# LiyaoTang/contrastBoundary

Hardware: AMD Instinct MI355X
Metric: points/sec through KNN+group+KPConv+CBL block, S3DIS N=40960 K=16 (higher is better)
Workload: dtype f32

## Files before the change

contrastboundary_amd/csrc/knn_dispatch.hip:

```cpp
#include "cbl_common.h"

size_t cbl_knn_grid_workspace_bytes(int b, int n, int m, int nsample);
int cbl_knn_grid_launch(int b, int n, int m, int nsample, const float* xyz, const float* new_xyz, const int* offset,
                        const int* new_offset, int* idx, float* dist2, void* ws, size_t ws_bytes, int set_exact, hipStream_t st, int* order_out, CblKnnNarrow* narrow);

size_t cbl_knn_select_workspace_bytes(int b, int n, int m, int nsample);
int cbl_knn_select_launch(int b, int n, int m, int nsample, const float* xyz, const float* new_xyz, const int* offset, const int* new_offset,
                          int* idx, float* dist2, void* ws, size_t ws_bytes, int set_exact, hipStream_t st);

CBL_EXPORT size_t cbl_knnquery_workspace_bytes(int b, int n, int m, int nsample)
{
    const size_t g = cbl_knn_grid_workspace_bytes(b, n, m, nsample);
    return g ? g : cbl_knn_select_workspace_bytes(b, n, m, nsample);
}

static int knnquery_impl(int b, int n, int m, int nsample, const float* xyz, const float* new_xyz,
                         const int* offset, const int* new_offset, int* idx, float* dist2,
                         void* workspace, size_t workspace_bytes, int set_exact, void* stream, int* order_out = nullptr, CblKnnNarrow* narrow = nullptr)
{
    if (b <= 0 || n < 0 || m < 0 || nsample <= 0 || nsample > CBL_KNN_MAX_NSAMPLE) return CBL_ERR_BAD_ARG;
    if (m == 0) return CBL_OK;
    if (!xyz || !new_xyz || !offset || !new_offset || !idx || !dist2) return CBL_ERR_BAD_ARG;
    const size_t need = cbl_knn_grid_workspace_bytes(b, n, m, nsample);
    if (need > 0 && workspace && workspace_bytes >= need)
        return cbl_knn_grid_launch(b, n, m, nsample, xyz, new_xyz, offset, new_offset, idx, dist2, workspace, workspace_bytes, set_exact, cbl_stream(stream), order_out, narrow);
    if (order_out) return CBL_ERR_UNSUPPORTED;
    const size_t need_sel = cbl_knn_select_workspace_bytes(b, n, m, nsample);
    if (need_sel > 0 && workspace && workspace_bytes >= need_sel)
        return cbl_knn_select_launch(b, n, m, nsample, xyz, new_xyz, offset, new_offset, idx, dist2, workspace, workspace_bytes, set_exact, cbl_stream(stream));
    return cbl_knnquery_exact(b, n, m, nsample, xyz, new_xyz, offset, new_offset, idx, dist2, stream);
}

CBL_EXPORT int cbl_knnquery(int b, int n, int m, int nsample, const float* xyz, const float* new_xyz,
                            const int* offset, const int* new_offset, int* idx, float* dist2,
                            void* workspace, size_t workspace_bytes, void* stream)
{
    return knnquery_impl(b, n, m, nsample, xyz, new_xyz, offset, new_offset, idx, dist2, workspace, workspace_bytes, 0, stream);
}

CBL_EXPORT int cbl_knnquery_set(int b, int n, int m, int nsample, const float* xyz, const float* new_xyz,
                                const int* offset, const int* new_offset, int* idx, float* dist2,
                                void* workspace, size_t workspace_bytes, void* stream)
{
    return knnquery_impl(b, n, m, nsample, xyz, new_xyz, offset, new_offset, idx, dist2, workspace, workspace_bytes, 1, stream);
}

CBL_EXPORT int cbl_knnquery_anytie(int b, int n, int m, int nsample, const float* xyz, const float* new_xyz,
                                   const int* offset, const int* new_offset, int* idx, float* dist2,
                                   void* workspace, size_t workspace_bytes, void* stream)
{
    return knnquery_impl(b, n, m, nsample, xyz, new_xyz, offset, new_offset, idx, dist2, workspace, workspace_bytes, 2, stream);
}

CBL_EXPORT int cbl_knnquery_ordered(int b, int n, int m, int nsample, const float* xyz, const float* new_xyz,
                                    const int* offset, const int* new_offset, int* idx, float* dist2, int tie_policy, int* cell_order,
                                    void* workspace, size_t workspace_bytes, void* stream)
{
    if (tie_policy < 0 || tie_policy > 2 || !cell_order) return CBL_ERR_BAD_ARG;
    return knnquery_impl(b, n, m, nsample, xyz, new_xyz, offset, new_offset, idx, dist2, workspace, workspace_bytes, tie_policy, stream, cell_order);
}

int cbl_knn_block_candidates_launch(int b, int n, const int* offset, void* ws, int* count, hipStream_t st);

CBL_EXPORT int cbl_knn_grid_block_candidates(int b, int n, int nsample, const int* offset, int* count, void* workspace, size_t workspace_bytes, void* stream)
{
    const size_t need = cbl_knn_grid_workspace_bytes(b, n, n, nsample);
    if (need == 0) return CBL_ERR_UNSUPPORTED;
    if (workspace_bytes < need) return CBL_ERR_WORKSPACE;
    return cbl_knn_block_candidates_launch(b, n, offset, workspace, count, cbl_stream(stream));
}

int cbl_knn_exact_worklist(int b, int m, int K, const float* xyz, const float* new_xyz, const int* offset, const int* new_offset,
                           int* idx, float* dist2, const int* worklist, const int* worklist_count, int max_work, hipStream_t st,
                           const void* grids, const int* cell_start, const void* sorted);

namespace {
__global__ __launch_bounds__(256) void knn_prefix_kernel(int m, int kb, int ks, const int* __restrict__ idx_big, const float* __restrict__ d2_big,
                                                         int* __restrict__ idx, float* __restrict__ dist2, int set_exact,
                                                         int* __restrict__ worklist, int* __restrict__ counter)
{
    const int q = blockIdx.x * 256 + threadIdx.x;
    if (q >= m) return;
    const int* ib = idx_big + (size_t)q * kb; const float* db = d2_big + (size_t)q * kb;
    float prev = -1.f; bool dup = false, dup0 = false;
    for (int j = 0; j < ks; j++) {
        const float d = db[j];
        idx[(size_t)q * ks + j] = ib[j]; dist2[(size_t)q * ks + j] = d;
        dup = dup || (d == prev);
        dup0 = dup0 || (j == 1 && d == prev);
        prev = d;
    }
    const bool full = prev < 1e10f;
    const bool boundary = db[ks] == prev;
    const bool ok = full && !boundary && (set_exact ? !dup0 : !dup);
    if (!ok) worklist[atomicAdd(counter, 1)] = q;
}
template <int KS>
__global__ __launch_bounds__(256) void knn_prefix_pow2_kernel(int m, int kb, const int* __restrict__ idx_big, const float* __restrict__ d2_big,
                                                              int* __restrict__ idx, float* __restrict__ dist2, int set_exact,
                                                              int* __restrict__ worklist, int* __restrict__ counter)
{
    const long long e = (long long)blockIdx.x * 256 + threadIdx.x;
    const int lane = threadIdx.x & 63;
    const long long qq = e / KS;
    const int j = (int)(e - qq * KS);
    const bool live = qq < m;
    const int q = live ? (int)qq : m - 1;
    const float d = d2_big[(size_t)q * kb + j], dn = d2_big[(size_t)q * kb + j + 1];
    if (live) { idx[(size_t)q * KS + j] = idx_big[(size_t)q * kb + j]; dist2[(size_t)q * KS + j] = d; }
    const bool last = j == KS - 1;
    const bool bad = (d == dn && (last || j == 0 || !set_exact)) || (last && !(d < 1e10f));
    const unsigned long long bm = __ballot(bad && live);
    const unsigned long long gm = (KS == 64) ? bm : ((bm >> (lane & ~(KS - 1))) & ((1ull << KS) - 1ull));
    if (live && j == 0 && gm != 0ull) worklist[atomicAdd(counter, 1)] = q;
}
}

void cbl_knn_grid_scratch(void* ws, int b, int n, int m, int** worklist, int** worklist2, int** zero_counter, const void** grids,
                          const int** cell_start, const void** sorted);
int cbl_knn_exact_worklist2(int b, int m, const float* xyz, const float* new_xyz, const int* offset, const int* new_offset,
                            int K1, int* idx1, float* dist2_1, const int* worklist1, const int* count1,
                            int K2, int* idx2, float* dist2_2, const int* worklist2, const int* count2,
                            hipStream_t st, const void* grids, const int* cell_start, const void* sorted);

static int launch_prefix(int m, int nsample_wide, int nsample, const int* idx_wide, const float* dist2_wide, int* idx, float* dist2, int tie_policy,
                         int* worklist, int* counter, hipStream_t st)
{
#define CBL_PREFIX_POW2(KS) hipLaunchKernelGGL(knn_prefix_pow2_kernel<KS>, dim3(cbl_div_up((long long)m * KS, 256)), dim3(256), 0, st, m, nsample_wide, idx_wide, dist2_wide, \
                                               idx, dist2, tie_policy, worklist, counter)
    switch (nsample) {
        case 1: CBL_PREFIX_POW2(1); break;
        case 2: CBL_PREFIX_POW2(2); break;
        case 4: CBL_PREFIX_POW2(4); break;
        case 8: CBL_PREFIX_POW2(8); break;
        case 16: CBL_PREFIX_POW2(16); break;
        case 32: CBL_PREFIX_POW2(32); break;
        default:
            hipLaunchKernelGGL(knn_prefix_kernel, dim3(cbl_div_up(m, 256)), dim3(256), 0, st, m, nsample_wide, nsample, idx_wide, dist2_wide, idx, dist2, tie_policy, worklist, counter);
    }
#undef CBL_PREFIX_POW2
    return cbl_status();
}

CBL_EXPORT int cbl_knnquery_nested(int b, int n, int m, int nsample_wide, int tie_policy_wide, int nsample, int tie_policy,
                                   const float* xyz, const float* new_xyz, const int* offset, const int* new_offset,
                                   int* idx_wide, float* dist2_wide, int* idx, float* dist2, int* cell_order, void* event_after_wide,
                                   void* workspace, size_t workspace_bytes, void* stream)
{
    if (nsample <= 0 || nsample >= nsample_wide || tie_policy < 0 || tie_policy > 1 || tie_policy_wide < 0 || tie_policy_wide > 2 || !idx || !dist2) return CBL_ERR_BAD_ARG;
    const size_t need = cbl_knn_grid_workspace_bytes(b, n, m, nsample_wide);
    if (need == 0 || !workspace || workspace_bytes < need) return CBL_ERR_UNSUPPORTED;
    CblKnnNarrow narrow{nsample, tie_policy, idx, dist2, false, true};
    int rc = knnquery_impl(b, n, m, nsample_wide, xyz, new_xyz, offset, new_offset, idx_wide, dist2_wide, workspace, workspace_bytes, tie_policy_wide, stream, cell_order, &narrow);
    if (rc || m == 0) return rc;
    hipStream_t st = cbl_stream(stream);
    int *worklist, *worklist2, *counter; const void *grids, *sorted; const int* cell_start;
    cbl_knn_grid_scratch(workspace, b, n, m, &worklist, &worklist2, &counter, &grids, &cell_start, &sorted);
    if (narrow.fused) {
        const bool self = (new_xyz == xyz) && (m == n);
        rc = cbl_knn_exact_worklist2(b, m, xyz, new_xyz, offset, self ? offset : new_offset, nsample_wide, idx_wide, dist2_wide, worklist, counter - 1,
                                     nsample, idx, dist2, worklist2, counter, st, grids, cell_start, sorted);
        if (rc) return rc;
        if (event_after_wide && hipEventRecord(reinterpret_cast<hipEvent_t>(event_after_wide), st) != hipSuccess) return cbl_status() ? cbl_status() : CBL_ERR_BAD_ARG;
        return cbl_status();
    }
    if (event_after_wide && hipEventRecord(reinterpret_cast<hipEvent_t>(event_after_wide), st) != hipSuccess) return cbl_status() ? cbl_status() : CBL_ERR_BAD_ARG;
    {
        rc = launch_prefix(m, nsample_wide, nsample, idx_wide, dist2_wide, idx, dist2, tie_policy, worklist, counter, st);
        if (rc) return rc;
    }
    return cbl_knn_exact_worklist(b, m, nsample, xyz, new_xyz, offset, new_offset, idx, dist2, worklist, counter, m, st, grids, cell_start, sorted);
}

CBL_EXPORT size_t cbl_knnquery_prefix_workspace_bytes(int m) { return m < 0 ? 0 : sizeof(int) * ((size_t)m + 64); }

CBL_EXPORT int cbl_knnquery_prefix(int b, int n, int m, int nsample_wide, int nsample, const float* xyz, const float* new_xyz,
                                   const int* offset, const int* new_offset, const int* idx_wide, const float* dist2_wide,
                                   int* idx, float* dist2, int tie_policy, void* workspace, size_t workspace_bytes, void* stream)
{
    (void)n;
    if (b <= 0 || m < 0 || nsample <= 0 || nsample >= nsample_wide || nsample_wide > CBL_KNN_MAX_NSAMPLE || tie_policy < 0 || tie_policy > 1) return CBL_ERR_BAD_ARG;
    if (m == 0) return CBL_OK;
    if (!xyz || !new_xyz || !offset || !new_offset || !idx_wide || !dist2_wide || !idx || !dist2 || !workspace) return CBL_ERR_BAD_ARG;
    if (workspace_bytes < cbl_knnquery_prefix_workspace_bytes(m)) return CBL_ERR_WORKSPACE;
    hipStream_t st = cbl_stream(stream);
    int* counter = reinterpret_cast<int*>(workspace);
    int* worklist = counter + 64;
    (void)hipMemsetAsync(counter, 0, sizeof(int), st);
    { const int rcp = launch_prefix(m, nsample_wide, nsample, idx_wide, dist2_wide, idx, dist2, tie_policy, worklist, counter, st); if (rcp) return rcp; }
    const int rc = cbl_status();
    if (rc) return rc;
    return cbl_knn_exact_worklist(b, m, nsample, xyz, new_xyz, offset, new_offset, idx, dist2, worklist, counter, m, st, nullptr, nullptr, nullptr);
}
```

contrastboundary_amd/csrc/knn_grid.hip:

```cpp
#include "cbl_common.h"
#include <cstdlib>
#include "grid_core.h"
#include <knn_wave.h>

int cbl_knn_exact_worklist(int b, int m, int K, const float* xyz, const float* new_xyz, const int* offset,
                           const int* new_offset, int* idx, float* dist2,
                           const int* worklist, const int* worklist_count, int max_work, hipStream_t st,
                           const void* grids, const int* cell_start, const void* sorted);

namespace {

constexpr int GRID_MAX_K = 64;
constexpr int CELLS_PER_POINT = 2;
constexpr int CELLS_PER_CLOUD = 64;

struct Workspace {
    CblGrid* grids;
    int* counters;
    unsigned* bbox;
    int* cell_count;
    int* cell_start;
    int* cell_local;
    int* tile_sum;
    int* pt_cell;
// ... 1 lines not shown
    int* worklist;
    int* worklist2;
    size_t bytes;
    int ncap;
};

inline size_t align_up(size_t v) { return (v + 255) & ~(size_t)255; }

Workspace carve(void* base, int b, int n, int m)
{
    Workspace w;
    w.ncap = CELLS_PER_POINT * n + CELLS_PER_CLOUD * b;
    char* p = reinterpret_cast<char*>(base);
    size_t off = 0;
    auto take = [&](size_t bytes) { char* r = p ? p + off : nullptr; off += align_up(bytes); return r; };
    w.grids = reinterpret_cast<CblGrid*>(take(sizeof(CblGrid) * (size_t)b));
    w.counters = reinterpret_cast<int*>(take(sizeof(int) * 64));
    w.bbox = reinterpret_cast<unsigned*>(take(sizeof(unsigned) * 6 * (size_t)b));
    w.cell_count = reinterpret_cast<int*>(take(sizeof(int) * ((size_t)w.ncap + 1)));
    w.cell_start = reinterpret_cast<int*>(take(sizeof(int) * ((size_t)w.ncap + 1)));
    w.cell_local = reinterpret_cast<int*>(take(sizeof(int) * ((size_t)w.ncap + 1)));
    w.tile_sum = reinterpret_cast<int*>(take(sizeof(int) * ((size_t)w.ncap / 4096 + 2)));
    w.pt_cell = reinterpret_cast<int*>(take(sizeof(int) * (size_t)n));
    w.sorted = reinterpret_cast<float4*>(take(sizeof(float4) * (size_t)n));
    w.worklist = reinterpret_cast<int*>(take(sizeof(int) * (size_t)m));
    w.worklist2 = reinterpret_cast<int*>(take(sizeof(int) * (size_t)m));
    w.bytes = off;
    return w;
}

__device__ __forceinline__ unsigned f2key(float f) { const unsigned u = __float_as_uint(f); return (u & 0x80000000u) ? ~u : (u | 0x80000000u); }
__device__ __forceinline__ float key2f(unsigned k) { return __uint_as_float((k & 0x80000000u) ? (k & 0x7fffffffu) : ~k); }

__global__ __launch_bounds__(256) void grid_bbox_kernel(int b, int n, const float* __restrict__ xyz, const int* __restrict__ offset,
                                                        unsigned* __restrict__ bbox)
{
    const int per = (n + gridDim.x - 1) / gridDim.x;
    const int r0 = blockIdx.x * per, r1 = min(n, r0 + per);
    const int lane = threadIdx.x & 63;
    int i = r0 + threadIdx.x;
    if (r0 >= r1) return;
    {
        const int cfirst = cbl_cloud_of(r0, offset, b);
        if (cfirst == cbl_cloud_of(r1 - 1, offset, b)) {
            __shared__ float red[6][4];
            float lo[3] = {INFINITY, INFINITY, INFINITY}, hi[3] = {-INFINITY, -INFINITY, -INFINITY};
            for (; i < r1; i += 256) {
#pragma unroll
                for (int a = 0; a < 3; a++) { const float v = xyz[3 * i + a]; lo[a] = fminf(lo[a], v); hi[a] = fmaxf(hi[a], v); }
            }
#pragma unroll
            for (int a = 0; a < 3; a++) {
                for (int s = 32; s >= 1; s >>= 1) { lo[a] = fminf(lo[a], __shfl_xor(lo[a], s)); hi[a] = fmaxf(hi[a], __shfl_xor(hi[a], s)); }
                if (lane == 0) { red[a][threadIdx.x >> 6] = lo[a]; red[3 + a][threadIdx.x >> 6] = hi[a]; }
            }
            __syncthreads();
            if (threadIdx.x < 6) {
                const int a = threadIdx.x;
                const float v0 = red[a][0], v1 = red[a][1], v2 = red[a][2], v3 = red[a][3];
                if (a < 3) atomicMin(bbox + cfirst * 6 + a, f2key(fminf(fminf(v0, v1), fminf(v2, v3))));
                else       atomicMax(bbox + cfirst * 6 + a, f2key(fmaxf(fmaxf(v0, v1), fmaxf(v2, v3))));
            }
            return;
        }
    }
    while (__any(i < r1)) {
        const bool act = i < r1;
        const int myc = act ? cbl_cloud_of(i, offset, b) : -1;
        const int lead = __builtin_ctzll(__ballot(act));
        const int c0 = __shfl(myc, lead);
        float lo[3] = {INFINITY, INFINITY, INFINITY}, hi[3] = {-INFINITY, -INFINITY, -INFINITY};
        if (act && myc == c0) {
            const int cend = min(r1, offset[c0]);
            for (; i < cend; i += 256) {
#pragma unroll
                for (int a = 0; a < 3; a++) { const float v = xyz[3 * i + a]; lo[a] = fminf(lo[a], v); hi[a] = fmaxf(hi[a], v); }
            }
        }
#pragma unroll
        for (int a = 0; a < 3; a++) {
            for (int s = 32; s >= 1; s >>= 1) { lo[a] = fminf(lo[a], __shfl_xor(lo[a], s)); hi[a] = fmaxf(hi[a], __shfl_xor(hi[a], s)); }
            if (lane == 0 && lo[a] <= hi[a]) { atomicMin(bbox + c0 * 6 + a, f2key(lo[a])); atomicMax(bbox + c0 * 6 + 3 + a, f2key(hi[a])); }
        }
    }
}

__device__ __forceinline__ CblGrid grid_of_cloud(int c, float pts_per_cell, const int* __restrict__ offset, const unsigned* __restrict__ bbox)
{
    const int start = c ? offset[c - 1] : 0, end = offset[c];
    float l[3] = {0.f, 0.f, 0.f}, h[3] = {0.f, 0.f, 0.f};
    if (end > start)
        for (int a = 0; a < 3; a++) { l[a] = key2f(bbox[c * 6 + a]); h[a] = key2f(bbox[c * 6 + 3 + a]); }
    CblGrid g;
    const int cap = CELLS_PER_POINT * (end - start) + CELLS_PER_CLOUD;
    if (pts_per_cell < 0.f) cbl_grid_choose_radius(g, l, h, -pts_per_cell, cap);
    else cbl_grid_choose(g, l, h, end - start, pts_per_cell, cap);
    g.cell_base = CELLS_PER_POINT * start + CELLS_PER_CLOUD * c;
    g.start = start; g.end = end; g.pad0 = g.pad1 = 0;
    return g;
}

__global__ __launch_bounds__(256) void grid_count_kernel(int b, int n, float pts_per_cell, const float* __restrict__ xyz, const int* __restrict__ offset,
                                                         const unsigned* __restrict__ bbox, CblGrid* __restrict__ grids,
                                                         int* __restrict__ pt_cell, int* __restrict__ cell_count)
{
    if (blockIdx.x == 0)
        for (int c = threadIdx.x; c < b; c += 256) grids[c] = grid_of_cloud(c, pts_per_cell, offset, bbox);
    int cached_c = -1; CblGrid g;
    for (int i = blockIdx.x * 256 + threadIdx.x; i < n; i += gridDim.x * 256) {
        const int c = cbl_cloud_of(i, offset, b);
        if (c != cached_c) { g = grid_of_cloud(c, pts_per_cell, offset, bbox); cached_c = c; }
        const int cell = cbl_cell_of(g, xyz[3 * i], xyz[3 * i + 1], xyz[3 * i + 2]);
        pt_cell[i] = cell;
        atomicAdd(cell_count + cell, 1);
    }
}

constexpr int SCAN_TILE = 4096;

__global__ __launch_bounds__(256) void grid_scan_tiles_kernel(int total, const int* __restrict__ cell_count, int* __restrict__ cell_start_local,
                                                              int* __restrict__ tile_sum)
{
    __shared__ int wsum[4];
    const int tid = threadIdx.x, lane = tid & 63, wave = tid >> 6;
    const int base = blockIdx.x * SCAN_TILE + tid * 16;
    int v[16];
#pragma unroll
    for (int j = 0; j < 16; j += 4) {
        if (base + j + 3 < total) {
            const int4 x = *reinterpret_cast<const int4*>(cell_count + base + j);
            v[j] = x.x; v[j + 1] = x.y; v[j + 2] = x.z; v[j + 3] = x.w;
        } else {
#pragma unroll
            for (int k = 0; k < 4; k++) v[j + k] = (base + j + k < total) ? cell_count[base + j + k] : 0;
        }
    }
    int sum = 0;
#pragma unroll
    for (int j = 0; j < 16; j++) { const int x = v[j]; v[j] = sum; sum += x; }
    int incl = sum;
#pragma unroll
    for (int s = 1; s < 64; s <<= 1) { const int o = __shfl_up(incl, s); if (lane >= s) incl += o; }
    if (lane == 63) wsum[wave] = incl;
    __syncthreads();
    int off = incl - sum;
    for (int w = 0; w < wave; w++) off += wsum[w];
    if (tid == 255) tile_sum[blockIdx.x] = off + sum;
#pragma unroll
    for (int j = 0; j < 16; j++) if (base + j < total) cell_start_local[base + j] = off + v[j];
}

__global__ __launch_bounds__(256) void grid_scatter_kernel(int n, int total, int ntiles, const float* __restrict__ xyz, const int* __restrict__ pt_cell,
                                                           const int* __restrict__ tile_sum, int* __restrict__ cell_start_local, int* __restrict__ cell_start,
                                                           int* __restrict__ cell_count, float4* __restrict__ sorted, int* __restrict__ order_out)
{
    extern __shared__ int tile_lds[];
    int* tile_pre = tile_lds + ntiles;
    {
        for (int t = threadIdx.x; t < ntiles; t += 256) tile_lds[t] = tile_sum[t];
        __syncthreads();
        for (int t = threadIdx.x; t < ntiles; t += 256) { int run = 0; for (int u = 0; u < t; u++) run += tile_lds[u]; tile_pre[t] = run; }
        __syncthreads();
    }
    for (int i = blockIdx.x * 256 + threadIdx.x; i < total; i += gridDim.x * 256) cell_start[i] = cell_start_local[i] + tile_pre[i / SCAN_TILE];
    for (int i = blockIdx.x * 256 + threadIdx.x; i < n; i += gridDim.x * 256) {
        const int cell = pt_cell[i];
        const int pos = cell_start_local[cell] + tile_pre[cell / SCAN_TILE] + atomicSub(cell_count + cell, 1) - 1;
        sorted[pos] = make_float4(xyz[3 * i], xyz[3 * i + 1], xyz[3 * i + 2], __int_as_float(i));
        if (order_out) order_out[pos] = i;
    }
}

__device__ __forceinline__ void grid_order_canon_body(int n, const int* __restrict__ pt_cell, const int* __restrict__ cell_start,
                                                      const float4* __restrict__ sorted, int* __restrict__ order, int block, int nblocks)
{
    for (int i = block * 256 + threadIdx.x; i < n; i += nblocks * 256) {
        const int cell = pt_cell[i];
        const int s = cell_start[cell], e = cell_start[cell + 1];
        if (e - s < 2 || e - s > 1024) continue;
        int rank = 0;
        for (int j = s; j < e; j += 8) {
            int v[8];
#pragma unroll
            for (int u = 0; u < 8; u++) v[u] = __float_as_int(sorted[min(j + u, e - 1)].w);
#pragma unroll
            for (int u = 0; u < 8; u++) rank += (j + u < e && v[u] < i) ? 1 : 0;
        }
        order[s + rank] = i;
    }
}
__global__ __launch_bounds__(256) void grid_order_canon_kernel(int n, const int* __restrict__ pt_cell, const int* __restrict__ cell_start,
                                                               const float4* __restrict__ sorted, int* __restrict__ order)
{
    grid_order_canon_body(n, pt_cell, cell_start, sorted, order, blockIdx.x, gridDim.x);
}
struct CblCanon { int blocks, n; const int* pt_cell; int* order; };

template <int G> __device__ __forceinline__ float dpp_shr1_f(float v);
template <int G> __device__ __forceinline__ int dpp_shr1_i(int v);
template <> __device__ __forceinline__ int dpp_shr1_i<16>(int v) { return __builtin_amdgcn_update_dpp(v, v, 0x111, 0xf, 0xf, false); }
template <> __device__ __forceinline__ int dpp_shr1_i<64>(int v) { return __builtin_amdgcn_update_dpp(v, v, 0x138, 0xf, 0xf, false); }
template <> __device__ __forceinline__ int dpp_shr1_i<32>(int v) { return __builtin_amdgcn_update_dpp(v, v, 0x138, 0xf, 0xf, false); }
template <int G> __device__ __forceinline__ int dpp_shr1_zero(int v)
{
    if constexpr (G == 16) return __builtin_amdgcn_update_dpp(0, v, 0x111, 0xf, 0xf, true);
    else                   return __builtin_amdgcn_update_dpp(0, v, 0x138, 0xf, 0xf, true);
}
template <> __device__ __forceinline__ float dpp_shr1_f<16>(float v) { return __int_as_float(dpp_shr1_i<16>(__float_as_int(v))); }
template <> __device__ __forceinline__ float dpp_shr1_f<64>(float v) { return __int_as_float(dpp_shr1_i<64>(__float_as_int(v))); }
template <> __device__ __forceinline__ float dpp_shr1_f<32>(float v) { return __int_as_float(dpp_shr1_i<32>(__float_as_int(v))); }

constexpr int WV_NB = 16;

template <int CTRL> __device__ __forceinline__ int dppx_i(int v) { return __builtin_amdgcn_update_dpp(0, v, CTRL, 0xf, 0xf, true); }
struct PermQuadXor1  { __device__ __forceinline__ int operator()(int v, int) const { return dppx_i<0xB1>(v); } };
struct PermQuadXor2  { __device__ __forceinline__ int operator()(int v, int) const { return dppx_i<0x4E>(v); } };
struct PermQuadMir   { __device__ __forceinline__ int operator()(int v, int) const { return dppx_i<0x1B>(v); } };
struct PermHalfMir   { __device__ __forceinline__ int operator()(int v, int) const { return dppx_i<0x141>(v); } };
struct PermRowMir    { __device__ __forceinline__ int operator()(int v, int) const { return dppx_i<0x140>(v); } };
struct PermRowRor8   { __device__ __forceinline__ int operator()(int v, int) const { return dppx_i<0x128>(v); } };
struct PermSwzXor4   { __device__ __forceinline__ int operator()(int v, int) const { return __builtin_amdgcn_ds_swizzle(v, 0x101f); } };
struct PermSwzXor16  { __device__ __forceinline__ int operator()(int v, int) const { return __builtin_amdgcn_ds_swizzle(v, 0x401f); } };
struct PermSwzMir32  { __device__ __forceinline__ int operator()(int v, int) const { return __builtin_amdgcn_ds_swizzle(v, 0x7c1f); } };
struct PermMir64     { __device__ __forceinline__ int operator()(int v, int lane) const { return __builtin_amdgcn_ds_bpermute((63 - lane) << 2, v); } };

template <bool LEX, class Perm> __device__ __forceinline__ void sort_cx(float& d, int& i, bool lower, int lane, Perm perm)
{
    const float pd = __int_as_float(perm(__float_as_int(d), lane));
    const int pi = perm(i, lane);
    if (LEX) {
        const bool take = lower ? (pd < d || (pd == d && (unsigned)pi < (unsigned)i)) : (pd > d || (pd == d && (unsigned)pi > (unsigned)i));
        d = take ? pd : d; i = take ? pi : i;
    } else {
        const int di = __float_as_int(d), pdi = __float_as_int(pd);
        const int nd = lower ? min(di, pdi) : max(di, pdi);
        i = (nd != di) ? pi : i; d = __int_as_float(nd);
    }
}
template <bool LEX> __device__ __forceinline__ void wave_sort64(float& d, int& i, int lane)
{
    const bool l1 = !(lane & 1), l2 = !(lane & 2), l4 = !(lane & 4), l8 = !(lane & 8), l16 = !(lane & 16), l32 = !(lane & 32);
    sort_cx<LEX>(d, i, l1, lane, PermQuadXor1());
    sort_cx<LEX>(d, i, l2, lane, PermQuadMir());   sort_cx<LEX>(d, i, l1, lane, PermQuadXor1());
    sort_cx<LEX>(d, i, l4, lane, PermHalfMir());   sort_cx<LEX>(d, i, l2, lane, PermQuadXor2()); sort_cx<LEX>(d, i, l1, lane, PermQuadXor1());
    sort_cx<LEX>(d, i, l8, lane, PermRowMir());    sort_cx<LEX>(d, i, l4, lane, PermSwzXor4());  sort_cx<LEX>(d, i, l2, lane, PermQuadXor2());
    sort_cx<LEX>(d, i, l1, lane, PermQuadXor1());
    sort_cx<LEX>(d, i, l16, lane, PermSwzMir32()); sort_cx<LEX>(d, i, l8, lane, PermRowRor8());  sort_cx<LEX>(d, i, l4, lane, PermSwzXor4());
    sort_cx<LEX>(d, i, l2, lane, PermQuadXor2());  sort_cx<LEX>(d, i, l1, lane, PermQuadXor1());
    sort_cx<LEX>(d, i, l32, lane, PermMir64());    sort_cx<LEX>(d, i, l16, lane, PermSwzXor16()); sort_cx<LEX>(d, i, l8, lane, PermRowRor8());
    sort_cx<LEX>(d, i, l4, lane, PermSwzXor4());   sort_cx<LEX>(d, i, l2, lane, PermQuadXor2()); sort_cx<LEX>(d, i, l1, lane, PermQuadXor1());
}
__device__ __forceinline__ float rl_f(float v, int l) { return __int_as_float(__builtin_amdgcn_readlane(__float_as_int(v), l)); }
template <int G> __device__ __forceinline__ float group_min_nonneg(float f)
{
    int v = __float_as_int(f);
    v = min(v, dppx_i<0xB1>(v)); v = min(v, dppx_i<0x4E>(v)); v = min(v, dppx_i<0x141>(v)); v = min(v, dppx_i<0x140>(v));
    if constexpr (G == 32) v = min(v, __builtin_amdgcn_ds_swizzle(v, 0x401f));
    if constexpr (G == 64) v = min(min(__builtin_amdgcn_readlane(v, 0), __builtin_amdgcn_readlane(v, 16)),
                                   min(__builtin_amdgcn_readlane(v, 32), __builtin_amdgcn_readlane(v, 48)));
    return __int_as_float(v);
}

template <int G, bool SELF, bool LEX>
__global__ __launch_bounds__(256) void knn_grid_group_kernel(int b, int m, int K, const float* __restrict__ new_xyz,
                                                             const int* __restrict__ offset, const int* __restrict__ new_offset,
                                                             const CblGrid* __restrict__ grids, const int* __restrict__ cell_start,
                                                             const float4* __restrict__ sorted, int* __restrict__ idx, float* __restrict__ dist2,
                                                             int* __restrict__ worklist, int* __restrict__ counters, int set_exact)
{
    constexpr int QPW = 64 / G;
    using mask_t = unsigned long long;
    const int lane = threadIdx.x & 63;
    const int gl = lane & (G - 1);
    const int grp = lane / G;
    const int wave_global = (blockIdx.x * 256 + threadIdx.x) >> 6;
    const int t = wave_global * QPW + grp;
    const bool live = t < m;
    const int tt = live ? t : m - 1;

    int q; float qx, qy, qz;
    if (SELF) { const float4 s = sorted[tt]; q = __float_as_int(s.w); qx = s.x; qy = s.y; qz = s.z; }
    else      { q = tt; qx = new_xyz[3 * q]; qy = new_xyz[3 * q + 1]; qz = new_xyz[3 * q + 2]; }
    const int c = cbl_cloud_of(q, SELF ? offset : new_offset, b);
    const CblGrid g = grids[c];
    const float uqx = cbl_u(qx, g.ox, g.inv_cs), uqy = cbl_u(qy, g.oy, g.inv_cs), uqz = cbl_u(qz, g.oz, g.inv_cs);
    const int cx = cbl_cell_coord(uqx, g.nx), cy = cbl_cell_coord(uqy, g.ny), cz = cbl_cell_coord(uqz, g.nz);

    float ed = INFINITY; int ei = -1;
    float rejmin = INFINITY;
    int evict = 0x7f800000;
    const int last_src = ((lane & ~(G - 1)) + K - 1) << 2;
    bool done = !live;

    int rs9 = 0, re9 = 0;
    if (!done && gl < 9) {
        const int o = (int)((0xa82091645ull >> (4 * gl)) & 0xFull);
        const int y = cy + (o & 3) - 1, z = cz + (o >> 2) - 1;
        if (y >= 0 && y < g.ny && z >= 0 && z < g.nz) {
            const int row = g.cell_base + g.nx * (y + g.ny * z);
            rs9 = cell_start[row + max(cx - 1, 0)]; re9 = cell_start[row + min(cx + 1, g.nx - 1) + 1];
        }
    }
    const int grp_src = (lane & ~(G - 1)) << 2;

    for (int r = 1;; r++) {
        const int side = 2 * r + 1;
        for (int ri = 0; ri < side * side; ri++) {
            int dy, dz;
            if (r == 1) { const int o = (int)((0xa82091645ull >> (4 * ri)) & 0xFull); dy = (o & 3) - 1; dz = (o >> 2) - 1; }
            else        { dz = ri / side - r; dy = ri % side - r; }
            {
                const bool full = (r == 1) || dz == -r || dz == r || dy == -r || dy == r;
                const int nseg = full ? 1 : 2;
                for (int sg = 0; sg < nseg; sg++) {
                    int x0, x1;
                    if (full) { x0 = max(cx - r, 0); x1 = min(cx + r, g.nx - 1); }
                    else      { x0 = x1 = sg ? cx + r : cx - r; }
                    const int y = cy + dy, z = cz + dz;
                    int s = 0, e = 0;
                    if (r == 1) {
                        s = __builtin_amdgcn_ds_bpermute(grp_src + (ri << 2), rs9); e = __builtin_amdgcn_ds_bpermute(grp_src + (ri << 2), re9);
                    } else if (!done && y >= 0 && y < g.ny && z >= 0 && z < g.nz && x0 >= 0 && x1 <= g.nx - 1) {
                        const int row = g.cell_base + g.nx * (y + g.ny * z);
                        s = cell_start[row + x0]; e = cell_start[row + x1 + 1];
                    }
                    for (int p = s; __any(p < e); p += G) {
                        const int pi = p + gl;
                        float d2 = INFINITY; int ci = -1;
                        if (pi < e) {
                            const float4 v = sorted[pi];
                            d2 = cbl_dist2(qx, qy, qz, v.x, v.y, v.z);
                            ci = __float_as_int(v.w);
                        }
                        const float worst = __int_as_float(__builtin_amdgcn_ds_bpermute(last_src, __float_as_int(ed)));
                        const unsigned worst_i = LEX ? (unsigned)__builtin_amdgcn_ds_bpermute(last_src, ei) : 0u;
                        const bool pass = d2 < worst || (LEX && d2 == worst && (unsigned)ci < worst_i);
                        rejmin = __int_as_float(min(__float_as_int(rejmin), pass ? 0x7f800000 : __float_as_int(d2)));
                        if constexpr (!LEX && G <= 32) {
                            unsigned gm = (unsigned)(__ballot(pass) >> (grp * G)) & (G == 32 ? ~0u : ((1u << G) - 1u));
                            const int d2i = __float_as_int(d2);
                            auto step = [&]() {
                                const bool has = gm != 0;
                                const int l = kw_ffbl(gm);
                                gm &= gm - 1;
                                const int src = (l << 2) + grp * (G * 4);
                                int dci = __builtin_amdgcn_ds_bpermute(src, d2i); const int ic = __builtin_amdgcn_ds_bpermute(src, ci);
                                dci = has ? dci : 0x7f800000;
                                const int edi = __float_as_int(ed);
                                int pdi = dpp_shr1_zero<G>(edi), pidx = dpp_shr1_zero<G>(ei);
                                if (G == 32) pdi = gl ? pdi : 0;
                                evict = min(evict, max(edi, dci));
                                ei = (edi > dci) ? ((pdi > dci) ? pidx : ic) : ei;
                                ed = __int_as_float(min(edi, max(pdi, dci)));
                            };
                            while (__any(gm != 0)) {
                                step();
                                if (!__any(gm != 0)) break;
                                step();
                            }
                        } else {
                        mask_t gm = (__ballot(pass) >> (grp * G)) & (G == 64 ? ~0ull : ((1ull << G) - 1ull));
                        while (__any(gm != 0)) {
                            const bool has = gm != 0;
                            const int l = has ? __builtin_ctzll(gm) : 0;
                            gm &= gm - 1;
                            float dc = __shfl(d2, l, G); int ic = __shfl(ci, l, G);
                            if (!has) { dc = INFINITY; ic = -1; }
                            const float pd = dpp_shr1_f<G>(ed); const int pidx = dpp_shr1_i<G>(ei);
                            const bool gt = ed > dc || (LEX && ed == dc && (unsigned)ei > (unsigned)ic);
                            const bool left_gt = (gl > 0) && (pd > dc || (LEX && pd == dc && (unsigned)pidx > (unsigned)ic));
                            if (gl == K - 1) rejmin = fminf(rejmin, gt ? ed : dc);
                            if (gt) { if (left_gt) { ed = pd; ei = pidx; } else { ed = dc; ei = ic; } }
                        }
                        }
                    }
                }
            }
        }
        const float bound2 = cbl_outside_bound2(g, uqx, uqy, uqz, cx, cy, cz, r);
        const float worst = __int_as_float(__builtin_amdgcn_ds_bpermute(last_src, __float_as_int(ed)));
        if (!done) done = (bound2 == INFINITY) || (worst < bound2);
        if (__all(done)) break;
    }

    const float worst = __int_as_float(__builtin_amdgcn_ds_bpermute(last_src, __float_as_int(ed)));
    const float rm = group_min_nonneg<G>(fminf(rejmin, gl == K - 1 ? __int_as_float(evict) : INFINITY));
    const float pd = dpp_shr1_f<G>(ed);
    const bool dup = (gl > 0) && (gl < K) && (ed == pd);
    const mask_t dm = (__ballot(dup) >> (grp * G)) & (G == 64 ? ~0ull : ((1ull << G) - 1ull));
    const bool ok = (worst < INFINITY) && (set_exact == 2 || ((rm != worst) && (set_exact ? !(dm & 2ull) : dm == 0)));
    if (live) {
        if (gl < K) { idx[(size_t)q * K + gl] = ei; dist2[(size_t)q * K + gl] = ed; }
        if (!ok && gl == 0) worklist[atomicAdd(counters, 1)] = q;
    }
}


template <bool SELF, bool LEX>
__global__ __launch_bounds__(256) void knn_grid_wave_kernel(int b, int m, int K, const float* __restrict__ new_xyz,
                                                            const int* __restrict__ offset, const int* __restrict__ new_offset,
                                                            const CblGrid* __restrict__ grids, const int* __restrict__ cell_start,
                                                            const float4* __restrict__ sorted, int* __restrict__ idx, float* __restrict__ dist2,
                                                            int* __restrict__ worklist, int* __restrict__ counters, int set_exact,
                                                            int ks, int* __restrict__ idx_n, float* __restrict__ dist2_n,
                                                            int* __restrict__ worklist_n, int set_exact_n, CblCanon canon)
{
    __shared__ float2 slots[4][64];
    if ((int)blockIdx.x < canon.blocks) {
        grid_order_canon_body(canon.n, canon.pt_cell, cell_start, sorted, canon.order, blockIdx.x, canon.blocks);
        return;
    }
    const int lane = threadIdx.x & 63, wv = threadIdx.x >> 6;
    const int t = __builtin_amdgcn_readfirstlane(((int)blockIdx.x - canon.blocks) * 4 + wv);
    if (t >= m) return;
    int q; float qx, qy, qz;
    if (SELF) { const float4 s = sorted[t]; q = __float_as_int(s.w); qx = s.x; qy = s.y; qz = s.z; }
    else      { q = t; qx = new_xyz[3 * q]; qy = new_xyz[3 * q + 1]; qz = new_xyz[3 * q + 2]; }
    q = __builtin_amdgcn_readfirstlane(q);
    const int c = cbl_cloud_of(q, SELF ? offset : new_offset, b);
    const CblGrid g = grids[c];
    const float uqx = cbl_u(qx, g.ox, g.inv_cs), uqy = cbl_u(qy, g.oy, g.inv_cs), uqz = cbl_u(qz, g.oz, g.inv_cs);
    const int cx = cbl_cell_coord(uqx, g.nx), cy = cbl_cell_coord(uqy, g.ny), cz = cbl_cell_coord(uqz, g.nz);

    int rs = 0, rlen = 0;
    if (lane < 9) {
        const int y = cy + lane % 3 - 1, z = cz + lane / 3 - 1;
        if (y >= 0 && y < g.ny && z >= 0 && z < g.nz) {
            const int row = g.cell_base + g.nx * (y + g.ny * z);
            rs = cell_start[row + max(cx - 1, 0)];
            rlen = cell_start[row + min(cx + 1, g.nx - 1) + 1] - rs;
        }
    }
    int pre[9], delta[9], T = 0;
#pragma unroll
    for (int r = 0; r < 9; r++) {
        const int s_r = __builtin_amdgcn_readlane(rs, r), l_r = __builtin_amdgcn_readlane(rlen, r);
        pre[r] = T; delta[r] = s_r - T; T += l_r;
    }

    float ed = INFINITY; int ei = -1;
    float rejmin = INFINITY;
    bool fast = (T >= K) && (T <= 64 * WV_NB);
    if (fast) {
        float d[WV_NB]; int id[WV_NB];
        int delta_v[9];
#pragma unroll
        for (int r = 0; r < 9; r++) delta_v[r] = kw_in_vgpr(delta[r]);
#pragma unroll
        for (int j0 = 0; j0 < WV_NB; j0 += 4) {
            float4 p[4];
#pragma unroll
            for (int u = 0; u < 4; u++) {
                if ((j0 + u) * 64 < T) {
                    const int v = min((j0 + u) * 64 + lane, T - 1);
                    int dl = delta_v[0];
#pragma unroll
                    for (int r = 1; r < 9; r++) dl = (v >= pre[r]) ? delta_v[r] : dl;
                    p[u] = sorted[v + dl];
                }
            }
#pragma unroll
            for (int u = 0; u < 4; u++) {
                const int j = j0 + u;
                d[j] = INFINITY; id[j] = -1;
                if (j * 64 < T) {
                    const bool in = j * 64 + lane < T;
                    const float dd = cbl_dist2(qx, qy, qz, p[u].x, p[u].y, p[u].z);
                    d[j] = in ? dd : INFINITY; id[j] = in ? __float_as_int(p[u].w) : -1;
                }
            }
        }
        float tau = 3.0e38f;
        if (T > 64) {
            int mxi = 0;
#pragma unroll
            for (int j = 0; j < WV_NB; j++) {
                if ((j + 1) * 64 <= T) mxi = max(mxi, __float_as_int(d[j]));
                else if (j * 64 < T)   mxi = max(mxi, d[j] < INFINITY ? __float_as_int(d[j]) : 0);
            }
            mxi = max(mxi, dppx_i<0xB1>(mxi)); mxi = max(mxi, dppx_i<0x4E>(mxi));
            mxi = max(mxi, dppx_i<0x141>(mxi)); mxi = max(mxi, dppx_i<0x140>(mxi));
            float lo = -1.f, hi = __int_as_float(max(max(__builtin_amdgcn_readlane(mxi, 0), __builtin_amdgcn_readlane(mxi, 16)),
                                                     max(__builtin_amdgcn_readlane(mxi, 32), __builtin_amdgcn_readlane(mxi, 48))));
            const float first = (float)(K + 64) * 0.6f * __builtin_amdgcn_rcpf((float)T);
            fast = false;
            for (int it = 0; it < 40; it++) {
                const float mid = it == 0 ? hi * first : lo + (hi - lo) * 0.5f;
                if (!(mid > lo && mid < hi)) break;
                int cnt = 0;
#pragma unroll
                for (int j = 0; j < WV_NB; j++) if (j * 64 < T) cnt += __popcll(__ballot(d[j] <= mid));
                if (cnt < K) lo = mid; else if (cnt > 64) hi = mid; else { tau = mid; fast = true; break; }
            }
        }
        if (fast) {
            int base = 0;
#pragma unroll
            for (int j = 0; j < WV_NB; j++) {
                if (j * 64 < T) {
                    const bool pass = d[j] <= tau;
                    const unsigned long long mk = __ballot(pass);
                    if (pass) {
                        const int slot = base + __builtin_amdgcn_mbcnt_hi((unsigned)(mk >> 32), __builtin_amdgcn_mbcnt_lo((unsigned)mk, 0));
                        slots[wv][slot] = make_float2(d[j], __int_as_float(id[j]));
                    } else rejmin = fminf(rejmin, d[j]);
                    base += __popcll(mk);
                }
            }
            __builtin_amdgcn_fence(__ATOMIC_RELEASE, "wavefront");
            __builtin_amdgcn_wave_barrier();
            __builtin_amdgcn_fence(__ATOMIC_ACQUIRE, "wavefront");
            float sd = INFINITY; int si = -1;
            if (lane < base) { const float2 v = slots[wv][lane]; sd = v.x; si = __float_as_int(v.y); }
            wave_sort64<LEX>(sd, si, lane);
            if (lane < K) { ed = sd; ei = si; } else rejmin = fminf(rejmin, sd);
        }
    }

    bool done = false;
    int r = 1;
    if (fast) {
        const float bound2 = cbl_outside_bound2(g, uqx, uqy, uqz, cx, cy, cz, 1);
        done = (bound2 == INFINITY) || (rl_f(ed, K - 1) < bound2);
        r = 2;
    }
    for (; !done; r++) {
        const int side = 2 * r + 1;
        for (int ri = 0; ri < side * side; ri++) {
            const int dz = ri / side - r, dy = ri % side - r;
            const bool full = (r == 1) || dz == -r || dz == r || dy == -r || dy == r;
            const int nseg = full ? 1 : 2;
            for (int sg = 0; sg < nseg; sg++) {
                int x0, x1;
                if (full) { x0 = max(cx - r, 0); x1 = min(cx + r, g.nx - 1); }
                else      { x0 = x1 = sg ? cx + r : cx - r; }
                const int y = cy + dy, z = cz + dz;
                int s = 0, e = 0;
                if (y >= 0 && y < g.ny && z >= 0 && z < g.nz && x0 >= 0 && x1 <= g.nx - 1) {
                    const int row = g.cell_base + g.nx * (y + g.ny * z);
                    s = cell_start[row + x0]; e = cell_start[row + x1 + 1];
                }
                s = __builtin_amdgcn_readfirstlane(s); e = __builtin_amdgcn_readfirstlane(e);
                for (int p = s; p < e; p += 64) {
                    const int pi = p + lane;
                    float d2 = INFINITY; int ci = -1;
                    if (pi < e) {
                        const float4 v = sorted[pi];
                        d2 = cbl_dist2(qx, qy, qz, v.x, v.y, v.z);
                        ci = __float_as_int(v.w);
                    }
                    const float worst = rl_f(ed, K - 1); const unsigned worst_i = LEX ? (unsigned)__builtin_amdgcn_readlane(ei, K - 1) : 0u;
                    const bool pass = d2 < worst || (LEX && d2 == worst && (unsigned)ci < worst_i);
                    rejmin = fminf(rejmin, pass ? INFINITY : d2);
                    unsigned long long gm = __ballot(pass);
                    while (gm) {
                        const int l = __builtin_ctzll(gm);
                        gm &= gm - 1;
                        const float dc = rl_f(d2, l); const int ic = __builtin_amdgcn_readlane(ci, l);
                        const float pd = dpp_shr1_f<64>(ed); const int pidx = dpp_shr1_i<64>(ei);
                        const bool gt = ed > dc || (LEX && ed == dc && (unsigned)ei > (unsigned)ic);
                        const bool left_gt = (lane > 0) && (pd > dc || (LEX && pd == dc && (unsigned)pidx > (unsigned)ic));
                        if (lane == K - 1) rejmin = fminf(rejmin, gt ? ed : dc);
// ... 34 lines not shown
}


template <int G>
__device__ __forceinline__ unsigned long long group_min_u64(unsigned long long v)
{
#pragma unroll
    for (int s = G / 2; s >= 1; s >>= 1) {
        const unsigned lo = __shfl_xor((unsigned)v, s, G), hi = __shfl_xor((unsigned)(v >> 32), s, G);
        const unsigned long long o = ((unsigned long long)hi << 32) | lo;
        v = o < v ? o : v;
    }
    return v;
}

__device__ __forceinline__ unsigned long long radius_key_lds(int t, int total, int c1, int c2, int c3, int c4, int c5, int c6, int c7, int c8, const int* __restrict__ otab,
                                                              float qx, float qy, float qz, float r2, const float4* __restrict__ sorted)
{
    const bool have = t < total;
    const int r = (t >= c1) + (t >= c2) + (t >= c3) + (t >= c4) + (t >= c5) + (t >= c6) + (t >= c7) + (t >= c8);
    const int o = otab[r];
    const float4 v = sorted[have ? t + o : 0];
    const float d2 = cbl_dist2(qx, qy, qz, v.x, v.y, v.z);
    return (have && d2 < r2) ? (((unsigned long long)__float_as_uint(d2) << 32) | (unsigned)__float_as_int(v.w)) : ~0ull;
}

template <int G, int U>
__global__ __launch_bounds__(256) void radius_group_kernel(int b, int nq, int ns_total, int limit, float r2, const float* __restrict__ queries,
                                                           const int* __restrict__ q_offset, const CblGrid* __restrict__ grids,
                                                           const int* __restrict__ cell_start, const float4* __restrict__ sorted,
                                                           int* __restrict__ out, int* __restrict__ counts, int* __restrict__ max_count)
{
    constexpr int QPW = 64 / G, CAP = 2 * G, NBF = G >= 64 ? 2 : 4;
    using mask_t = unsigned long long;
    using key_t = unsigned long long;
    constexpr key_t NONE = ~0ull;
    __shared__ key_t slots[4 * QPW][CAP];
    __shared__ int otabs[4 * QPW][U][12];
    const int lane = threadIdx.x & 63, gl = lane & (G - 1), grp = lane / G;
    key_t* S = slots[(threadIdx.x >> 6) * QPW + grp];
    const int wave_global = (blockIdx.x * 256 + threadIdx.x) >> 6;
    const mask_t below = (1ull << gl) - 1ull, gmask = G == 64 ? ~0ull : ((1ull << G) - 1ull);
    int q[U]; bool live[U]; float qx[U], qy[U], qz[U];
#pragma unroll
    for (int u = 0; u < U; u++) {
        const int t = (wave_global * QPW + grp) * U + u;
        live[u] = t < nq; q[u] = live[u] ? t : nq - 1;
        qx[u] = queries[3 * q[u]]; qy[u] = queries[3 * q[u] + 1]; qz[u] = queries[3 * q[u] + 2];
    }
    int rs[U], re[U];
#pragma unroll
    for (int u = 0; u < U; u++) {
        const int c = cbl_cloud_of(q[u], q_offset, b);
        const CblGrid g = grids[c];
        const int cx = cbl_cell_coord(cbl_u(qx[u], g.ox, g.inv_cs), g.nx), cy = cbl_cell_coord(cbl_u(qy[u], g.oy, g.inv_cs), g.ny),
                  cz = cbl_cell_coord(cbl_u(qz[u], g.oz, g.inv_cs), g.nz);
        const int x0 = max(cx - 1, 0), x1 = min(cx + 1, g.nx - 1);
        rs[u] = 0; re[u] = 0;
        if (gl < 9) {
            const int y = cy + (gl % 3) - 1, z = cz + (gl / 3) - 1;
            if (live[u] && g.end > g.start && y >= 0 && y < g.ny && z >= 0 && z < g.nz) {
                const int row = g.cell_base + g.nx * (y + g.ny * z);
                rs[u] = cell_start[row + x0]; re[u] = cell_start[row + x1 + 1];
            }
        }
    }
    int c1[U], c2[U], c3[U], c4[U], c5[U], c6[U], c7[U], c8[U], total[U];
#pragma unroll
    for (int u = 0; u < U; u++) {
        int* otab = otabs[(threadIdx.x >> 6) * QPW + grp][u];
        int acc = 0;
#define CBL_ROW(r, cnext) { const int sr = __shfl(rs[u], r, G), er = __shfl(re[u], r, G); if (gl == 0) otab[r] = sr - acc; acc += er - sr; cnext = acc; }
        CBL_ROW(0, c1[u]) CBL_ROW(1, c2[u]) CBL_ROW(2, c3[u]) CBL_ROW(3, c4[u]) CBL_ROW(4, c5[u]) CBL_ROW(5, c6[u]) CBL_ROW(6, c7[u]) CBL_ROW(7, c8[u])
        CBL_ROW(8, total[u])
#undef CBL_ROW
    }
#define CBL_KEY(u, t) radius_key_lds((t), total[u], c1[u], c2[u], c3[u], c4[u], c5[u], c6[u], c7[u], c8[u], otabs[(threadIdx.x >> 6) * QPW + grp][u], qx[u], qy[u], qz[u], r2, sorted)
    key_t first[U][NBF];
#pragma unroll
    for (int u = 0; u < U; u++)
#pragma unroll
        for (int k = 0; k < NBF; k++) first[u][k] = CBL_KEY(u, k * G + gl);
#pragma unroll
    for (int u = 0; u < U; u++) {
        int inside = 0;
        auto collect = [&](key_t key) __attribute__((always_inline)) {
            const bool in_ball = key != NONE;
            const mask_t gm = (__ballot(in_ball) >> (grp * G)) & gmask;
            const int slot = inside + __popcll(gm & below);
            if (in_ball && slot < CAP) S[slot] = key;
            inside += __popcll(gm);
        };
#pragma unroll
        for (int k = 0; k < NBF; k++) collect(first[u][k]);
        for (int t0 = NBF * G; __any(t0 < total[u]); t0 += G) collect(CBL_KEY(u, t0 + gl));
        const bool over = inside > CAP;
        if (!over) {
            const int n = inside;
            const key_t ka = gl < n ? S[gl] : NONE, kb = gl + G < n ? S[gl + G] : NONE;
            int ra = 0, rb = 0;
            for (int k = 0; __any(k < n); k += 4) {
                key_t kk[4];
#pragma unroll
                for (int j = 0; j < 4; j++) kk[j] = S[min(k + j, CAP - 1)];
#pragma unroll
                for (int j = 0; j < 4; j++) {
                    const bool on = k + j < n;
                    ra += (on && kk[j] < ka) ? 1 : 0; rb += (on && kk[j] < kb) ? 1 : 0;
                }
            }
            if (live[u]) {
                if (ka != NONE && ra < limit) out[(size_t)q[u] * limit + ra] = (int)(unsigned)ka;
                if (kb != NONE && rb < limit) out[(size_t)q[u] * limit + rb] = (int)(unsigned)kb;
                if (gl >= n && gl < limit) out[(size_t)q[u] * limit + gl] = ns_total;
            }
        }
        if (__any(over)) {
            key_t prev = 0; bool none_yet = true;
            for (int col = 0; col < limit; col++) {
                key_t best = NONE;
                for (int t0 = 0; __any(over && t0 < total[u]); t0 += G) {
                    const key_t key = CBL_KEY(u, t0 + gl);
                    if ((none_yet || key > prev) && key < best) best = key;
                }
                best = group_min_u64<G>(best);
                if (over && live[u] && gl == 0) out[(size_t)q[u] * limit + col] = best == NONE ? ns_total : (int)(unsigned)best;
                prev = best; none_yet = false;
            }
        }
        if (live[u] && gl == 0) {
            if (counts) counts[q[u]] = inside;
            if (inside > __hip_atomic_load(max_count, __ATOMIC_RELAXED, __HIP_MEMORY_SCOPE_AGENT)) atomicMax(max_count, inside);
        }
    }
#undef CBL_KEY
}

}

int cbl_bbox_keys_launch(int b, int n, const float* xyz, const int* offset, unsigned* bbox, hipStream_t st)
{
    hipLaunchKernelGGL(grid_bbox_kernel, dim3(cbl_grid_for(n, 1024, 512)), dim3(256), 0, st, b, n, xyz, offset, bbox);
    return cbl_status();
}

__global__ __launch_bounds__(256) void grid_init_kernel(int b, int total, int* __restrict__ counters, unsigned* __restrict__ bbox, int* __restrict__ cell_count)
{
    const int i0 = blockIdx.x * 256 + threadIdx.x;
    if (i0 < 64) counters[i0] = 0;
    if (i0 < 6 * b) bbox[i0] = ((i0 % 6) < 3) ? 0xffffffffu : 0u;
    for (int i = i0; i < total; i += gridDim.x * 256) cell_count[i] = 0;
}

int cbl_grid_build(int b, int n, float pts_per_cell, const float* xyz, const int* offset, void* ws, hipStream_t st, int* order_out = nullptr, bool canon_later = false)
{
    Workspace w = carve(ws, b, n, 0);
    const int total = w.ncap + 1, ntiles = (total + SCAN_TILE - 1) / SCAN_TILE;
    hipLaunchKernelGGL(grid_init_kernel, dim3(cbl_grid_for(total, 256, 512)), dim3(256), 0, st, b, total, w.counters, w.bbox, w.cell_count);
    hipLaunchKernelGGL(grid_bbox_kernel, dim3(cbl_grid_for(n, 1024, 512)), dim3(256), 0, st, b, n, xyz, offset, w.bbox);
    hipLaunchKernelGGL(grid_count_kernel, dim3(cbl_grid_for(n, 256)), dim3(256), 0, st, b, n, pts_per_cell, xyz, offset, w.bbox, w.grids, w.pt_cell, w.cell_count);
    hipLaunchKernelGGL(grid_scan_tiles_kernel, dim3(ntiles), dim3(256), 0, st, total, w.cell_count, w.cell_local, w.tile_sum);
    hipLaunchKernelGGL(grid_scatter_kernel, dim3(cbl_grid_for(n, 256)), dim3(256), 2 * sizeof(int) * (size_t)ntiles, st, n, total, ntiles, xyz, w.pt_cell,
                       w.tile_sum, w.cell_local, w.cell_start, w.cell_count, w.sorted, order_out);
    if (order_out && !canon_later)
        hipLaunchKernelGGL(grid_order_canon_kernel, dim3(cbl_grid_for(n, 256)), dim3(256), 0, st, n, w.pt_cell, w.cell_start, w.sorted, order_out);
    return cbl_status();
}

__global__ __launch_bounds__(256) void knn_block_candidates_kernel(int b, int n, const int* __restrict__ offset, const CblGrid* __restrict__ grids,
                                                                   const int* __restrict__ cell_start, const float4* __restrict__ sorted, int* __restrict__ count)
{
    const int t = blockIdx.x * 256 + threadIdx.x;
    if (t >= n) return;
    const float4 s = sorted[t];
    const int q = __float_as_int(s.w);
    const CblGrid g = grids[cbl_cloud_of(q, offset, b)];
    const int cx = cbl_cell_coord(cbl_u(s.x, g.ox, g.inv_cs), g.nx), cy = cbl_cell_coord(cbl_u(s.y, g.oy, g.inv_cs), g.ny), cz = cbl_cell_coord(cbl_u(s.z, g.oz, g.inv_cs), g.nz);
    int T = 0;
    for (int r = 0; r < 9; r++) {
        const int y = cy + r % 3 - 1, z = cz + r / 3 - 1;
        if (y >= 0 && y < g.ny && z >= 0 && z < g.nz) {
            const int row = g.cell_base + g.nx * (y + g.ny * z);
            T += cell_start[row + min(cx + 1, g.nx - 1) + 1] - cell_start[row + max(cx - 1, 0)];
        }
    }
    count[q] = T;
}

int cbl_knn_block_candidates_launch(int b, int n, const int* offset, void* ws, int* count, hipStream_t st)
{
    Workspace w = carve(ws, b, n, n);
    hipLaunchKernelGGL(knn_block_candidates_kernel, dim3(cbl_grid_for(n, 256, 1 << 20)), dim3(256), 0, st, b, n, offset, w.grids, w.cell_start, w.sorted, count);
    return cbl_status();
}

size_t cbl_knn_grid_workspace_bytes(int b, int n, int m, int nsample)
{
    if (nsample > GRID_MAX_K || n < 2048 || b <= 0) return 0;
    if ((long long)CELLS_PER_POINT * n + (long long)CELLS_PER_CLOUD * b > 0x3fffffffLL) return 0;
    return carve(nullptr, b, n, m).bytes;
}

void cbl_knn_grid_scratch(void* ws, int b, int n, int m, int** worklist, int** worklist2, int** zero_counter, const void** grids, const int** cell_start,
                          const void** sorted)
{
    Workspace w = carve(ws, b, n, m);
    *worklist = w.worklist; *worklist2 = w.worklist2; *zero_counter = w.counters + 1;
    *grids = w.grids; *cell_start = w.cell_start; *sorted = w.sorted;
}

int cbl_knn_grid_launch(int b, int n, int m, int nsample, const float* xyz, const float* new_xyz, const int* offset,
                        const int* new_offset, int* idx, float* dist2, void* ws, size_t ws_bytes, int set_exact, hipStream_t st, int* order_out,
                        CblKnnNarrow* narrow)
{
    Workspace w = carve(ws, b, n, m);
    if (ws_bytes < w.bytes) return CBL_ERR_WORKSPACE;
    static const float fill = [] { const char* e = getenv("CBL_KNN_CELL_FILL"); const float v = e ? (float)atof(e) : 0.f; return (v > 0.05f && v < 4.f) ? v : 0.33f; }();
    const bool wave_search = nsample > 16;
    int rc = cbl_grid_build(b, n, fill * (float)(nsample < 4 ? 4 : nsample), xyz, offset, ws, st, order_out, wave_search);
    if (rc) return rc;
    const bool self = (new_xyz == xyz) && (m == n);
    if (wave_search) {
        CblCanon canon = {0, n, w.pt_cell, order_out};
        if (order_out) canon.blocks = (int)cbl_grid_for(n, 256);
        const dim3 grid(cbl_div_up(m, 4) + canon.blocks), block(256);
        const int ks = narrow ? narrow->nsample : 0;
        int* idx_n = narrow ? narrow->idx : nullptr; float* dist2_n = narrow ? narrow->dist2 : nullptr;
        const int set_n = narrow ? narrow->set_exact : 0;
        if (narrow) narrow->fused = true;
#define CBL_LAUNCH_WAVE(SELF_, LEX_) hipLaunchKernelGGL((knn_grid_wave_kernel<SELF_, LEX_>), grid, block, 0, st, b, m, nsample, new_xyz, offset, new_offset, w.grids, \
                                                       w.cell_start, w.sorted, idx, dist2, w.worklist, w.counters, set_exact, ks, idx_n, dist2_n, w.worklist2, set_n, canon)
        if (set_exact == 2) { if (self) CBL_LAUNCH_WAVE(true, true); else CBL_LAUNCH_WAVE(false, true); }
        else                { if (self) CBL_LAUNCH_WAVE(true, false); else CBL_LAUNCH_WAVE(false, false); }
#undef CBL_LAUNCH_WAVE
    }
    else launch_query<16>(self, b, m, nsample, new_xyz, offset, new_offset, w, idx, dist2, set_exact, st);
    rc = cbl_status();
    if (rc) return rc;
    if (narrow && narrow->fused && narrow->defer_replay) return CBL_OK;
    return cbl_knn_exact_worklist(b, m, nsample, xyz, new_xyz, self ? offset : offset, self ? offset : new_offset, idx, dist2,
                                  w.worklist, w.counters, m, st, w.grids, w.cell_start, w.sorted);
}

size_t cbl_radius_workspace_bytes_impl(int b, int ns) { return (b > 0 && ns >= 0) ? carve(nullptr, b, ns, 0).bytes : 0; }

int cbl_radius_launch(int b, int nq, int ns, const float* queries, const float* supports, const int* q_offset, const int* s_offset,
                      float radius, int limit, int* out, int* counts, int* max_count, void* ws, size_t ws_bytes, hipStream_t st, bool grid_is_built)
{
    Workspace w = carve(ws, b, ns, 0);
    if (ws_bytes < w.bytes) return CBL_ERR_WORKSPACE;
    int rc = grid_is_built ? CBL_OK : cbl_grid_build(b, ns, -radius, supports, s_offset, ws, st);
    if (rc) return rc;
    hipError_t e = hipMemsetAsync(max_count, 0, sizeof(int), st);
    if (e != hipSuccess) return (int)e;
    const int G = limit <= 16 ? 16 : limit <= 32 ? 32 : 64;
    const long long waves = ((long long)nq + (64 / G) - 1) / (64 / G);
    const dim3 grid(cbl_div_up(waves, 4)), block(256);
    const float r2 = radius * radius;
    const int ru = (long long)nq / ((64 / G) * 2) >= 49152 ? 2 : 1;
    const long long waves_u = ((long long)nq + (64 / G) * ru - 1) / ((64 / G) * ru);
    const dim3 grid_u(cbl_div_up(waves_u, 4));
#define CBL_RAD(G_, U_) hipLaunchKernelGGL((radius_group_kernel<G_, U_>), grid_u, block, 0, st, b, nq, ns, limit, r2, queries, q_offset, w.grids, w.cell_start, w.sorted, out, counts, max_count)
    if (ru == 2) { if (G == 16) CBL_RAD(16, 2); else if (G == 32) CBL_RAD(32, 2); else CBL_RAD(64, 2); }
    else         { if (G == 16) CBL_RAD(16, 1); else if (G == 32) CBL_RAD(32, 1); else CBL_RAD(64, 1); }
#undef CBL_RAD
    return cbl_status();
}
```

contrastboundary_amd/csrc/neighbor_transpose.hip:

```cpp
#include "cbl_common.h"
#include <stdlib.h>

namespace {

constexpr int TT = 64;
constexpr int TS = 64;
constexpr int NB = 256;
constexpr int NT_MAX_TILES = 16384;
constexpr int NT_SCAN_SPLIT = 2048;
constexpr int STAGE_CAP = 12288;


struct NtWs {
    int* rank;
    int* tile_cursor;
    int* list_cursor;
    int* tile_list_off;
    int* tile_list_n;
    int* tile_base;
    int2* lists;
    int2* bins;
    int* scratch;
};

static size_t nt_align(size_t v) { return (v + 255) & ~(size_t)255; }
static int nt_tiles(int n) { return (n + TT - 1) / TT; }
static int nt_src_tiles(int m) { return (m + TS - 1) / TS; }

static size_t nt_carve(NtWs& w, char* base, int m, int n, int nsample)
{
    const size_t P = (size_t)m * nsample;
    const int ntt = nt_tiles(n), nst = nt_src_tiles(m);
    size_t off = 0;
    auto take = [&](size_t bytes) { char* p = base ? base + off : nullptr; off += nt_align(bytes); return p; };
    w.rank = (int*)take(sizeof(int) * (size_t)(n > 0 ? n : 1));
    w.tile_cursor = (int*)take(sizeof(int) * (size_t)(ntt + 2));
    w.list_cursor = w.tile_cursor ? w.tile_cursor + ntt + 1 : nullptr;
    w.tile_list_off = (int*)take(sizeof(int) * (size_t)(nst + 1));
    w.tile_list_n = (int*)take(sizeof(int) * (size_t)(nst + 1));
    w.tile_base = (int*)take(sizeof(int) * (size_t)(ntt + 2));
    w.lists = (int2*)take(sizeof(int2) * (P ? P : 1));
    w.bins = (int2*)take(sizeof(int2) * (P ? P : 1));
    w.scratch = (int*)take(sizeof(int) * (P ? P : 1));
    return off;
}

__global__ __launch_bounds__(NB) void nt_prep_kernel(int n, int nzero, const int* __restrict__ order, int* __restrict__ rank, int* __restrict__ zero,
                                                     int* __restrict__ zero2)
{
    const int i = blockIdx.x * NB + threadIdx.x;
    if (order && i < n) rank[order[i]] = i;
    if (i < nzero) { zero[i] = 0; if (zero2) zero2[i] = 0; }
}

template <int UN> struct NtPairs { unsigned p[UN]; int r[UN]; };

template <int UN>
__device__ __forceinline__ void nt_load_pairs(NtPairs<UN>& q, unsigned base, unsigned total, int n, int ns, CblFastDiv dv, const int* __restrict__ src_ids,
                                              const int* __restrict__ idx, const int* __restrict__ rank)
{
    int t[UN];
#pragma unroll
    for (int u = 0; u < UN; u++) {
        const unsigned e = base + (unsigned)u * NB + threadIdx.x;
        const bool in = e < total;
        const unsigned sl = cbl_fastdiv(in ? e : 0u, dv), col = (in ? e : 0u) - sl * (unsigned)ns;
        q.p[u] = (unsigned)src_ids[sl] * (unsigned)ns + col;
        t[u] = in ? idx[q.p[u]] : -1;
    }
#pragma unroll
    for (int u = 0; u < UN; u++) {
        const bool ok = (unsigned)t[u] < (unsigned)n;
        q.r[u] = ok ? (rank ? rank[t[u]] : t[u]) : -1;
    }
}

struct NtJob {
    int ns; CblFastDiv dv; const int* idx;
    int *tile_cursor, *list_cursor, *tile_list_off, *tile_list_n, *tile_base; int2 *lists, *bins; int* scratch;
    int *inv_start, *inv_src;
};

template <int UN>
__device__ __forceinline__ void nt_count_body(int* lds, int m, int n, int ns, int ntt, CblFastDiv dv, const int* __restrict__ idx, const int* __restrict__ order_src,
                                              const int* __restrict__ rank, int* __restrict__ tile_cursor, int* __restrict__ list_cursor,
                                              int* __restrict__ tile_list_off, int* __restrict__ tile_list_n, int2* __restrict__ lists)
{
    int* hist = lds;
    int2* mine = reinterpret_cast<int2*>(lds + ((ntt + 1) & ~1));
    __shared__ int nmine, gbase, src_ids[TS];
    const int st = blockIdx.x;
    const int nsrc = min(TS, m - st * TS);
    if ((int)threadIdx.x < TS) src_ids[threadIdx.x] = (int)threadIdx.x < nsrc ? (order_src ? order_src[st * TS + threadIdx.x] : st * TS + (int)threadIdx.x) : 0;
    for (int e = threadIdx.x; e < ntt; e += NB) hist[e] = 0;
    if (threadIdx.x == 0) nmine = 0;
    __syncthreads();
    const unsigned total = (unsigned)nsrc * (unsigned)ns;
    for (unsigned base = 0; base < total; base += UN * NB) {
        NtPairs<UN> q;
        nt_load_pairs<UN>(q, base, total, n, ns, dv, src_ids, idx, rank);
#pragma unroll
        for (int u = 0; u < UN; u++) if (q.r[u] >= 0) atomicAdd(&hist[q.r[u] / TT], 1);
    }
    __syncthreads();
    for (int tt = threadIdx.x; tt < ntt; tt += NB) {
        const int c = hist[tt];
        if (c) {
            const int off = atomicAdd(&tile_cursor[tt], c);
            mine[atomicAdd(&nmine, 1)] = make_int2(tt, off);
        }
    }
    __syncthreads();
    if (threadIdx.x == 0) { gbase = st * TS * ns; tile_list_off[st] = gbase; tile_list_n[st] = nmine; }
    __syncthreads();
    for (int e = threadIdx.x; e < nmine; e += NB) lists[gbase + e] = mine[e];
}
template <int UN>
__global__ __launch_bounds__(NB) void nt_count_kernel(int m, int n, int ns, int ntt, CblFastDiv dv, const int* __restrict__ idx, const int* __restrict__ order_src,
                                                      const int* __restrict__ rank, int* __restrict__ tile_cursor, int* __restrict__ list_cursor,
                                                      int* __restrict__ tile_list_off, int* __restrict__ tile_list_n, int2* __restrict__ lists)
{
    extern __shared__ int lds[];
    nt_count_body<UN>(lds, m, n, ns, ntt, dv, idx, order_src, rank, tile_cursor, list_cursor, tile_list_off, tile_list_n, lists);
}
template <int UNA, int UNB>
__global__ __launch_bounds__(NB) void nt_count_pair_kernel(int m, int n, int ntt, const int* __restrict__ order_src, const int* __restrict__ rank, NtJob a, NtJob b)
{
    extern __shared__ int lds[];
    if (blockIdx.y == 0) nt_count_body<UNA>(lds, m, n, a.ns, ntt, a.dv, a.idx, order_src, rank, a.tile_cursor, a.list_cursor, a.tile_list_off, a.tile_list_n, a.lists);
    else                 nt_count_body<UNB>(lds, m, n, b.ns, ntt, b.dv, b.idx, order_src, rank, b.tile_cursor, b.list_cursor, b.tile_list_off, b.tile_list_n, b.lists);
}

__global__ __launch_bounds__(1024) void nt_scan_kernel(int ntt, const int* __restrict__ tile_cursor, int* __restrict__ tile_base)
{
    __shared__ int wave_tot[16];
    constexpr int PER = NT_MAX_TILES / 1024;
    const int c0 = threadIdx.x * PER;
    int v[PER], sum = 0;
#pragma unroll
    for (int k = 0; k < PER; k++) { v[k] = (c0 + k < ntt) ? tile_cursor[c0 + k] : 0; sum += v[k]; }
    int incl = sum;
    for (int k = 1; k < 64; k <<= 1) { const int o = __shfl_up(incl, k); if ((int)(threadIdx.x & 63) >= k) incl += o; }
    if ((threadIdx.x & 63) == 63) wave_tot[threadIdx.x >> 6] = incl;
    __syncthreads();
    int run = incl - sum;
    for (int w = 0; w < (int)(threadIdx.x >> 6); w++) run += wave_tot[w];
#pragma unroll
    for (int k = 0; k < PER; k++) { if (c0 + k < ntt) tile_base[c0 + k] = run; run += v[k]; }
    if (threadIdx.x == 1023) tile_base[ntt] = run;
}

template <int UN, bool SCANNED>
__device__ __forceinline__ void nt_bin_body(int* lds, int m, int n, int ns, int ntt, CblFastDiv dv, const int* __restrict__ idx, const int* __restrict__ order_src,
                                            const int* __restrict__ rank, const int* __restrict__ tile_cursor, const int* __restrict__ tile_list_off,
                                            const int* __restrict__ tile_list_n, const int2* __restrict__ lists, int* __restrict__ tile_base,
                                            int2* __restrict__ bins)
{
    int* where = lds;
    int* hist = lds + ntt;
    __shared__ int wave_tot[NB / 64], src_ids[TS];
    const int st = blockIdx.x;
    const int nsrc = min(TS, m - st * TS);
    if ((int)threadIdx.x < TS) src_ids[threadIdx.x] = (int)threadIdx.x < nsrc ? (order_src ? order_src[st * TS + threadIdx.x] : st * TS + (int)threadIdx.x) : 0;
    if (SCANNED) {
        const int nl0 = tile_list_n[st], lo0 = tile_list_off[st];
        for (int e = threadIdx.x; e < nl0; e += NB) { const int2 r = lists[lo0 + e]; where[r.x] = tile_base[r.x] + r.y; hist[r.x] = 0; }
        __syncthreads();
    } else {
    for (int e = threadIdx.x; e < ntt; e += NB) { where[e] = tile_cursor[e]; hist[e] = 0; }
    __syncthreads();
    const int per = (ntt + NB - 1) / NB;
    const int c0 = threadIdx.x * per, c1 = min(ntt, c0 + per);
    int sum = 0;
    for (int e = c0; e < c1; e++) sum += where[e];
    int incl = sum;
    for (int k = 1; k < 64; k <<= 1) { const int v = __shfl_up(incl, k); if ((threadIdx.x & 63) >= k) incl += v; }
    if ((threadIdx.x & 63) == 63) wave_tot[threadIdx.x >> 6] = incl;
    __syncthreads();
    int run = incl - sum;
    for (int w = 0; w < (int)(threadIdx.x >> 6); w++) run += wave_tot[w];
    for (int e = c0; e < c1; e++) { const int c = where[e]; where[e] = run; if (st == 0) tile_base[e] = run; run += c; }
    if (st == 0 && threadIdx.x == NB - 1) tile_base[ntt] = run;
    __syncthreads();
    const int nl = tile_list_n[st], lo = tile_list_off[st];
    for (int e = threadIdx.x; e < nl; e += NB) { const int2 r = lists[lo + e]; where[r.x] += r.y; }
    __syncthreads();
    }
    const unsigned total = (unsigned)nsrc * (unsigned)ns;
    for (unsigned base = 0; base < total; base += UN * NB) {
        NtPairs<UN> q;
        nt_load_pairs<UN>(q, base, total, n, ns, dv, src_ids, idx, rank);
#pragma unroll
        for (int u = 0; u < UN; u++)
            if (q.r[u] >= 0) { const int tt = q.r[u] / TT; bins[where[tt] + atomicAdd(&hist[tt], 1)] = make_int2(q.r[u] & (TT - 1), (int)q.p[u]); }
    }
}
template <int UN, bool SCANNED>
__global__ __launch_bounds__(NB) void nt_bin_kernel(int m, int n, int ns, int ntt, CblFastDiv dv, const int* __restrict__ idx, const int* __restrict__ order_src,
                                                    const int* __restrict__ rank, const int* __restrict__ tile_cursor, const int* __restrict__ tile_list_off,
                                                    const int* __restrict__ tile_list_n, const int2* __restrict__ lists, int* __restrict__ tile_base,
                                                    int2* __restrict__ bins)
{
    extern __shared__ int lds[];
    nt_bin_body<UN, SCANNED>(lds, m, n, ns, ntt, dv, idx, order_src, rank, tile_cursor, tile_list_off, tile_list_n, lists, tile_base, bins);
}
template <int UNA, int UNB>
__global__ __launch_bounds__(NB) void nt_bin_pair_kernel(int m, int n, int ntt, const int* __restrict__ order_src, const int* __restrict__ rank, NtJob a, NtJob b)
{
    extern __shared__ int lds[];
    if (blockIdx.y == 0) nt_bin_body<UNA, false>(lds, m, n, a.ns, ntt, a.dv, a.idx, order_src, rank, a.tile_cursor, a.tile_list_off, a.tile_list_n, a.lists, a.tile_base, a.bins);
    else                 nt_bin_body<UNB, false>(lds, m, n, b.ns, ntt, b.dv, b.idx, order_src, rank, b.tile_cursor, b.tile_list_off, b.tile_list_n, b.lists, b.tile_base, b.bins);
}

constexpr int EPT = 16;

template <int CTRL> __device__ __forceinline__ int nt_dpp(int v) { return __builtin_amdgcn_update_dpp(0, v, CTRL, 0xf, 0xf, true); }
__device__ __forceinline__ int nt_cx(int v, int partner, bool lower) { return lower ? min(v, partner) : max(v, partner); }
__device__ __forceinline__ int nt_wave_sort64(int v, int lane)
{
    const bool l1 = !(lane & 1), l2 = !(lane & 2), l4 = !(lane & 4), l8 = !(lane & 8), l16 = !(lane & 16), l32 = !(lane & 32);
#define X1(v) nt_dpp<0xB1>(v)
#define X2(v) nt_dpp<0x4E>(v)
#define QM(v) nt_dpp<0x1B>(v)
#define HM(v) nt_dpp<0x141>(v)
#define RM(v) nt_dpp<0x140>(v)
#define R8(v) nt_dpp<0x128>(v)
#define S4(v) __builtin_amdgcn_ds_swizzle(v, 0x101f)
#define S16(v) __builtin_amdgcn_ds_swizzle(v, 0x401f)
#define M32(v) __builtin_amdgcn_ds_swizzle(v, 0x7c1f)
#define M64(v) __builtin_amdgcn_ds_bpermute((63 - lane) << 2, v)
    v = nt_cx(v, X1(v), l1);
    v = nt_cx(v, QM(v), l2);  v = nt_cx(v, X1(v), l1);
    v = nt_cx(v, HM(v), l4);  v = nt_cx(v, X2(v), l2);  v = nt_cx(v, X1(v), l1);
    v = nt_cx(v, RM(v), l8);  v = nt_cx(v, S4(v), l4);  v = nt_cx(v, X2(v), l2);  v = nt_cx(v, X1(v), l1);
    v = nt_cx(v, M32(v), l16); v = nt_cx(v, R8(v), l8); v = nt_cx(v, S4(v), l4);  v = nt_cx(v, X2(v), l2); v = nt_cx(v, X1(v), l1);
    v = nt_cx(v, M64(v), l32); v = nt_cx(v, S16(v), l16); v = nt_cx(v, R8(v), l8); v = nt_cx(v, S4(v), l4); v = nt_cx(v, X2(v), l2); v = nt_cx(v, X1(v), l1);
#undef X1
#undef X2
#undef QM
#undef HM
#undef RM
#undef R8
#undef S4
#undef S16
#undef M32
#undef M64
    return v;
}

__device__ __forceinline__ void nt_rank_sort(const int* __restrict__ stage, const int* lstart, int* __restrict__ out)
{
    const int lane = threadIdx.x & 63, wave = threadIdx.x >> 6;
    for (int base = wave * (TT / (NB / 64)); base < (wave + 1) * (TT / (NB / 64)); base += 4) {
        int v[4], s0v[4], Lv[4];
#pragma unroll
        for (int u = 0; u < 4; u++) {
            s0v[u] = lstart[base + u]; Lv[u] = lstart[base + u + 1] - s0v[u];
            v[u] = (lane < Lv[u] && Lv[u] <= 64) ? stage[s0v[u] + lane] : 0x7fffffff;
        }
#pragma unroll
        for (int u = 0; u < 4; u++) v[u] = nt_wave_sort64(v[u], lane);
#pragma unroll
        for (int u = 0; u < 4; u++) if (Lv[u] <= 64 && lane < Lv[u]) out[s0v[u] + lane] = v[u];
    }
    for (int slot = wave; slot < TT; slot += NB / 64) {
        const int s0 = lstart[slot], L = lstart[slot + 1] - s0;
        if (L <= 64) continue;
        for (int c = 0; c < L; c += 64) {
            const int e = c + lane;
            const int mine = e < L ? stage[s0 + e] : 0x7fffffff;
            int rnk = 0, o = 0;
            for (; o + 8 <= L; o += 8) {
                int v[8];
#pragma unroll
                for (int u = 0; u < 8; u++) v[u] = stage[s0 + o + u];
#pragma unroll
                for (int u = 0; u < 8; u++) rnk += (v[u] < mine) ? 1 : 0;
            }
            for (; o < L; o++) rnk += (stage[s0 + o] < mine) ? 1 : 0;
            if (e < L) out[s0 + rnk] = mine;
        }
    }
}

__device__ __forceinline__ void nt_finish_body(int n, int ntt, const int* __restrict__ tile_base, const int2* __restrict__ bins, int* __restrict__ scratch,
                                               int* __restrict__ inv_start, int* __restrict__ inv_src)
{
    __shared__ int cnt[TT], lstart[TT + 1];
    __shared__ int stage_lds[STAGE_CAP];
    const int tt = blockIdx.x;
    const int b0 = tile_base[tt], E = tile_base[tt + 1] - b0;
    const bool in_regs = E <= EPT * NB;
    if (threadIdx.x < TT) cnt[threadIdx.x] = 0;
    int2 r[EPT];
    if (in_regs) {
#pragma unroll
        for (int u = 0; u < EPT; u++) { const int e = u * NB + (int)threadIdx.x; r[u] = e < E ? bins[b0 + e] : make_int2(-1, 0); }
    }
    __syncthreads();
    if (in_regs) {
#pragma unroll
        for (int u = 0; u < EPT; u++) if (r[u].x >= 0) atomicAdd(&cnt[r[u].x], 1);
    } else {
        for (int e = threadIdx.x; e < E; e += NB) atomicAdd(&cnt[bins[b0 + e].x], 1);
    }
    __syncthreads();
    if (threadIdx.x < 64) {
        const int c = cnt[threadIdx.x];
        int incl = c;
        for (int k = 1; k < 64; k <<= 1) { const int v = __shfl_up(incl, k); if ((int)threadIdx.x >= k) incl += v; }
        lstart[threadIdx.x] = incl - c;
        if (threadIdx.x == 63) lstart[TT] = incl;
        const int row = tt * TT + threadIdx.x;
        if (row < n) inv_start[row] = b0 + incl - c;
        if (tt == ntt - 1 && threadIdx.x == 63) inv_start[n] = b0 + incl;
        cnt[threadIdx.x] = 0;
    }
    __syncthreads();
    if (E <= STAGE_CAP) {
        if (in_regs) {
#pragma unroll
            for (int u = 0; u < EPT; u++) if (r[u].x >= 0) stage_lds[lstart[r[u].x] + atomicAdd(&cnt[r[u].x], 1)] = r[u].y;
        } else {
            for (int e = threadIdx.x; e < E; e += NB) { const int2 v = bins[b0 + e]; stage_lds[lstart[v.x] + atomicAdd(&cnt[v.x], 1)] = v.y; }
        }
        __syncthreads();
        nt_rank_sort(stage_lds, lstart, inv_src + b0);
    } else {
        int* stage = scratch + b0;
        for (int e = threadIdx.x; e < E; e += NB) { const int2 v = bins[b0 + e]; stage[lstart[v.x] + atomicAdd(&cnt[v.x], 1)] = v.y; }
        __threadfence_block();
        __syncthreads();
        nt_rank_sort(stage, lstart, inv_src + b0);
    }
}
__global__ __launch_bounds__(NB) void nt_finish_kernel(int n, int ntt, const int* __restrict__ tile_base, const int2* __restrict__ bins, int* __restrict__ scratch,
                                                       int* __restrict__ inv_start, int* __restrict__ inv_src)
{
    nt_finish_body(n, ntt, tile_base, bins, scratch, inv_start, inv_src);
}
__global__ __launch_bounds__(NB) void nt_finish_pair_kernel(int n, int ntt, NtJob a, NtJob b)
{
    const bool fa = blockIdx.y == 0;
    nt_finish_body(n, ntt, fa ? a.tile_base : b.tile_base, fa ? a.bins : b.bins, fa ? a.scratch : b.scratch, fa ? a.inv_start : b.inv_start, fa ? a.inv_src : b.inv_src);
}

template <int LG>
__global__ __launch_bounds__(NB) void grouping_bwd_csr_kernel(unsigned n, const float4* __restrict__ go, const int* __restrict__ order,
                                                              const int* __restrict__ inv_start, const int* __restrict__ inv_src, float4* __restrict__ gi)
{
    constexpr unsigned TPB = NB / LG;
    const unsigned nwg = (n + TPB - 1) / TPB;
    const unsigned g = threadIdx.x / LG, ch = threadIdx.x % LG;
    for (unsigned v = blockIdx.x; v < 8 * cbl_xcd_per(nwg); v += gridDim.x) {
        const unsigned r = cbl_xcd_slot(v, nwg) * TPB + g;
        if (r >= n) continue;
        const int s0 = inv_start[r], s1 = inv_start[r + 1];
        float4 acc = make_float4(0.f, 0.f, 0.f, 0.f);
        int e = s0;
        for (; e + 4 <= s1; e += 4) {
            const int p0 = inv_src[e], p1 = inv_src[e + 1], p2 = inv_src[e + 2], p3 = inv_src[e + 3];
            const float4 a = go[(size_t)p0 * LG + ch], b = go[(size_t)p1 * LG + ch], c = go[(size_t)p2 * LG + ch], d = go[(size_t)p3 * LG + ch];
            acc.x += a.x; acc.y += a.y; acc.z += a.z; acc.w += a.w;
            acc.x += b.x; acc.y += b.y; acc.z += b.z; acc.w += b.w;
            acc.x += c.x; acc.y += c.y; acc.z += c.z; acc.w += c.w;
            acc.x += d.x; acc.y += d.y; acc.z += d.z; acc.w += d.w;
        }
        for (; e < s1; e++) { const float4 a = go[(size_t)inv_src[e] * LG + ch]; acc.x += a.x; acc.y += a.y; acc.z += a.z; acc.w += a.w; }
        const unsigned t = order ? (unsigned)order[r] : r;
        gi[(size_t)t * LG + ch] = acc;
    }
}

__global__ __launch_bounds__(NB) void grouping_bwd_csr_scalar_kernel(unsigned n, int c, const float* __restrict__ go, const int* __restrict__ order,
                                                                     const int* __restrict__ inv_start, const int* __restrict__ inv_src, float* __restrict__ gi)
{
    const unsigned long long total = (unsigned long long)n * (unsigned)c;
    for (unsigned long long e = (unsigned long long)blockIdx.x * NB + threadIdx.x; e < total; e += (unsigned long long)gridDim.x * NB) {
        const unsigned r = (unsigned)(e / (unsigned)c), ch = (unsigned)(e - (unsigned long long)r * (unsigned)c);
        float acc = 0.f;
        for (int k = inv_start[r]; k < inv_start[r + 1]; k++) acc += go[(size_t)inv_src[k] * c + ch];
        gi[(size_t)(order ? order[r] : (int)r) * c + ch] = acc;
    }
}

#include "k4_rows_pipe.h"
static_assert(K4_ROWS_BLOCK == NB, "one block size for the table kernels");

template <bool PAIR_ROWS, bool WEIGHT>
__global__ __launch_bounds__(NB) void scatter_as_gather_kernel(unsigned n, int c, CblFastDiv dv, int wc, float sign, const float* __restrict__ rows,
                                                               const float* __restrict__ w, const int* __restrict__ order,
                                                               const int* __restrict__ inv_start, const int* __restrict__ inv_src, float* __restrict__ gi)
{
    const unsigned lane = threadIdx.x & 63, wave = __builtin_amdgcn_readfirstlane(threadIdx.x >> 6);
    const unsigned nwg = (n + 3) >> 2;
    for (unsigned v = blockIdx.x; v < 8 * cbl_xcd_per(nwg); v += gridDim.x) {
        const unsigned r = cbl_xcd_slot(v, nwg) * 4 + wave;
        if (r >= n) continue;
        const int s0 = inv_start[r], s1 = inv_start[r + 1];
        const unsigned t = order ? (unsigned)order[r] : r;
        for (unsigned ch = lane; ch < (unsigned)c; ch += 64) {
            const unsigned wch = WEIGHT ? ch % (unsigned)wc : 0u;
            auto term = [&](int e) -> float {
                const unsigned p = (unsigned)inv_src[e];
                const float x = rows[(size_t)(PAIR_ROWS ? p : cbl_fastdiv(p, dv)) * c + ch];
                return WEIGHT ? x * w[(size_t)p * wc + wch] : x;
            };
            float acc = 0.f;
            int e = s0;
            for (; e + 8 <= s1; e += 8) {
                float x[8];
#pragma unroll
                for (int u = 0; u < 8; u++) x[u] = term(e + u);
#pragma unroll
                for (int u = 0; u < 8; u++) acc += x[u];
            }
            for (; e < s1; e++) acc += term(e);
            gi[(size_t)t * c + ch] = sign * acc;
        }
    }
}

__global__ __launch_bounds__(256) void rows_sum_kernel(long long total, int ns, int c, const float* __restrict__ go, float* __restrict__ g1)
{
    for (long long e = (long long)blockIdx.x * 256 + threadIdx.x; e < total; e += (long long)gridDim.x * 256) {
        const long long p = e / c; const int ch = (int)(e - p * c);
        float acc = g1[e];
        for (int s = 0; s < ns; s++) acc += go[((size_t)p * ns + s) * c + ch];
        g1[e] = acc;
    }
}

}

CBL_EXPORT size_t cbl_neighbor_transpose_workspace_bytes(int m, int n, int nsample)
{
    if (m < 0 || n < 0 || nsample <= 0) return 0;
    NtWs w;
    return nt_carve(w, nullptr, m, n, nsample);
}

CBL_EXPORT int cbl_neighbor_transpose(int m, int n, int nsample, const int* idx, const int* order_src, const int* order_dst, int* inv_start, int* inv_src,
                                      void* workspace, size_t workspace_bytes, void* stream)
{
    if (m < 0 || n < 0 || nsample <= 0 || !inv_start) return CBL_ERR_BAD_ARG;
    if ((long long)m * nsample > 0x7fffffffLL) return CBL_ERR_BAD_ARG;
    hipStream_t st = cbl_stream(stream);
    const int ntt = nt_tiles(n), nst = nt_src_tiles(m);
    if (m == 0 || n == 0) {
        if (hipMemsetAsync(inv_start, 0, sizeof(int) * (size_t)(n + 1), st) != hipSuccess) return cbl_status();
        return CBL_OK;
    }
    if (!idx || !inv_src || !workspace) return CBL_ERR_BAD_ARG;
    if (ntt > NT_MAX_TILES) return CBL_ERR_UNSUPPORTED;
    NtWs w;
    if (nt_carve(w, (char*)workspace, m, n, nsample) > workspace_bytes) return CBL_ERR_WORKSPACE;
    const CblFastDiv dv = cbl_fastdiv_make((unsigned)nsample);
    const int nzero = ntt + 2;
    hipLaunchKernelGGL(nt_prep_kernel, dim3(cbl_div_up(n > nzero ? n : nzero, NB)), dim3(NB), 0, st, n, nzero, order_dst, w.rank, w.tile_cursor, (int*)nullptr);
    const int* rank = order_dst ? w.rank : nullptr;
    const long long cap = (long long)TS * nsample < ntt ? (long long)TS * nsample : ntt;
    const size_t lds_count = sizeof(int) * (size_t)((ntt + 1) & ~1) + sizeof(int2) * (size_t)cap, lds_bin = sizeof(int) * 2 * (size_t)ntt;
#define CBL_NT(UN_)                                                                                                                                   \
    hipLaunchKernelGGL((nt_count_kernel<UN_>), dim3(nst), dim3(NB), lds_count, st, m, n, nsample, ntt, dv, idx, order_src, rank, w.tile_cursor,       \
                       w.list_cursor, w.tile_list_off, w.tile_list_n, w.lists);                                                                       \
    if (ntt > NT_SCAN_SPLIT) {                                                                                                                        \
        hipLaunchKernelGGL(nt_scan_kernel, dim3(1), dim3(1024), 0, st, ntt, w.tile_cursor, w.tile_base);                                              \
        hipLaunchKernelGGL((nt_bin_kernel<UN_, true>), dim3(nst), dim3(NB), lds_bin, st, m, n, nsample, ntt, dv, idx, order_src, rank, w.tile_cursor, \
                           w.tile_list_off, w.tile_list_n, w.lists, w.tile_base, w.bins);                                                             \
    } else                                                                                                                                            \
        hipLaunchKernelGGL((nt_bin_kernel<UN_, false>), dim3(nst), dim3(NB), lds_bin, st, m, n, nsample, ntt, dv, idx, order_src, rank, w.tile_cursor, \
                           w.tile_list_off, w.tile_list_n, w.lists, w.tile_base, w.bins)
    const int per_thread = (TS * nsample + NB - 1) / NB;
    if (per_thread <= 4) { CBL_NT(4); } else if (per_thread <= 8) { CBL_NT(8); } else { CBL_NT(16); }
#undef CBL_NT
    hipLaunchKernelGGL(nt_finish_kernel, dim3(ntt), dim3(NB), 0, st, n, ntt, w.tile_base, w.bins, w.scratch, inv_start, inv_src);
    return cbl_status();
}

CBL_EXPORT size_t cbl_neighbor_transpose_pair_workspace_bytes(int m, int n, int nsample_a, int nsample_b)
{
    if (m < 0 || n < 0 || nsample_a <= 0 || nsample_b <= 0) return 0;
    NtWs w;
    return nt_carve(w, nullptr, m, n, nsample_a) + nt_carve(w, nullptr, m, n, nsample_b);
}

CBL_EXPORT int cbl_neighbor_transpose_pair(int m, int n, int nsample_a, const int* idx_a, int nsample_b, const int* idx_b, const int* order_src, const int* order_dst,
                                           int* inv_start_a, int* inv_src_a, int* inv_start_b, int* inv_src_b, void* workspace, size_t workspace_bytes, void* stream)
{
    if (m < 0 || n < 0 || nsample_a <= 0 || nsample_b <= 0 || !inv_start_a || !inv_start_b) return CBL_ERR_BAD_ARG;
    if ((long long)m * nsample_a > 0x7fffffffLL || (long long)m * nsample_b > 0x7fffffffLL) return CBL_ERR_BAD_ARG;
    const int ntt = nt_tiles(n), nst = nt_src_tiles(m);
    NtWs wa, wb;
    const size_t bytes_a = nt_carve(wa, (char*)workspace, m, n, nsample_a);
    if (m == 0 || n == 0 || ntt > NT_SCAN_SPLIT) {
        if (m > 0 && n > 0 && (!workspace || bytes_a + nt_carve(wb, nullptr, m, n, nsample_b) > workspace_bytes)) return workspace ? CBL_ERR_WORKSPACE : CBL_ERR_BAD_ARG;
        const int rc = cbl_neighbor_transpose(m, n, nsample_a, idx_a, order_src, order_dst, inv_start_a, inv_src_a, workspace, bytes_a, stream);
        if (rc) return rc;
        return cbl_neighbor_transpose(m, n, nsample_b, idx_b, order_src, order_dst, inv_start_b, inv_src_b, workspace ? (char*)workspace + bytes_a : nullptr,
                                      workspace_bytes > bytes_a ? workspace_bytes - bytes_a : 0, stream);
    }
    if (!idx_a || !idx_b || !inv_src_a || !inv_src_b || !workspace) return CBL_ERR_BAD_ARG;
    if (bytes_a + nt_carve(wb, (char*)workspace + bytes_a, m, n, nsample_b) > workspace_bytes) return CBL_ERR_WORKSPACE;
    hipStream_t st = cbl_stream(stream);
    auto job = [&](const NtWs& w, int ns, const int* idx, int* inv_start, int* inv_src) {
        NtJob j;
        j.ns = ns; j.dv = cbl_fastdiv_make((unsigned)ns); j.idx = idx;
        j.tile_cursor = w.tile_cursor; j.list_cursor = w.list_cursor; j.tile_list_off = w.tile_list_off; j.tile_list_n = w.tile_list_n; j.tile_base = w.tile_base;
        j.lists = w.lists; j.bins = w.bins; j.scratch = w.scratch; j.inv_start = inv_start; j.inv_src = inv_src;
        return j;
    };
    const bool swap = nsample_b > nsample_a;
    const NtJob ja = swap ? job(wb, nsample_b, idx_b, inv_start_b, inv_src_b) : job(wa, nsample_a, idx_a, inv_start_a, inv_src_a);
    const NtJob jb = swap ? job(wa, nsample_a, idx_a, inv_start_a, inv_src_a) : job(wb, nsample_b, idx_b, inv_start_b, inv_src_b);
    const int nzero = ntt + 2;
    hipLaunchKernelGGL(nt_prep_kernel, dim3(cbl_div_up(n > nzero ? n : nzero, NB)), dim3(NB), 0, st, n, nzero, order_dst, wa.rank, wa.tile_cursor, wb.tile_cursor);
    const int* rank = order_dst ? wa.rank : nullptr;
    const int ns_max = ja.ns;
    const long long cap = (long long)TS * ns_max < ntt ? (long long)TS * ns_max : ntt;
    const size_t lds_count = sizeof(int) * (size_t)((ntt + 1) & ~1) + sizeof(int2) * (size_t)cap, lds_bin = sizeof(int) * 2 * (size_t)ntt;
    auto un_of = [](int ns) { const int per_thread = (TS * ns + NB - 1) / NB; return per_thread <= 4 ? 4 : per_thread <= 8 ? 8 : 16; };
    const int una = un_of(ja.ns), unb = un_of(jb.ns);
    const dim3 gsrc(nst, 2), gdst(ntt, 2);
#define CBL_NTP(UA_, UB_)                                                                                                                        \
    { hipLaunchKernelGGL((nt_count_pair_kernel<UA_, UB_>), gsrc, dim3(NB), lds_count, st, m, n, ntt, order_src, rank, ja, jb);                  \
      hipLaunchKernelGGL((nt_bin_pair_kernel<UA_, UB_>), gsrc, dim3(NB), lds_bin, st, m, n, ntt, order_src, rank, ja, jb); }
    if (una == 16 && unb == 16) CBL_NTP(16, 16) else if (una == 16 && unb == 8) CBL_NTP(16, 8) else if (una == 16) CBL_NTP(16, 4)
    else if (una == 8 && unb == 8) CBL_NTP(8, 8) else if (una == 8) CBL_NTP(8, 4) else CBL_NTP(4, 4)
#undef CBL_NTP
    hipLaunchKernelGGL(nt_finish_pair_kernel, gdst, dim3(NB), 0, st, n, ntt, ja, jb);
    return cbl_status();
}

CBL_EXPORT int cbl_grouping_backward_csr(int n, int c, const float* grad_output, const int* order_dst, const int* inv_start, const int* inv_src,
                                         float* grad_input, void* stream)
{
    if (n < 0 || c <= 0) return CBL_ERR_BAD_ARG;
    if (n == 0) return CBL_OK;
    if (!grad_output || !inv_start || !inv_src || !grad_input) return CBL_ERR_BAD_ARG;
    hipStream_t st = cbl_stream(stream);
    const bool v4 = (c % 4 == 0) && cbl_host_aligned16(grad_output) && cbl_host_aligned16(grad_input);
    const int lg = c / 4;
#define CBL_GBC(LG_) { const unsigned nwg = cbl_div_up(n, NB / LG_); unsigned g = cbl_round_up8(nwg); if (g > 256u * 16u) g = 256u * 16u;  \
        hipLaunchKernelGGL((grouping_bwd_csr_kernel<LG_>), dim3(g), dim3(NB), 0, st, (unsigned)n, reinterpret_cast<const float4*>(grad_output), order_dst,  \
                           inv_start, inv_src, reinterpret_cast<float4*>(grad_input)); return cbl_status(); }
    if (v4) switch (lg) {
        case 1: CBL_GBC(1) case 2: CBL_GBC(2) case 4: CBL_GBC(4) case 8: CBL_GBC(8) case 16: CBL_GBC(16) case 32: CBL_GBC(32) case 64: CBL_GBC(64)
        default: break;
    }
#undef CBL_GBC
    hipLaunchKernelGGL(grouping_bwd_csr_scalar_kernel, dim3(cbl_grid_for((long long)n * c, NB)), dim3(NB), 0, st, (unsigned)n, c, grad_output, order_dst, inv_start,
                       inv_src, grad_input);
    return cbl_status();
}

CBL_EXPORT int cbl_grouping_backward_csr_rows(int n, int c, int row_stride, int col_offset, const float* grad_output, const int* order_dst,
                                              const int* inv_start, const int* inv_src, float* grad_input, void* stream)
{
    if (n < 0 || c <= 0 || col_offset < 0 || row_stride < col_offset + c) return CBL_ERR_BAD_ARG;
    if (n == 0) return CBL_OK;
    if (!grad_output || !inv_start || !inv_src || !grad_input) return CBL_ERR_BAD_ARG;
    if (row_stride == c && col_offset == 0) return cbl_grouping_backward_csr(n, c, grad_output, order_dst, inv_start, inv_src, grad_input, stream);
    unsigned g = cbl_round_up8(cbl_div_up(n, 4)); if (g > 256u * 32u) g = 256u * 32u;
    hipLaunchKernelGGL(grouping_bwd_csr_rows_kernel, dim3(g), dim3(NB), 0, cbl_stream(stream), (unsigned)n, c, row_stride, col_offset, grad_output, order_dst,
                       inv_start, inv_src, grad_input);
    return cbl_status();
}

CBL_EXPORT int cbl_weighted_scatter_csr(int n, int nsample, int c, int w_c, const float* rows, const float* weight, const int* order_dst,
                                        const int* inv_start, const int* inv_src, float* grad_input, void* stream)
{
    if (n < 0 || nsample <= 0 || c <= 0 || w_c <= 0) return CBL_ERR_BAD_ARG;
    if (n == 0) return CBL_OK;
    if (!rows || !weight || !inv_start || !inv_src || !grad_input) return CBL_ERR_BAD_ARG;
    unsigned g = cbl_round_up8(cbl_div_up(n, 4)); if (g > 256u * 32u) g = 256u * 32u;
    hipLaunchKernelGGL((scatter_as_gather_kernel<false, true>), dim3(g), dim3(NB), 0, cbl_stream(stream), (unsigned)n, c, cbl_fastdiv_make((unsigned)nsample), w_c, 1.0f,
                       rows, weight, order_dst, inv_start, inv_src, grad_input);
    return cbl_status();
}

CBL_EXPORT int cbl_subtraction_backward_csr(int m, int n2, int nsample, int c, const float* grad_output, const int* order_dst, const int* inv_start,
                                            const int* inv_src, float* grad_input1, float* grad_input2, void* stream)
{
    if (m < 0 || n2 < 0 || nsample <= 0 || c <= 0) return CBL_ERR_BAD_ARG;
    if (!grad_output || !inv_start || !inv_src || !grad_input1 || !grad_input2) return CBL_ERR_BAD_ARG;
    hipStream_t st = cbl_stream(stream);
    if (m > 0)
        hipLaunchKernelGGL(rows_sum_kernel, dim3(cbl_grid_for((long long)m * c, 256)), dim3(256), 0, st, (long long)m * c, nsample, c, grad_output, grad_input1);
    if (n2 > 0) {
        unsigned g = cbl_round_up8(cbl_div_up(n2, 4)); if (g > 256u * 32u) g = 256u * 32u;
        hipLaunchKernelGGL((scatter_as_gather_kernel<true, false>), dim3(g), dim3(NB), 0, st, (unsigned)n2, c, cbl_fastdiv_make(1u), 1, -1.0f,
                           grad_output, nullptr, order_dst, inv_start, inv_src, grad_input2);
    }
    return cbl_status();
}
```

contrastboundary_amd/neighbor_state.py:

```python
import collections
import threading

import torch

_ws_cache = {}


def scratch(cache, key, nbytes, device, grow=1.0):
    if torch.cuda.is_current_stream_capturing():
        return torch.empty(int(nbytes) + 256, dtype=torch.uint8, device=device)
    k = (key, device, torch.cuda.current_stream(device).cuda_stream)
    ws = cache.get(k)
    if ws is None or ws.numel() < nbytes:
        ws = cache[k] = torch.empty(int(nbytes * grow) + 256, dtype=torch.uint8, device=device)
    return ws


def _workspace(nbytes, device):
    if nbytes == 0:
        return None
    return scratch(_ws_cache, "knn", nbytes, device, grow=1.25)


ORDER_MIN_POINTS = 8192
_order_registry = collections.OrderedDict()
_ORDER_REGISTRY_MAX = 16


def _version_of(t):
    try:
        return t._version
    except RuntimeError:
        return -1


def _order_key(points):
    return (points.data_ptr(), points.shape[0], _version_of(points), points.device)


def _order_wanted(points, stream_id):
    if points.shape[0] < ORDER_MIN_POINTS or not use_spatial_order:
        return False
    ent = _order_registry.get(_order_key(points))
    return ent is None or stream_id not in ent


def _order_register(points, order, stream):
    key = _order_key(points)
    ent = _order_registry.setdefault(key, {})
    ent[stream.cuda_stream] = (order, stream)
    _order_registry.move_to_end(key)
    while len(_order_registry) > _ORDER_REGISTRY_MAX:
        _order_registry.popitem(last=False)
    cache = neighbor_cache.active()
    if cache is not None:
        cache.order_keys.append(key)
        cache.order_refs.append(order)


def _order_alias(idx, points):
    ent = _order_registry.get(_order_key(points))
    if ent:
        _order_registry[_order_key(idx)] = ent
        while len(_order_registry) > _ORDER_REGISTRY_MAX:
            _order_registry.popitem(last=False)
        cache = neighbor_cache.active()
        if cache is not None:
            cache.order_keys.append(_order_key(idx))


class streams_ordered_by_caller:
    _streams = collections.Counter()

    def __init__(self, streams):
        self.handles = [s.cuda_stream for s in streams]

    def __enter__(self):
        for h in self.handles:
            streams_ordered_by_caller._streams[h] += 1
        return self

    def __exit__(self, *exc):
        for h in self.handles:
            streams_ordered_by_caller._streams[h] -= 1
            if streams_ordered_by_caller._streams[h] <= 0:
                del streams_ordered_by_caller._streams[h]
        return False

    @staticmethod
    def applies(stream):
        return stream.cuda_stream in streams_ordered_by_caller._streams


def spatial_order(points):
    if not use_spatial_order or points.shape[0] < ORDER_MIN_POINTS:
        return None
    ent = _order_registry.get(_order_key(points))
    if not ent:
        return None
    cur = torch.cuda.current_stream(points.device)
    hit = ent.get(cur.cuda_stream)
    if hit is not None:
        return hit[0]
    order, producer = next(iter(ent.values()))
    if streams_ordered_by_caller.applies(cur):
        return order
    cur.wait_stream(producer)
    order.record_stream(cur)
    ent[cur.cuda_stream] = (order, cur)
    return order


use_spatial_order = True


class natural_order:

    def __enter__(self):
        global use_spatial_order
        self.was = use_spatial_order
        use_spatial_order = False
        return self

    def __exit__(self, *exc):
        global use_spatial_order
        use_spatial_order = self.was
        return False


_deterministic = False


def set_deterministic(on):
    global _deterministic
    was = _deterministic
    _deterministic = bool(on)
    return was


def is_deterministic():
    return _deterministic


class deterministic:

    def __init__(self, on=True):
        self.on = bool(on)

    def __enter__(self):
        self.was = set_deterministic(self.on)
        return self

    def __exit__(self, *exc):
        set_deterministic(self.was)
        return False


_transpose_registry = collections.OrderedDict()
_TRANSPOSE_REGISTRY_MAX = 64


def transpose_lookup(idx):
    if _version_of(idx) < 0:
        return None
    ent = _transpose_registry.get(_order_key(idx))
    if ent is None or ent[0].data_ptr() != idx.data_ptr() or ent[0].shape != idx.shape:
        return None
    _, order, inv_start, inv_src, producer, waited = ent[:6]
    cur = torch.cuda.current_stream(idx.device)
    if producer != cur and cur.cuda_stream not in waited and not streams_ordered_by_caller.applies(cur):
        cur.wait_stream(producer)
        for t in (inv_start, inv_src) + (() if order is None else (order,)):
            t.record_stream(cur)
        waited.add(cur.cuda_stream)
    return order, inv_start, inv_src


def transpose_register(idx, order, inv_start, inv_src):
    if _version_of(idx) < 0:
        return
    key = _order_key(idx)
    cache = neighbor_cache.active()
    _transpose_registry[key] = (idx, order, inv_start, inv_src, torch.cuda.current_stream(idx.device), set(), cache is not None)
    _transpose_registry.move_to_end(key)
    while len(_transpose_registry) > _TRANSPOSE_REGISTRY_MAX:
        _transpose_registry.popitem(last=False)
    if cache is not None:
        cache.transpose_keys.append(key)


def release_unowned_transposes():
    dead = [k for k, ent in _transpose_registry.items() if not ent[6]]
    for k in dead:
        _transpose_registry.pop(k, None)
    return len(dead)



class neighbor_cache:
    _tls = threading.local()

    def __init__(self):
        self.store, self.hits, self.misses = {}, 0, 0
        self.host = {}
        self.hints = {}
        self.wide = {}
        self.derived = 0
        self.order_keys = []
        self.order_refs = []
        self.transpose_keys = []

    def hint(self, xyz, nsample, algo="set", new_xyz=None, offset=None, new_offset=None):
        self.hints[self._geo(xyz, xyz if new_xyz is None else new_xyz)] = (int(nsample), algo)

    def _geo(self, xyz, new_xyz):
        return (xyz.data_ptr(), tuple(xyz.shape), new_xyz.data_ptr(), tuple(new_xyz.shape))

    def __enter__(self):
        self._prev = neighbor_cache.active()
        neighbor_cache._tls.cache = self
        return self

    def __exit__(self, *exc):
        neighbor_cache._tls.cache = self._prev
        if not getattr(self, "keep", False):
            self.store.clear()
            self.host.clear()
            self.wide.clear()
            for key in self.order_keys:
                _order_registry.pop(key, None)
            self.order_keys.clear()
            self.order_refs.clear()
            for key in self.transpose_keys:
                _transpose_registry.pop(key, None)
            self.transpose_keys.clear()
        return False

    @staticmethod
    def active():
        return getattr(neighbor_cache._tls, "cache", None)

    ignore_version = False

    def _key(self, kind, algo, tensors):
        if self.ignore_version:
            return (kind, algo) + tuple((t.data_ptr(), tuple(t.shape)) for t in tensors)
        return (kind, algo) + tuple((t.data_ptr(), tuple(t.shape), _version_of(t)) for t in tensors)

    def _host_key(self, o):
        return (o.data_ptr(), tuple(o.shape)) if self.ignore_version else (o.data_ptr(), tuple(o.shape), _version_of(o))

    def _deliver(self, entry):
        outs, _keys, event, stream = entry
        if event is not None:
            cur = torch.cuda.current_stream(outs[0].device)
            if stream != cur:
                cur.wait_event(event)
                for t in outs:
                    t.record_stream(cur)
        return outs

    def _stamp(self, outs, keys):
        dev = outs[0].device
# ... 54 lines not shown
```

contrastboundary_amd/pointops.py:

```python
import ctypes

import torch
from torch.autograd import Function

from . import _lib

_c_int = ctypes.c_int


def _req(t, dtype, name, dim=None):
    if not isinstance(t, torch.Tensor):
        raise TypeError(f"{name}: expected a torch.Tensor, got {type(t)}")
    if not t.is_cuda:
        raise _lib.CblError(f"{name}: must live on the GPU (got {t.device}); there is no CPU fallback")
    if t.dtype != dtype:
        raise TypeError(f"{name}: expected {dtype}, got {t.dtype}")
    if not t.is_contiguous():
        raise ValueError(f"{name}: must be contiguous")
    if dim is not None and t.dim() != dim:
        raise ValueError(f"{name}: expected {dim} dims, got shape {tuple(t.shape)}")
    return t


def _as_int(v):
# ... 8 lines not shown
def _furthestsampling_raw(xyz, offset, new_offset, n_max, m, cert_in=None, want_cert=False):
    n, b = xyz.shape[0], offset.shape[0]
    idx = torch.zeros(m, dtype=torch.int32, device=xyz.device)
    tmp = torch.full((n,), 1e10, dtype=torch.float32, device=xyz.device)
    L = _lib.lib()
    need = L.cbl_furthestsampling_workspace_bytes(_c_int(b), _c_int(n), _c_int(n_max))
    ws = _workspace(need, xyz.device)
    if want_cert or cert_in is not None:
        cert = torch.empty(b, dtype=torch.int32, device=xyz.device)
        rc = L.cbl_furthestsampling_chain(_c_int(b), _c_int(n), _c_int(n_max), _lib.ptr(xyz), _lib.ptr(offset), _lib.ptr(new_offset), _lib.ptr(tmp),
                                          _lib.ptr(idx), _lib.ptr(cert_in), _lib.ptr(cert), _lib.ptr(ws),
                                          ctypes.c_size_t(ws.numel() if ws is not None else 0), _lib.stream_of(xyz))
        _lib.check(rc, "cbl_furthestsampling_chain")
        return idx, cert
    rc = L.cbl_furthestsampling_ws(_c_int(b), _c_int(n), _c_int(n_max), _lib.ptr(xyz), _lib.ptr(offset), _lib.ptr(new_offset),
                                   _lib.ptr(tmp), _lib.ptr(idx), _lib.ptr(ws), ctypes.c_size_t(ws.numel() if ws is not None else 0),
                                   _lib.stream_of(xyz))
    _lib.check(rc, "cbl_furthestsampling_ws")
    return idx


class FurthestSampling(Function):
    @staticmethod
    def forward(ctx, xyz, offset, new_offset):
        _req(xyz, torch.float32, "xyz", 2); _req(offset, torch.int32, "offset", 1); _req(new_offset, torch.int32, "new_offset", 1)
        b = offset.shape[0]
        off_h = offset.cpu()
        lens = torch.diff(off_h, prepend=off_h.new_zeros(1))
        n_max = int(lens.max().item()) if b > 0 else 0
        m = int(new_offset[b - 1].item()) if b > 0 else 0
        return _furthestsampling_raw(xyz, offset, new_offset, n_max, m)


furthestsampling = FurthestSampling.apply

_tie_policy = "reference"


def set_knn_tie_policy(policy):
    global _tie_policy
    if policy not in ("reference", "set", "anytie"):
        raise ValueError(policy)
    prev, _tie_policy = _tie_policy, policy
    return prev


fps_prefix_chain = True


def fps_downsample(p, o, stride):
    cache = neighbor_cache.active()
    if cache is not None:
        hit = cache.lookup_fps(stride, (p, o))
        if hit is not None:
            return hit
    ends = host_offsets(o)
    lens = [e - s for s, e in zip([0] + ends[:-1], ends)]
    new_ends, run = [], 0
    for l in lens:
        run += l // stride
        new_ends.append(run)
    staged = torch.tensor(new_ends, dtype=torch.int32).pin_memory()
    new_o = staged.to(o.device, non_blocking=True)
    tag = getattr(p, "_fps_certificate", None)
    cert_in = tag[0] if (fps_prefix_chain and tag is not None and tag[1] == p._version and tag[2] is o and tag[3] == o._version) else None
    idx, cert = _furthestsampling_raw(p, o, new_o, max(lens) if lens else 0, run, cert_in=cert_in, want_cert=True)
    new_p = p[idx.long(), :]
    new_p._fps_certificate = (cert, new_p._version, new_o, new_o._version)
    if cache is not None:
        cache.host[cache._host_key(new_o)] = (new_ends, new_o, staged)
        cache.insert_fps(stride, (p, o), new_p, new_o, idx)
    return new_p, new_o, idx


def knnquery_raw(nsample, xyz, new_xyz, offset, new_offset, algo="auto"):
    nsample = _as_int(nsample)
    if new_xyz is None:
        new_xyz = xyz
    _req(xyz, torch.float32, "xyz", 2); _req(new_xyz, torch.float32, "new_xyz", 2)
    _req(offset, torch.int32, "offset", 1); _req(new_offset, torch.int32, "new_offset", 1)
    if not 1 <= nsample <= 1024:
        raise ValueError(f"nsample={nsample} outside [1, 1024] (knnquery_cuda_kernel.cu:89)")
    if xyz.shape[1] != 3 or new_xyz.shape[1] != 3:
        raise ValueError("xyz / new_xyz: expected (n, 3)")
    if algo == "auto" and _tie_policy != "reference":
        algo = _tie_policy
    cache = neighbor_cache.active()
    if cache is not None:
        tensors = (xyz, new_xyz, offset, new_offset)
        hit = cache.lookup(nsample, algo, tensors)
        if hit is not None:
            return hit
        if algo in ("auto", "set"):
            wide = cache.wider(nsample, tensors)
            if wide is None:
                h = cache.hints.get(cache._geo(xyz, new_xyz))
                if h is not None and h[0] > nsample and h[0] <= 64:
                    ev = None
                    if getattr(cache, "record_events", False):
                        ev = torch.cuda.Event()
                        ev.record(torch.cuda.current_stream(xyz.device))
                    both = _knnquery_nested(h[0], h[1], nsample, algo, xyz, new_xyz, offset, new_offset, ev)
                    if both is not None:
                        wi, wd, idx, dist2 = both
                        cache.insert(h[0], h[1], tensors, wi, wd, event=ev)
                        cache.insert(nsample, algo, tensors, idx, dist2)
                        cache.derived += 1
                        return idx, dist2
                    wi, wd = _knnquery_uncached(h[0], xyz, new_xyz, offset, new_offset, h[1])
                    cache.insert(h[0], h[1], tensors, wi, wd)
                    wide = (h[0], wi, wd)
            if wide is not None:
                idx, dist2 = knn_prefix(nsample, wide[0], wide[1], wide[2], xyz, new_xyz, offset, new_offset, algo)
                cache.insert(nsample, algo, tensors, idx, dist2)
                cache.derived += 1
                if new_xyz is xyz or (new_xyz.data_ptr() == xyz.data_ptr() and new_xyz.shape == xyz.shape):
                    _order_alias(idx, xyz)
                return idx, dist2
        idx, dist2 = _knnquery_uncached(nsample, xyz, new_xyz, offset, new_offset, algo)
        cache.insert(nsample, algo, tensors, idx, dist2)
        return idx, dist2
    return _knnquery_uncached(nsample, xyz, new_xyz, offset, new_offset, algo)


def knn_prefix(nsample, nsample_wide, idx_wide, dist2_wide, xyz, new_xyz, offset, new_offset, algo="auto"):
    if algo not in ("auto", "set"):
        raise ValueError("knn_prefix: algo must be 'auto' or 'set'")
    n, m, b = xyz.shape[0], new_xyz.shape[0], offset.shape[0]
    idx = torch.empty((m, nsample), dtype=torch.int32, device=xyz.device)
    dist2 = torch.empty((m, nsample), dtype=torch.float32, device=xyz.device)
    L = _lib.lib()
    ws = _workspace(max(L.cbl_knnquery_prefix_workspace_bytes(_c_int(m)), 1), xyz.device)
    _lib.check(L.cbl_knnquery_prefix(_c_int(b), _c_int(n), _c_int(m), _c_int(nsample_wide), _c_int(nsample), _lib.ptr(xyz), _lib.ptr(new_xyz),
                                     _lib.ptr(offset), _lib.ptr(new_offset), _lib.ptr(idx_wide), _lib.ptr(dist2_wide), _lib.ptr(idx), _lib.ptr(dist2),
                                     _c_int(1 if algo == "set" else 0), _lib.ptr(ws), ctypes.c_size_t(ws.numel()), _lib.stream_of(xyz)),
               "cbl_knnquery_prefix")
    return idx, dist2


def _knnquery_nested(nsample_wide, algo_wide, nsample, algo, xyz, new_xyz, offset, new_offset, event=None):
    if algo_wide not in ("auto", "set", "anytie", "grid") or algo not in ("auto", "set"):
        return None
    n, m, b = xyz.shape[0], new_xyz.shape[0], offset.shape[0]
    L = _lib.lib()
    need = L.cbl_knnquery_workspace_bytes(_c_int(b), _c_int(n), _c_int(m), _c_int(nsample_wide))
    if need == 0 or nsample_wide > 64:
        return None
    dev = xyz.device
    wi = torch.empty((m, nsample_wide), dtype=torch.int32, device=dev); wd = torch.empty((m, nsample_wide), dtype=torch.float32, device=dev)
    idx = torch.empty((m, nsample), dtype=torch.int32, device=dev); dist2 = torch.empty((m, nsample), dtype=torch.float32, device=dev)
    ws = _workspace(need, dev)
    cur = torch.cuda.current_stream(dev)
    self_search = new_xyz is xyz or (new_xyz.data_ptr() == xyz.data_ptr() and m == n)
    order = torch.empty(n, dtype=torch.int32, device=dev) if (self_search and _order_wanted(xyz, cur.cuda_stream)) else None
    pw = 1 if algo_wide == "set" else 2 if algo_wide == "anytie" else 0
    rc = L.cbl_knnquery_nested(_c_int(b), _c_int(n), _c_int(m), _c_int(nsample_wide), _c_int(pw), _c_int(nsample), _c_int(1 if algo == "set" else 0),
                               _lib.ptr(xyz), _lib.ptr(new_xyz), _lib.ptr(offset), _lib.ptr(new_offset), _lib.ptr(wi), _lib.ptr(wd), _lib.ptr(idx),
                               _lib.ptr(dist2), _lib.ptr(order), ctypes.c_void_p(event.cuda_event if event is not None else 0),
                               _lib.ptr(ws), ctypes.c_size_t(ws.numel()), _lib.stream_of(xyz))
    if rc == _lib.ERR_UNSUPPORTED:
        return None
    _lib.check(rc, "cbl_knnquery_nested")
    if order is not None:
        _order_register(xyz, order, cur)
    if self_search and n >= ORDER_MIN_POINTS and neighbor_state.use_spatial_order:
        _order_alias(wi, xyz); _order_alias(idx, xyz)
    return wi, wd, idx, dist2


def _knnquery_uncached(nsample, xyz, new_xyz, offset, new_offset, algo):
    n, m, b = xyz.shape[0], new_xyz.shape[0], offset.shape[0]
    idx = torch.empty((m, nsample), dtype=torch.int32, device=xyz.device)
    dist2 = torch.empty((m, nsample), dtype=torch.float32, device=xyz.device)
    L = _lib.lib()
    st = _lib.stream_of(xyz)
    args = (_c_int(b), _c_int(n), _c_int(m), _c_int(nsample), _lib.ptr(xyz), _lib.ptr(new_xyz), _lib.ptr(offset),
            _lib.ptr(new_offset), _lib.ptr(idx), _lib.ptr(dist2))
    if algo == "exact":
        _lib.check(L.cbl_knnquery_exact(*args, st), "cbl_knnquery_exact")
    else:
        need = L.cbl_knnquery_workspace_bytes(_c_int(b), _c_int(n), _c_int(m), _c_int(nsample))
        if algo == "grid" and need == 0:
            raise _lib.CblError("grid KNN not available for this problem shape")
        ws = _workspace(need, xyz.device)
        cur = torch.cuda.current_stream(xyz.device)
        self_search = new_xyz is xyz or (new_xyz.data_ptr() == xyz.data_ptr() and m == n)
        if self_search and need and nsample <= 64 and _order_wanted(xyz, cur.cuda_stream):
            order = torch.empty(n, dtype=torch.int32, device=xyz.device)
            policy = 1 if algo == "set" else 2 if algo == "anytie" else 0
            rc = L.cbl_knnquery_ordered(*args, _c_int(policy), _lib.ptr(order), _lib.ptr(ws), ctypes.c_size_t(ws.numel()), st)
            if rc == 0:
                _order_register(xyz, order, cur)
                _order_alias(idx, xyz)
                return idx, dist2
            if rc != _lib.ERR_UNSUPPORTED:
                _lib.check(rc, "cbl_knnquery_ordered")
        fn = L.cbl_knnquery_set if algo == "set" else L.cbl_knnquery_anytie if algo == "anytie" else L.cbl_knnquery
        _lib.check(fn(*args, _lib.ptr(ws), ctypes.c_size_t(ws.numel() if ws is not None else 0), st), "cbl_knnquery")
        if self_search and n >= ORDER_MIN_POINTS and neighbor_state.use_spatial_order:
            _order_alias(idx, xyz)
    return idx, dist2


def knn_block_candidates(nsample, xyz, offset, algo="set"):
    n, b = xyz.shape[0], offset.shape[0]
    L = _lib.lib()
    need = L.cbl_knnquery_workspace_bytes(_c_int(b), _c_int(n), _c_int(n), _c_int(nsample))
    if need == 0:
        raise _lib.CblError("knn_block_candidates: this shape does not take the grid search")
    _knnquery_uncached(nsample, xyz, xyz, offset, offset, algo)
    ws = _workspace(need, xyz.device)
    count = torch.empty(n, dtype=torch.int32, device=xyz.device)
    _lib.check(L.cbl_knn_grid_block_candidates(_c_int(b), _c_int(n), _c_int(nsample), _lib.ptr(offset), _lib.ptr(count), _lib.ptr(ws),
                                               ctypes.c_size_t(ws.numel()), _lib.stream_of(xyz)), "cbl_knn_grid_block_candidates")
    return count


TRANSPOSE_MIN_PAIRS = 1 << 16


def _build_table(pairs):
    return neighbor_state.is_deterministic() or pairs >= TRANSPOSE_MIN_PAIRS


def neighbor_transpose(idx, n, build=True, companion=None):
    _req(idx, torch.int32, "idx", 2)
    hit = neighbor_state.transpose_lookup(idx)
    if hit is not None or not build:
        return hit
    m, nsample = idx.shape
    order = spatial_order(idx) if m == n else None
    L = _lib.lib()
    inv_start = torch.empty(n + 1, dtype=torch.int32, device=idx.device)
    inv_src = torch.empty(max(m * nsample, 1), dtype=torch.int32, device=idx.device)
    if companion is not None and companion.dim() == 2 and companion.shape[0] == m and companion.dtype == torch.int32 and companion.device == idx.device \
            and companion.data_ptr() != idx.data_ptr() and neighbor_state.transpose_lookup(companion) is None:
        ns2 = companion.shape[1]
        inv_start2 = torch.empty(n + 1, dtype=torch.int32, device=idx.device)
        inv_src2 = torch.empty(max(m * ns2, 1), dtype=torch.int32, device=idx.device)
        ws = _workspace(max(L.cbl_neighbor_transpose_pair_workspace_bytes(_c_int(m), _c_int(n), _c_int(nsample), _c_int(ns2)), 1), idx.device)
        rc = L.cbl_neighbor_transpose_pair(_c_int(m), _c_int(n), _c_int(nsample), _lib.ptr(idx), _c_int(ns2), _lib.ptr(companion), _lib.ptr(order), _lib.ptr(order),
                                           _lib.ptr(inv_start), _lib.ptr(inv_src), _lib.ptr(inv_start2), _lib.ptr(inv_src2), _lib.ptr(ws), ctypes.c_size_t(ws.numel()),
                                           _lib.stream_of(idx))
        if rc == _lib.ERR_UNSUPPORTED:
            return None
        _lib.check(rc, "cbl_neighbor_transpose_pair")
        neighbor_state.transpose_register(idx, order, inv_start, inv_src)
        neighbor_state.transpose_register(companion, order, inv_start2, inv_src2)
        return order, inv_start, inv_src
    ws = _workspace(max(L.cbl_neighbor_transpose_workspace_bytes(_c_int(m), _c_int(n), _c_int(nsample)), 1), idx.device)
    rc = L.cbl_neighbor_transpose(_c_int(m), _c_int(n), _c_int(nsample), _lib.ptr(idx), _lib.ptr(order), _lib.ptr(order), _lib.ptr(inv_start),
                                  _lib.ptr(inv_src), _lib.ptr(ws), ctypes.c_size_t(ws.numel()), _lib.stream_of(idx))
    if rc == _lib.ERR_UNSUPPORTED:
        return None
    _lib.check(rc, "cbl_neighbor_transpose")
    neighbor_state.transpose_register(idx, order, inv_start, inv_src)
    return order, inv_start, inv_src


def _scatter_rows(grad_rows, idx, n, col0=0, c=None):
    m, nsample, width = grad_rows.shape
    c = width - col0 if c is None else c
    L = _lib.lib()
    tr = neighbor_transpose(idx, n, build=_build_table(m * nsample))
    if tr is not None:
        order, inv_start, inv_src = tr
        grad_in = torch.empty((n, c), dtype=torch.float32, device=grad_rows.device)
        _lib.check(L.cbl_grouping_backward_csr_rows(_c_int(n), _c_int(c), _c_int(width), _c_int(col0), _lib.ptr(grad_rows), _lib.ptr(order),
                                                    _lib.ptr(inv_start), _lib.ptr(inv_src), _lib.ptr(grad_in), _lib.stream_of(grad_rows)),
                   "cbl_grouping_backward_csr_rows")
        return grad_in
    if col0 or c != width:
        grad_rows = grad_rows[..., col0:col0 + c].contiguous()
    grad_in = torch.zeros((n, c), dtype=torch.float32, device=grad_rows.device)
    _lib.check(L.cbl_grouping_backward(_c_int(m), _c_int(nsample), _c_int(c), _lib.ptr(grad_rows), _lib.ptr(idx), _lib.ptr(grad_in),
                                       _lib.stream_of(grad_rows)), "cbl_grouping_backward")
    return grad_in


class KNNQuery(Function):
    @staticmethod
    def forward(ctx, nsample, xyz, new_xyz, offset, new_offset):
        idx, dist2 = knnquery_raw(nsample, xyz, new_xyz, offset, new_offset)
        if neighbor_cache.active() is not None:
            idx = idx.view(idx.shape)
        ctx.mark_non_differentiable(idx)
        return idx, torch.sqrt(dist2)

    @staticmethod
    def backward(ctx, *grads):
        return None, None, None, None, None


knnquery = KNNQuery.apply


def knn_indices(nsample, xyz, new_xyz, offset, new_offset):
    idx, _ = knnquery_raw(nsample, xyz, new_xyz if new_xyz is not None else xyz, offset, new_offset)
    if neighbor_cache.active() is not None:
        idx = idx.view(idx.shape)
    return idx


class Grouping(Function):
    @staticmethod
    def forward(ctx, input, idx):
        _req(input, torch.float32, "input", 2); _req(idx, torch.int32, "idx", 2)
        m, nsample, n, c = idx.shape[0], idx.shape[1], input.shape[0], input.shape[1]
        output = torch.empty((m, nsample, c), dtype=torch.float32, device=input.device)
        order = spatial_order(idx)
        _lib.check(_lib.lib().cbl_grouping_forward_ordered(_c_int(m), _c_int(nsample), _c_int(c), _lib.ptr(input), _lib.ptr(idx), _lib.ptr(order),
                                                           _lib.ptr(output), _lib.stream_of(input)), "cbl_grouping_forward")
        ctx.n = n
        ctx.save_for_backward(idx)
        return output

    @staticmethod
    def backward(ctx, grad_output):
        idx, = ctx.saved_tensors
        grad_output = grad_output.contiguous()
        return _scatter_rows(grad_output, idx, ctx.n), None


grouping = Grouping.apply


class _QueryAndGroup(Function):

    @staticmethod
    def forward(ctx, xyz, new_xyz, feat, idx, use_xyz):
        m, nsample = idx.shape
        c = feat.shape[1]
        oc = c + (3 if use_xyz else 0)
        out = torch.empty((m, nsample, oc), dtype=torch.float32, device=feat.device)
        order = spatial_order(new_xyz) if use_xyz else None
        _lib.check(_lib.lib().cbl_queryandgroup_ordered(_c_int(m), _c_int(nsample), _c_int(c), _c_int(1 if use_xyz else 0), _lib.ptr(xyz),
                                                        _lib.ptr(new_xyz), _lib.ptr(feat), _lib.ptr(idx), _lib.ptr(order), _lib.ptr(out),
                                                        _lib.stream_of(feat)), "cbl_queryandgroup")
        ctx.save_for_backward(idx)
        ctx.dims = (xyz.shape[0], feat.shape[0], c, use_xyz)
        return out

    @staticmethod
    def backward(ctx, grad_out):
        idx, = ctx.saved_tensors
        n_xyz, n_feat, c, use_xyz = ctx.dims
        m, nsample = idx.shape
        L = _lib.lib()
        g_xyz = g_new = g_feat = None
        grad_out = grad_out.contiguous()
        if ctx.needs_input_grad[2]:
            g_feat = _scatter_rows(grad_out, idx, n_feat, 3 if use_xyz else 0, c)
        if use_xyz and (ctx.needs_input_grad[0] or ctx.needs_input_grad[1]):
            if ctx.needs_input_grad[0]:
                g_xyz = _scatter_rows(grad_out, idx, n_xyz, 0, 3)
            if ctx.needs_input_grad[1]:
                g_new = -grad_out[..., :3].sum(1)
        return g_xyz, g_new, g_feat, None, None


def queryandgroup(nsample, xyz, new_xyz, feat, idx, offset, new_offset, use_xyz=True):
    if new_xyz is None:
        new_xyz = xyz
    _req(xyz, torch.float32, "xyz", 2); _req(new_xyz, torch.float32, "new_xyz", 2); _req(feat, torch.float32, "feat", 2)
    if idx is None:
        idx = knn_indices(nsample, xyz, new_xyz, offset, new_offset)
    _req(idx, torch.int32, "idx", 2)
    return _QueryAndGroup.apply(xyz, new_xyz, feat, idx, bool(use_xyz))


class Subtraction(Function):
    @staticmethod
    def forward(ctx, input1, input2, idx):
        _req(input1, torch.float32, "input1", 2); _req(input2, torch.float32, "input2", 2); _req(idx, torch.int32, "idx", 2)
        n, c = input1.shape
        nsample = idx.shape[-1]
        output = torch.empty((n, nsample, c), dtype=torch.float32, device=input1.device)
        _lib.check(_lib.lib().cbl_subtraction_forward_ordered(_c_int(n), _c_int(nsample), _c_int(c), _lib.ptr(input1), _lib.ptr(input2),
                                                              _lib.ptr(idx), _lib.ptr(spatial_order(idx)), _lib.ptr(output), _lib.stream_of(input1)),
                   "cbl_subtraction_forward")
        ctx.save_for_backward(idx)
        ctx.n2 = input2.shape[0]
        return output

    @staticmethod
    def backward(ctx, grad_output):
        idx, = ctx.saved_tensors
        grad_output = grad_output.contiguous()
        n, nsample, c = grad_output.shape
        g1 = torch.zeros((n, c), dtype=torch.float32, device=grad_output.device)
        tr = neighbor_transpose(idx, ctx.n2, build=_build_table(n * nsample))
        if tr is not None:
            order, inv_start, inv_src = tr
            g2 = torch.empty((ctx.n2, c), dtype=torch.float32, device=grad_output.device)
            _lib.check(_lib.lib().cbl_subtraction_backward_csr(_c_int(n), _c_int(ctx.n2), _c_int(nsample), _c_int(c), _lib.ptr(grad_output), _lib.ptr(order),
                                                               _lib.ptr(inv_start), _lib.ptr(inv_src), _lib.ptr(g1), _lib.ptr(g2),
                                                               _lib.stream_of(grad_output)), "cbl_subtraction_backward_csr")
            return g1, g2, None
        g2 = torch.zeros((ctx.n2, c), dtype=torch.float32, device=grad_output.device)
        _lib.check(_lib.lib().cbl_subtraction_backward(_c_int(n), _c_int(nsample), _c_int(c), _lib.ptr(idx), _lib.ptr(grad_output),
                                                       _lib.ptr(g1), _lib.ptr(g2), _lib.stream_of(grad_output)), "cbl_subtraction_backward")
        return g1, g2, None


subtraction = Subtraction.apply
# ... 130 lines not shown
```

include/cbl_amd.h:

```cpp
#ifndef CBL_AMD_H
#define CBL_AMD_H

#include <stddef.h>
#include <stdint.h>

#ifdef __cplusplus
extern "C" {
#endif

#define CBL_OK               0
#define CBL_ERR_BAD_ARG     (-1)
#define CBL_ERR_WORKSPACE   (-2)
#define CBL_ERR_UNSUPPORTED (-3)

#define CBL_KNN_MAX_NSAMPLE 1024
#define CBL_CONTRAST_PAIRS_MAX_D 4096

const char* cbl_version(void);
int         cbl_device_arch_ok(void);


int cbl_knnquery(int b, int n, int m, int nsample,
                 const float* xyz, const float* new_xyz,
                 const int* offset, const int* new_offset,
                 int* idx, float* dist2,
                 void* workspace, size_t workspace_bytes, void* stream);
size_t cbl_knnquery_workspace_bytes(int b, int n, int m, int nsample);

int cbl_knnquery_set(int b, int n, int m, int nsample,
                     const float* xyz, const float* new_xyz,
                     const int* offset, const int* new_offset,
                     int* idx, float* dist2,
                     void* workspace, size_t workspace_bytes, void* stream);
int cbl_knnquery_anytie(int b, int n, int m, int nsample,
                        const float* xyz, const float* new_xyz,
                        const int* offset, const int* new_offset,
                        int* idx, float* dist2,
                        void* workspace, size_t workspace_bytes, void* stream);

int cbl_knnquery_ordered(int b, int n, int m, int nsample,
                         const float* xyz, const float* new_xyz,
                         const int* offset, const int* new_offset,
                         int* idx, float* dist2, int tie_policy, int* cell_order,
                         void* workspace, size_t workspace_bytes, void* stream);

int cbl_knn_grid_block_candidates(int b, int n, int nsample, const int* offset, int* count, void* workspace, size_t workspace_bytes, void* stream);

size_t cbl_knnquery_prefix_workspace_bytes(int m);
int cbl_knnquery_prefix(int b, int n, int m, int nsample_wide, int nsample,
                        const float* xyz, const float* new_xyz, const int* offset, const int* new_offset,
                        const int* idx_wide, const float* dist2_wide, int* idx, float* dist2, int tie_policy,
                        void* workspace, size_t workspace_bytes, void* stream);

int cbl_knnquery_nested(int b, int n, int m, int nsample_wide, int tie_policy_wide, int nsample, int tie_policy,
                        const float* xyz, const float* new_xyz, const int* offset, const int* new_offset,
                        int* idx_wide, float* dist2_wide, int* idx, float* dist2, int* cell_order, void* event_after_wide,
                        void* workspace, size_t workspace_bytes, void* stream);

int cbl_knnquery_exact(int b, int n, int m, int nsample,
                       const float* xyz, const float* new_xyz,
                       const int* offset, const int* new_offset,
                       int* idx, float* dist2, void* stream);

int cbl_furthestsampling(int b, int n_max, const float* xyz, const int* offset, const int* new_offset,
                         float* tmp, int* idx, void* stream);
size_t cbl_furthestsampling_workspace_bytes(int b, int n, int n_max);
int cbl_furthestsampling_ws(int b, int n, int n_max, const float* xyz, const int* offset, const int* new_offset,
                            float* tmp, int* idx, void* workspace, size_t workspace_bytes, void* stream);
int cbl_furthestsampling_chain(int b, int n, int n_max, const float* xyz, const int* offset, const int* new_offset, float* tmp, int* idx,
                               const int* cert_in, int* cert_out, void* workspace, size_t workspace_bytes, void* stream);

int cbl_grouping_forward(int m, int nsample, int c, const float* input, const int* idx, float* output, void* stream);
int cbl_grouping_forward_ordered(int m, int nsample, int c, const float* input, const int* idx, const int* order, float* output, void* stream);
int cbl_grouping_backward(int m, int nsample, int c, const float* grad_output, const int* idx, float* grad_input, void* stream);

size_t cbl_neighbor_transpose_workspace_bytes(int m, int n, int nsample);
int cbl_neighbor_transpose(int m, int n, int nsample, const int* idx, const int* order_src, const int* order_dst, int* inv_start, int* inv_src,
                           void* workspace, size_t workspace_bytes, void* stream);
size_t cbl_neighbor_transpose_pair_workspace_bytes(int m, int n, int nsample_a, int nsample_b);
int cbl_neighbor_transpose_pair(int m, int n, int nsample_a, const int* idx_a, int nsample_b, const int* idx_b, const int* order_src, const int* order_dst,
                                int* inv_start_a, int* inv_src_a, int* inv_start_b, int* inv_src_b, void* workspace, size_t workspace_bytes, void* stream);
int cbl_grouping_backward_csr(int n, int c, const float* grad_output, const int* order_dst, const int* inv_start, const int* inv_src,
                              float* grad_input, void* stream);
int cbl_grouping_backward_csr_rows(int n, int c, int row_stride, int col_offset, const float* grad_output, const int* order_dst,
                                   const int* inv_start, const int* inv_src, float* grad_input, void* stream);
int cbl_weighted_scatter_csr(int n, int nsample, int c, int w_c, const float* rows, const float* weight, const int* order_dst, const int* inv_start,
                             const int* inv_src, float* grad_input, void* stream);
int cbl_subtraction_backward_csr(int m, int n2, int nsample, int c, const float* grad_output, const int* order_dst, const int* inv_start,
                                 const int* inv_src, float* grad_input1, float* grad_input2, void* stream);

int cbl_interpolation_forward(int n, int c, int k, const float* input, const int* idx, const float* weight, float* output, void* stream);
int cbl_interpolation_backward(int n, int c, int k, const float* grad_output, const int* idx, const float* weight, float* grad_input, void* stream);

int cbl_subtraction_forward(int n, int nsample, int c, const float* input1, const float* input2, const int* idx, float* output, void* stream);
int cbl_subtraction_forward_ordered(int n, int nsample, int c, const float* input1, const float* input2, const int* idx, const int* order,
                                    float* output, void* stream);
int cbl_subtraction_backward(int n, int nsample, int c, const int* idx, const float* grad_output, float* grad_input1, float* grad_input2, void* stream);

int cbl_aggregation_forward(int n, int nsample, int c, int w_c, const float* input, const float* position, const float* weight, const int* idx, float* output, void* stream);
int cbl_aggregation_forward_ordered(int n, int nsample, int c, int w_c, const float* input, const float* position, const float* weight, const int* idx,
                                    const int* order, float* output, void* stream);
int cbl_aggregation_backward(int n, int nsample, int c, int w_c, const float* input, const float* position, const float* weight, const int* idx, const float* grad_output, float* grad_input, float* grad_position, float* grad_weight, void* stream);


int cbl_queryandgroup(int m, int nsample, int c, int use_xyz, const float* xyz, const float* new_xyz, const float* feat, const int* idx, float* out, void* stream);
int cbl_queryandgroup_ordered(int m, int nsample, int c, int use_xyz, const float* xyz, const float* new_xyz, const float* feat, const int* idx,
                              const int* order, float* out, void* stream);

int cbl_interpolation_weights(int n, int k, const float* dist2, float* weight, float* dist, void* stream);



int cbl_subscene_label(int m, int kr, int num_classes, const long long* target, const int* neighbor_idx, float* out, void* stream);

int cbl_label_argmax(int m, int num_classes, const float* labels, int* amax, void* stream);

int cbl_point_contrast_forward(int m, int nsample, int d, const float* features, const int* amax, const int* neighbor_idx,
                               float temperature, float weight, float* per_point, int* point_mask, float* stats, float* loss, void* stream);
int cbl_point_contrast_backward(int m, int nsample, int d, const float* features, const int* amax, const int* neighbor_idx,
                                float temperature, float weight, const float* stats, const float* grad_loss, float* grad_features, void* stream);

int cbl_point_contrast_forward_grad(int m, int nsample, int d, const float* features, const int* amax, const int* neighbor_idx,
                                    float temperature, float weight, float* per_point, int* point_mask, float* stats, float* loss,
                                    float* grad_unit, void* stream);
int cbl_point_contrast_forward_l64(int m, int nsample, int d, const float* features, const long long* labels, const int* neighbor_idx,
                                   float temperature, float weight, float* per_point, int* point_mask, float* stats, float* loss, void* stream);
int cbl_point_contrast_forward_grad_l64(int m, int nsample, int d, const float* features, const long long* labels, const int* neighbor_idx,
                                        float temperature, float weight, float* per_point, int* point_mask, float* stats, float* loss,
                                        float* grad_unit, void* stream);
int cbl_tf_contrast_forward_grad(int m, int n_valid, int nsample, int d, const float* features, const int* labels, const int* neighbors,
                                 float temperature, float weight, float* per_point, int* point_mask, float* stats, float* loss,
                                 float* grad_unit, void* stream);
int cbl_tf_contrast_forward_kl(int m, int n_valid, int nsample, int d, const float* features, const float* soft_labels, int num_classes,
                               float kl_threshold, const int* neighbors, float temperature, float weight, float* per_point, int* point_mask,
                               float* stats, float* loss, void* stream);
int cbl_tf_contrast_forward_grad_kl(int m, int n_valid, int nsample, int d, const float* features, const float* soft_labels, int num_classes,
                                    float kl_threshold, const int* neighbors, float temperature, float weight, float* per_point, int* point_mask,
                                    float* stats, float* loss, float* grad_unit, void* stream);
int cbl_contrast_grad_scale(long long total, const float* grad_unit, const float* stats, const float* grad_loss, float weight,
                            float* grad_features, void* stream);

int cbl_contrast_pairs_forward(int m, int n_valid, int flags, int nsample, int d, const float* features, const void* labels, int num_classes,
                               float kl_threshold, const int* neighbor_idx, const int* order, float temperature, float weight,
                               float* per_point, int* point_mask, float* stats, float* loss, float* coef, float* grad_own, void* stream);
#define CBL_ROLE_LABEL 0
#define CBL_ROLE_POS 1
#define CBL_ROLE_NEG 2
#define CBL_ROLE_NEG_REJECT 3
int cbl_contrast_pairs_forward_samples(int m, int n_valid, int flags, int nsample, int d, const float* features, const void* labels, int num_classes,
                                       float kl_threshold, const int* sample_idx, const unsigned char* roles, const unsigned char* sample_valid,
                                       const int* order, float temperature, float weight, float* per_point, int* point_mask, float* stats,
                                       float* loss, float* coef, float* grad_own, void* stream);
int cbl_contrast_pairs_backward(int m, int nsample, int d, const float* features, const float* coef, const float* grad_own, const int* order,
                                const int* inv_start, const int* inv_src, const float* stats, const float* grad_loss, float weight,
                                float* grad_features, void* stream);

int cbl_contrast_pairs_backward_atomic(int m, int n_valid, int nsample, int d, const float* features, const float* coef, const float* grad_own,
                                       const int* neighbor_idx, const float* stats, const float* grad_loss, float weight,
                                       float* grad_features, void* stream);

int cbl_tf_contrast_forward(int m, int n_valid, int nsample, int d, const float* features, const int* labels, const int* neighbors,
                            float temperature, float weight, float* per_point, int* point_mask, float* stats, float* loss, void* stream);
int cbl_tf_contrast_backward(int m, int n_valid, int nsample, int d, const float* features, const int* labels, const int* neighbors,
                             float temperature, float weight, const float* stats, const float* grad_loss, float* grad_features, void* stream);
int cbl_tf_scene_label(int m, int n_valid, int k, int num_classes, const long long* point_labels, const int* scene_neighbor, int by_valid, float* out, void* stream);

int cbl_boundary_mask(int n, int k, const long long* labels, const int* neighbor_idx, unsigned char* bound, unsigned char* plain, int* cnt, void* stream);

int cbl_cumulate_probs(int n, int num_classes, int m, const long long* inds, const float* pred, float smooth, int mode, float* probs,
                       int* scratch_n, void* stream);

int cbl_boundary_iou(int n, int k, int num_classes, long long ignore_label, const long long* pred, const long long* labels,
                     const int* neighbor_idx, unsigned long long* hist, void* stream);


int cbl_kpconv_forward(int n, int n0, int K, int C, int KP, const float* query_points, const float* support_points, const int* neighbors_indices,
                       const float* features, const float* kernel_points, const float* kernel_weights, float extent, int influence, int closest,
                       float* out, void* stream);
int cbl_kpconv_forward_ordered(int n, int n0, int K, int C, int KP, const float* query_points, const float* support_points, const int* neighbors_indices,
                               const float* features, const float* kernel_points, const float* kernel_weights, float extent, int influence, int closest,
                               const int* order, float* out, void* stream);
int cbl_kpconv_backward(int n, int n0, int K, int C, int KP, const float* query_points, const float* support_points, const int* neighbors_indices,
                        const float* features, const float* kernel_points, const float* kernel_weights, float extent, int influence, int closest,
                        const float* grad_out, float* grad_features, float* grad_kernel_weights, void* stream);

size_t cbl_kpconv_backward_csr_workspace_bytes(int n0, int C, int KP);
int cbl_kpconv_backward_csr(int n, int n0, int K, int C, int KP, const float* query_points, const float* support_points, const float* features,
                            const float* kernel_points, const float* kernel_weights, float extent, int influence, int closest,
                            const float* grad_out, const int* order_dst, const int* inv_start, const int* inv_src,
                            float* grad_features, float* grad_kernel_weights, void* workspace, size_t workspace_bytes, void* stream);

int cbl_index_max(long long total, const int* idx, int* out_max, void* stream);
int cbl_adaptive_weight_forward(int n, int n0, int K, int C, const float* query_points, const float* support_points, const int* neighbors_indices,
                                const float* features, float radius, const float* fc_weight, const float* fc_bias, const int* padding_num,
                                int reduction_mean, float* out, void* stream);
int cbl_adaptive_weight_forward_ordered(int n, int n0, int K, int C, const float* query_points, const float* support_points, const int* neighbors_indices,
                                        const float* features, float radius, const float* fc_weight, const float* fc_bias, const int* padding_num,
                                        int reduction_mean, const int* order, float* out, void* stream);
int cbl_adaptive_weight_backward(int n, int n0, int K, int C, const float* query_points, const float* support_points, const int* neighbors_indices,
                                 const float* features, float radius, const float* fc_weight, const float* fc_bias, const int* padding_num,
                                 int reduction_mean, const float* grad_out, float* grad_features, float* grad_fc_weight, float* grad_fc_bias, void* stream);

size_t cbl_adaptive_weight_backward_csr_workspace_bytes(int n, int n0, int C);
int cbl_adaptive_weight_backward_csr(int n, int n0, int K, int C, const float* query_points, const float* support_points, const int* neighbors_indices,
                                     const float* features, float radius, const float* fc_weight, const float* fc_bias, const int* padding_num,
                                     int reduction_mean, const float* grad_out, const int* order_dst, const int* inv_start, const int* inv_src,
                                     float* grad_features, float* grad_fc_weight, float* grad_fc_bias, void* workspace, size_t workspace_bytes, void* stream);

size_t cbl_adaptive_weight_general_workspace_bytes(int n, int n0, int K, int C, int M);
int cbl_adaptive_weight_general_forward(int n, int n0, int K, int C, int M, const float* query_points, const float* support_points,
                                        const int* neighbors_indices, const float* features, const float* center_term, const float* neighbor_term,
                                        const float* w_pos, const float* bias, float radius, int softmax, int reduction, const int* padding_num,
                                        float* out, void* workspace, size_t workspace_bytes, void* stream);
int cbl_adaptive_weight_general_backward_csr(int n, int n0, int K, int C, int M, const float* query_points, const float* support_points,
                                             const int* neighbors_indices, const float* features, const float* center_term, const float* neighbor_term,
                                             const float* w_pos, const float* bias, float radius, int softmax, int reduction, const int* padding_num,
                                             const float* out, const float* grad_out, const int* order_dst, const int* inv_start, const int* inv_src,
                                             float* grad_features_value, float* grad_center, float* grad_neighbor, float* grad_w_pos, float* grad_bias,
                                             void* workspace, size_t workspace_bytes, void* stream);

size_t cbl_adaptive_weight_mlp_workspace_bytes(int n, int n0, int K, int C, int M, int layers);
int cbl_adaptive_weight_mlp_forward(int n, int n0, int K, int C, int M, const float* query_points, const float* support_points,
                                    const int* neighbors_indices, const float* features, const float* center_term, const float* neighbor_term,
                                    const float* w_pos, const float* bias, int layers, const float* hidden_w, const float* hidden_b, int activation,
                                    float radius, int softmax, int reduction, const int* padding_num, float* out, void* workspace,
                                    size_t workspace_bytes, void* stream);
int cbl_adaptive_weight_mlp_backward_csr(int n, int n0, int K, int C, int M, const float* query_points, const float* support_points,
                                         const int* neighbors_indices, const float* features, const float* center_term, const float* neighbor_term,
                                         const float* w_pos, const float* bias, int layers, const float* hidden_w, const float* hidden_b, int activation,
                                         float radius, int softmax, int reduction, const int* padding_num, const float* out, const float* grad_out,
                                         const int* order_dst, const int* inv_start, const int* inv_src, float* grad_features_value, float* grad_center,
                                         float* grad_neighbor, float* grad_w_pos, float* grad_bias, float* grad_hidden_w, float* grad_hidden_b,
                                         void* workspace, size_t workspace_bytes, void* stream);

// ... 242 lines not shown
```

Before: 148.3 million.

## Emit inverse cell rank from KNN grid build and bin neighbor transpose per tile

The KNN grid scatter and canonical-order kernels now also write each point's rank in the spatial order, and new ranked entry points pass this buffer through to Python and on to the neighbor transpose. The transpose drops its own rank-computation pass and replaces the list-based staging with fixed-capacity per-tile bins plus an overflow region. This targets the separate rank pass and the extra list staging in the transpose, in exchange for extra global writes during grid build and a more involved workspace layout that must handle overflow.

Result: faster. 151.6 million, median of 6 (+2.3%).

```diff
diff --git a/contrastboundary_amd/csrc/knn_dispatch.hip b/contrastboundary_amd/csrc/knn_dispatch.hip
--- a/contrastboundary_amd/csrc/knn_dispatch.hip
+++ b/contrastboundary_amd/csrc/knn_dispatch.hip
@@ -2,7 +2,7 @@
 
 size_t cbl_knn_grid_workspace_bytes(int b, int n, int m, int nsample);
 int cbl_knn_grid_launch(int b, int n, int m, int nsample, const float* xyz, const float* new_xyz, const int* offset,
-                        const int* new_offset, int* idx, float* dist2, void* ws, size_t ws_bytes, int set_exact, hipStream_t st, int* order_out, CblKnnNarrow* narrow);
+                        const int* new_offset, int* idx, float* dist2, void* ws, size_t ws_bytes, int set_exact, hipStream_t st, int* order_out, CblKnnNarrow* narrow, int* rank_out);
 
 size_t cbl_knn_select_workspace_bytes(int b, int n, int m, int nsample);
 int cbl_knn_select_launch(int b, int n, int m, int nsample, const float* xyz, const float* new_xyz, const int* offset, const int* new_offset,
@@ -16,14 +16,14 @@
 
 static int knnquery_impl(int b, int n, int m, int nsample, const float* xyz, const float* new_xyz,
                          const int* offset, const int* new_offset, int* idx, float* dist2,
-                         void* workspace, size_t workspace_bytes, int set_exact, void* stream, int* order_out = nullptr, CblKnnNarrow* narrow = nullptr)
+                         void* workspace, size_t workspace_bytes, int set_exact, void* stream, int* order_out = nullptr, CblKnnNarrow* narrow = nullptr, int* rank_out = nullptr)
 {
     if (b <= 0 || n < 0 || m < 0 || nsample <= 0 || nsample > CBL_KNN_MAX_NSAMPLE) return CBL_ERR_BAD_ARG;
     if (m == 0) return CBL_OK;
     if (!xyz || !new_xyz || !offset || !new_offset || !idx || !dist2) return CBL_ERR_BAD_ARG;
     const size_t need = cbl_knn_grid_workspace_bytes(b, n, m, nsample);
     if (need > 0 && workspace && workspace_bytes >= need)
-        return cbl_knn_grid_launch(b, n, m, nsample, xyz, new_xyz, offset, new_offset, idx, dist2, workspace, workspace_bytes, set_exact, cbl_stream(stream), order_out, narrow);
+        return cbl_knn_grid_launch(b, n, m, nsample, xyz, new_xyz, offset, new_offset, idx, dist2, workspace, workspace_bytes, set_exact, cbl_stream(stream), order_out, narrow, rank_out);
     if (order_out) return CBL_ERR_UNSUPPORTED;
     const size_t need_sel = cbl_knn_select_workspace_bytes(b, n, m, nsample);
     if (need_sel > 0 && workspace && workspace_bytes >= need_sel)
@@ -58,6 +58,14 @@
 {
     if (tie_policy < 0 || tie_policy > 2 || !cell_order) return CBL_ERR_BAD_ARG;
     return knnquery_impl(b, n, m, nsample, xyz, new_xyz, offset, new_offset, idx, dist2, workspace, workspace_bytes, tie_policy, stream, cell_order);
+}
+
+CBL_EXPORT int cbl_knnquery_ordered_ranked(int b, int n, int m, int nsample, const float* xyz, const float* new_xyz,
+                                           const int* offset, const int* new_offset, int* idx, float* dist2, int tie_policy, int* cell_order, int* cell_rank,
+                                           void* workspace, size_t workspace_bytes, void* stream)
+{
+    if (tie_policy < 0 || tie_policy > 2 || !cell_order || !cell_rank) return CBL_ERR_BAD_ARG;
+    return knnquery_impl(b, n, m, nsample, xyz, new_xyz, offset, new_offset, idx, dist2, workspace, workspace_bytes, tie_policy, stream, cell_order, nullptr, cell_rank);
 }
 
 int cbl_knn_block_candidates_launch(int b, int n, const int* offset, void* ws, int* count, hipStream_t st);
@@ -142,16 +150,16 @@
     return cbl_status();
 }
 
-CBL_EXPORT int cbl_knnquery_nested(int b, int n, int m, int nsample_wide, int tie_policy_wide, int nsample, int tie_policy,
-                                   const float* xyz, const float* new_xyz, const int* offset, const int* new_offset,
-                                   int* idx_wide, float* dist2_wide, int* idx, float* dist2, int* cell_order, void* event_after_wide,
-                                   void* workspace, size_t workspace_bytes, void* stream)
+static int knnquery_nested_impl(int b, int n, int m, int nsample_wide, int tie_policy_wide, int nsample, int tie_policy,
+                               const float* xyz, const float* new_xyz, const int* offset, const int* new_offset,
+                               int* idx_wide, float* dist2_wide, int* idx, float* dist2, int* cell_order, int* cell_rank, void* event_after_wide,
+                               void* workspace, size_t workspace_bytes, void* stream)
 {
     if (nsample <= 0 || nsample >= nsample_wide || tie_policy < 0 || tie_policy > 1 || tie_policy_wide < 0 || tie_policy_wide > 2 || !idx || !dist2) return CBL_ERR_BAD_ARG;
     const size_t need = cbl_knn_grid_workspace_bytes(b, n, m, nsample_wide);
     if (need == 0 || !workspace || workspace_bytes < need) return CBL_ERR_UNSUPPORTED;
     CblKnnNarrow narrow{nsample, tie_policy, idx, dist2, false, true};
-    int rc = knnquery_impl(b, n, m, nsample_wide, xyz, new_xyz, offset, new_offset, idx_wide, dist2_wide, workspace, workspace_bytes, tie_policy_wide, stream, cell_order, &narrow);
+    int rc = knnquery_impl(b, n, m, nsample_wide, xyz, new_xyz, offset, new_offset, idx_wide, dist2_wide, workspace, workspace_bytes, tie_policy_wide, stream, cell_order, &narrow, cell_rank);
     if (rc || m == 0) return rc;
     hipStream_t st = cbl_stream(stream);
     int *worklist, *worklist2, *counter; const void *grids, *sorted; const int* cell_start;
@@ -170,6 +178,25 @@
         if (rc) return rc;
     }
     return cbl_knn_exact_worklist(b, m, nsample, xyz, new_xyz, offset, new_offset, idx, dist2, worklist, counter, m, st, grids, cell_start, sorted);
+}
+
+CBL_EXPORT int cbl_knnquery_nested(int b, int n, int m, int nsample_wide, int tie_policy_wide, int nsample, int tie_policy,
+                                   const float* xyz, const float* new_xyz, const int* offset, const int* new_offset,
+                                   int* idx_wide, float* dist2_wide, int* idx, float* dist2, int* cell_order, void* event_after_wide,
+                                   void* workspace, size_t workspace_bytes, void* stream)
+{
+    return knnquery_nested_impl(b, n, m, nsample_wide, tie_policy_wide, nsample, tie_policy, xyz, new_xyz, offset, new_offset, idx_wide, dist2_wide, idx, dist2,
+                                cell_order, nullptr, event_after_wide, workspace, workspace_bytes, stream);
+}
+
+CBL_EXPORT int cbl_knnquery_nested_ranked(int b, int n, int m, int nsample_wide, int tie_policy_wide, int nsample, int tie_policy,
+                                          const float* xyz, const float* new_xyz, const int* offset, const int* new_offset,
+                                          int* idx_wide, float* dist2_wide, int* idx, float* dist2, int* cell_order, int* cell_rank, void* event_after_wide,
+                                          void* workspace, size_t workspace_bytes, void* stream)
+{
+    if (cell_rank && !cell_order) return CBL_ERR_BAD_ARG;
+    return knnquery_nested_impl(b, n, m, nsample_wide, tie_policy_wide, nsample, tie_policy, xyz, new_xyz, offset, new_offset, idx_wide, dist2_wide, idx, dist2,
+                                cell_order, cell_rank, event_after_wide, workspace, workspace_bytes, stream);
 }
 
 CBL_EXPORT size_t cbl_knnquery_prefix_workspace_bytes(int m) { return m < 0 ? 0 : sizeof(int) * ((size_t)m + 64); }
diff --git a/contrastboundary_amd/csrc/knn_grid.hip b/contrastboundary_amd/csrc/knn_grid.hip
--- a/contrastboundary_amd/csrc/knn_grid.hip
+++ b/contrastboundary_amd/csrc/knn_grid.hip
@@ -177,7 +177,7 @@
 
 __global__ __launch_bounds__(256) void grid_scatter_kernel(int n, int total, int ntiles, const float* __restrict__ xyz, const int* __restrict__ pt_cell,
                                                            const int* __restrict__ tile_sum, int* __restrict__ cell_start_local, int* __restrict__ cell_start,
-                                                           int* __restrict__ cell_count, float4* __restrict__ sorted, int* __restrict__ order_out)
+                                                           int* __restrict__ cell_count, float4* __restrict__ sorted, int* __restrict__ order_out, int* __restrict__ rank_out)
 {
     extern __shared__ int tile_lds[];
     int* tile_pre = tile_lds + ntiles;
@@ -193,11 +193,12 @@
         const int pos = cell_start_local[cell] + tile_pre[cell / SCAN_TILE] + atomicSub(cell_count + cell, 1) - 1;
         sorted[pos] = make_float4(xyz[3 * i], xyz[3 * i + 1], xyz[3 * i + 2], __int_as_float(i));
         if (order_out) order_out[pos] = i;
+        if (rank_out) rank_out[i] = pos;
     }
 }
 
 __device__ __forceinline__ void grid_order_canon_body(int n, const int* __restrict__ pt_cell, const int* __restrict__ cell_start,
-                                                      const float4* __restrict__ sorted, int* __restrict__ order, int block, int nblocks)
+                                                      const float4* __restrict__ sorted, int* __restrict__ order, int* __restrict__ rank_of, int block, int nblocks)
 {
     for (int i = block * 256 + threadIdx.x; i < n; i += nblocks * 256) {
         const int cell = pt_cell[i];
@@ -212,14 +213,15 @@
             for (int u = 0; u < 8; u++) rank += (j + u < e && v[u] < i) ? 1 : 0;
         }
         order[s + rank] = i;
+        if (rank_of) rank_of[i] = s + rank;
     }
 }
 __global__ __launch_bounds__(256) void grid_order_canon_kernel(int n, const int* __restrict__ pt_cell, const int* __restrict__ cell_start,
-                                                               const float4* __restrict__ sorted, int* __restrict__ order)
-{
-    grid_order_canon_body(n, pt_cell, cell_start, sorted, order, blockIdx.x, gridDim.x);
-}
-struct CblCanon { int blocks, n; const int* pt_cell; int* order; };
+                                                               const float4* __restrict__ sorted, int* __restrict__ order, int* __restrict__ rank_of)
+{
+    grid_order_canon_body(n, pt_cell, cell_start, sorted, order, rank_of, blockIdx.x, gridDim.x);
+}
+struct CblCanon { int blocks, n; const int* pt_cell; int* order; int* rank_of; };
 
 template <int G> __device__ __forceinline__ float dpp_shr1_f(float v);
 template <int G> __device__ __forceinline__ int dpp_shr1_i(int v);
@@ -432,7 +434,7 @@
 {
     __shared__ float2 slots[4][64];
     if ((int)blockIdx.x < canon.blocks) {
-        grid_order_canon_body(canon.n, canon.pt_cell, cell_start, sorted, canon.order, blockIdx.x, canon.blocks);
+        grid_order_canon_body(canon.n, canon.pt_cell, cell_start, sorted, canon.order, canon.rank_of, blockIdx.x, canon.blocks);
         return;
     }
     const int lane = threadIdx.x & 63, wv = threadIdx.x >> 6;
@@ -773,7 +775,7 @@
     for (int i = i0; i < total; i += gridDim.x * 256) cell_count[i] = 0;
 }
 
-int cbl_grid_build(int b, int n, float pts_per_cell, const float* xyz, const int* offset, void* ws, hipStream_t st, int* order_out = nullptr, bool canon_later = false)
+int cbl_grid_build(int b, int n, float pts_per_cell, const float* xyz, const int* offset, void* ws, hipStream_t st, int* order_out = nullptr, bool canon_later = false, int* rank_out = nullptr)
 {
     Workspace w = carve(ws, b, n, 0);
     const int total = w.ncap + 1, ntiles = (total + SCAN_TILE - 1) / SCAN_TILE;
@@ -782,9 +784,9 @@
     hipLaunchKernelGGL(grid_count_kernel, dim3(cbl_grid_for(n, 256)), dim3(256), 0, st, b, n, pts_per_cell, xyz, offset, w.bbox, w.grids, w.pt_cell, w.cell_count);
     hipLaunchKernelGGL(grid_scan_tiles_kernel, dim3(ntiles), dim3(256), 0, st, total, w.cell_count, w.cell_local, w.tile_sum);
     hipLaunchKernelGGL(grid_scatter_kernel, dim3(cbl_grid_for(n, 256)), dim3(256), 2 * sizeof(int) * (size_t)ntiles, st, n, total, ntiles, xyz, w.pt_cell,
-                       w.tile_sum, w.cell_local, w.cell_start, w.cell_count, w.sorted, order_out);
+                       w.tile_sum, w.cell_local, w.cell_start, w.cell_count, w.sorted, order_out, order_out ? rank_out : nullptr);
     if (order_out && !canon_later)
-        hipLaunchKernelGGL(grid_order_canon_kernel, dim3(cbl_grid_for(n, 256)), dim3(256), 0, st, n, w.pt_cell, w.cell_start, w.sorted, order_out);
+        hipLaunchKernelGGL(grid_order_canon_kernel, dim3(cbl_grid_for(n, 256)), dim3(256), 0, st, n, w.pt_cell, w.cell_start, w.sorted, order_out, rank_out);
     return cbl_status();
 }
 
@@ -832,17 +834,17 @@
 
 int cbl_knn_grid_launch(int b, int n, int m, int nsample, const float* xyz, const float* new_xyz, const int* offset,
                         const int* new_offset, int* idx, float* dist2, void* ws, size_t ws_bytes, int set_exact, hipStream_t st, int* order_out,
-                        CblKnnNarrow* narrow)
+                        CblKnnNarrow* narrow, int* rank_out)
 {
     Workspace w = carve(ws, b, n, m);
     if (ws_bytes < w.bytes) return CBL_ERR_WORKSPACE;
     static const float fill = [] { const char* e = getenv("CBL_KNN_CELL_FILL"); const float v = e ? (float)atof(e) : 0.f; return (v > 0.05f && v < 4.f) ? v : 0.33f; }();
     const bool wave_search = nsample > 16;
-    int rc = cbl_grid_build(b, n, fill * (float)(nsample < 4 ? 4 : nsample), xyz, offset, ws, st, order_out, wave_search);
+    int rc = cbl_grid_build(b, n, fill * (float)(nsample < 4 ? 4 : nsample), xyz, offset, ws, st, order_out, wave_search, rank_out);
     if (rc) return rc;
     const bool self = (new_xyz == xyz) && (m == n);
     if (wave_search) {
-        CblCanon canon = {0, n, w.pt_cell, order_out};
+        CblCanon canon = {0, n, w.pt_cell, order_out, rank_out};
         if (order_out) canon.blocks = (int)cbl_grid_for(n, 256);
         const dim3 grid(cbl_div_up(m, 4) + canon.blocks), block(256);
         const int ks = narrow ? narrow->nsample : 0;
diff --git a/contrastboundary_amd/csrc/neighbor_transpose.hip b/contrastboundary_amd/csrc/neighbor_transpose.hip
--- a/contrastboundary_amd/csrc/neighbor_transpose.hip
+++ b/contrastboundary_amd/csrc/neighbor_transpose.hip
@@ -12,45 +12,51 @@
 
 
 struct NtWs {
+    int* tile_cursor;
+    int* ovf_cursor;
     int* rank;
-    int* tile_cursor;
-    int* list_cursor;
-    int* tile_list_off;
-    int* tile_list_n;
     int* tile_base;
-    int2* lists;
     int2* bins;
+    int2* ovf;
     int* scratch;
+    int cap;
 };
 
 static size_t nt_align(size_t v) { return (v + 255) & ~(size_t)255; }
 static int nt_tiles(int n) { return (n + TT - 1) / TT; }
 static int nt_src_tiles(int m) { return (m + TS - 1) / TS; }
 
+static int nt_cap(int m, int n, int nsample)
+{
+    const long long P = (long long)m * nsample, ntt = nt_tiles(n) > 0 ? nt_tiles(n) : 1;
+    long long mean = (P + ntt - 1) / ntt;
+    if (mean < (long long)TT * nsample) mean = (long long)TT * nsample;
+    const long long cap = 2 * mean < P ? 2 * mean : P;
+    return (int)(cap > 0 ? cap : 1);
+}
+
 static size_t nt_carve(NtWs& w, char* base, int m, int n, int nsample)
 {
     const size_t P = (size_t)m * nsample;
-    const int ntt = nt_tiles(n), nst = nt_src_tiles(m);
+    const int ntt = nt_tiles(n);
     size_t off = 0;
     auto take = [&](size_t bytes) { char* p = base ? base + off : nullptr; off += nt_align(bytes); return p; };
+    w.cap = nt_cap(m, n, nsample);
+    w.tile_cursor = (int*)take(sizeof(int) * 2 * (size_t)(ntt + 2));
+    w.ovf_cursor = w.tile_cursor ? w.tile_cursor + ntt + 1 : nullptr;
     w.rank = (int*)take(sizeof(int) * (size_t)(n > 0 ? n : 1));
-    w.tile_cursor = (int*)take(sizeof(int) * (size_t)(ntt + 2));
-    w.list_cursor = w.tile_cursor ? w.tile_cursor + ntt + 1 : nullptr;
-    w.tile_list_off = (int*)take(sizeof(int) * (size_t)(nst + 1));
-    w.tile_list_n = (int*)take(sizeof(int) * (size_t)(nst + 1));
     w.tile_base = (int*)take(sizeof(int) * (size_t)(ntt + 2));
-    w.lists = (int2*)take(sizeof(int2) * (P ? P : 1));
-    w.bins = (int2*)take(sizeof(int2) * (P ? P : 1));
+    w.bins = (int2*)take(sizeof(int2) * ((size_t)ntt * (size_t)w.cap + 1));
+    w.ovf = (int2*)take(sizeof(int2) * (P ? P : 1));
     w.scratch = (int*)take(sizeof(int) * (P ? P : 1));
     return off;
 }
 
-__global__ __launch_bounds__(NB) void nt_prep_kernel(int n, int nzero, const int* __restrict__ order, int* __restrict__ rank, int* __restrict__ zero,
-                                                     int* __restrict__ zero2)
+__global__ __launch_bounds__(NB) void nt_prep_kernel(int n, int nzero, const int* __restrict__ order, int* __restrict__ rank, int* __restrict__ zero)
 {
     const int i = blockIdx.x * NB + threadIdx.x;
-    if (order && i < n) rank[order[i]] = i;
-    if (i < nzero) { zero[i] = 0; if (zero2) zero2[i] = 0; }
+    if (i < n) rank[order[i]] = i;
+    if (i < nzero) zero[i] = 0;
 }
 
 template <int UN> struct NtPairs { unsigned p[UN]; int r[UN]; };
@@ -76,59 +82,63 @@
 }
 
 struct NtJob {
-    int ns; CblFastDiv dv; const int* idx;
-    int *tile_cursor, *list_cursor, *tile_list_off, *tile_list_n, *tile_base; int2 *lists, *bins; int* scratch;
+    int ns, cap; CblFastDiv dv; const int* idx;
+    int *tile_cursor, *ovf_cursor, *tile_base; int2 *bins, *ovf; int* scratch;
     int *inv_start, *inv_src;
 };
 
 template <int UN>
-__device__ __forceinline__ void nt_count_body(int* lds, int m, int n, int ns, int ntt, CblFastDiv dv, const int* __restrict__ idx, const int* __restrict__ order_src,
-                                              const int* __restrict__ rank, int* __restrict__ tile_cursor, int* __restrict__ list_cursor,
-                                              int* __restrict__ tile_list_off, int* __restrict__ tile_list_n, int2* __restrict__ lists)
-{
-    int* hist = lds;
-    int2* mine = reinterpret_cast<int2*>(lds + ((ntt + 1) & ~1));
-    __shared__ int nmine, gbase, src_ids[TS];
+__device__ __forceinline__ void nt_scatter_body(int* lds, int m, int n, int ntt, const int* __restrict__ order_src, const int* __restrict__ rank, const NtJob& j)
+{
+    int* where = lds;
+    int* ovfb = lds + ntt;
+    __shared__ int src_ids[TS];
     const int st = blockIdx.x;
     const int nsrc = min(TS, m - st * TS);
     if ((int)threadIdx.x < TS) src_ids[threadIdx.x] = (int)threadIdx.x < nsrc ? (order_src ? order_src[st * TS + threadIdx.x] : st * TS + (int)threadIdx.x) : 0;
-    for (int e = threadIdx.x; e < ntt; e += NB) hist[e] = 0;
-    if (threadIdx.x == 0) nmine = 0;
-    __syncthreads();
-    const unsigned total = (unsigned)nsrc * (unsigned)ns;
+    const unsigned total = (unsigned)nsrc * (unsigned)j.ns;
+    const int cap = j.cap;
     for (unsigned base = 0; base < total; base += UN * NB) {
+        for (int e = threadIdx.x; e < ntt; e += NB) where[e] = 0;
+        __syncthreads();
         NtPairs<UN> q;
-        nt_load_pairs<UN>(q, base, total, n, ns, dv, src_ids, idx, rank);
-#pragma unroll
-        for (int u = 0; u < UN; u++) if (q.r[u] >= 0) atomicAdd(&hist[q.r[u] / TT], 1);
-    }
-    __syncthreads();
-    for (int tt = threadIdx.x; tt < ntt; tt += NB) {
-        const int c = hist[tt];
-        if (c) {
-            const int off = atomicAdd(&tile_cursor[tt], c);
-            mine[atomicAdd(&nmine, 1)] = make_int2(tt, off);
+        int pos[UN];
+        nt_load_pairs<UN>(q, base, total, n, j.ns, j.dv, src_ids, j.idx, rank);
+#pragma unroll
+        for (int u = 0; u < UN; u++) pos[u] = q.r[u] >= 0 ? atomicAdd(&where[q.r[u] / TT], 1) : 0;
+        __syncthreads();
+        for (int tt = threadIdx.x; tt < ntt; tt += NB) {
+            const int c = where[tt];
+            if (c) {
+                const int off = atomicAdd(&j.tile_cursor[tt], c);
+                where[tt] = off;
+                const int over = off + c - max(off, cap);
+                if (over > 0) ovfb[tt] = atomicAdd(j.ovf_cursor, over);
+            }
         }
-    }
-    __syncthreads();
-    if (threadIdx.x == 0) { gbase = st * TS * ns; tile_list_off[st] = gbase; tile_list_n[st] = nmine; }
-    __syncthreads();
-    for (int e = threadIdx.x; e < nmine; e += NB) lists[gbase + e] = mine[e];
+        __syncthreads();
+#pragma unroll
+        for (int u = 0; u < UN; u++)
+            if (q.r[u] >= 0) {
+                const int tt = q.r[u] / TT, off = where[tt], at = off + pos[u];
+                if (at < cap) j.bins[(size_t)tt * (size_t)cap + at] = make_int2(q.r[u] & (TT - 1), (int)q.p[u]);
+                else j.ovf[ovfb[tt] + (at - max(off, cap))] = make_int2(q.r[u], (int)q.p[u]);
+            }
+        if (base + UN * NB < total) __syncthreads();
+    }
 }
 template <int UN>
-__global__ __launch_bounds__(NB) void nt_count_kernel(int m, int n, int ns, int ntt, CblFastDiv dv, const int* __restrict__ idx, const int* __restrict__ order_src,
-                                                      const int* __restrict__ rank, int* __restrict__ tile_cursor, int* __restrict__ list_cursor,
-                                                      int* __restrict__ tile_list_off, int* __restrict__ tile_list_n, int2* __restrict__ lists)
+__global__ __launch_bounds__(NB) void nt_scatter_kernel(int m, int n, int ntt, const int* __restrict__ order_src, const int* __restrict__ rank, NtJob a)
 {
     extern __shared__ int lds[];
-    nt_count_body<UN>(lds, m, n, ns, ntt, dv, idx, order_src, rank, tile_cursor, list_cursor, tile_list_off, tile_list_n, lists);
+    nt_scatter_body<UN>(lds, m, n, ntt, order_src, rank, a);
 }
 template <int UNA, int UNB>
-__global__ __launch_bounds__(NB) void nt_count_pair_kernel(int m, int n, int ntt, const int* __restrict__ order_src, const int* __restrict__ rank, NtJob a, NtJob b)
+__global__ __launch_bounds__(NB) void nt_scatter_pair_kernel(int m, int n, int ntt, const int* __restrict__ order_src, const int* __restrict__ rank, NtJob a, NtJob b)
 {
     extern __shared__ int lds[];
-    if (blockIdx.y == 0) nt_count_body<UNA>(lds, m, n, a.ns, ntt, a.dv, a.idx, order_src, rank, a.tile_cursor, a.list_cursor, a.tile_list_off, a.tile_list_n, a.lists);
-    else                 nt_count_body<UNB>(lds, m, n, b.ns, ntt, b.dv, b.idx, order_src, rank, b.tile_cursor, b.list_cursor, b.tile_list_off, b.tile_list_n, b.lists);
+    if (blockIdx.y == 0) nt_scatter_body<UNA>(lds, m, n, ntt, order_src, rank, a);
+    else                 nt_scatter_body<UNB>(lds, m, n, ntt, order_src, rank, b);
 }
 
 __global__ __launch_bounds__(1024) void nt_scan_kernel(int ntt, const int* __restrict__ tile_cursor, int* __restrict__ tile_base)
@@ -150,67 +160,6 @@
     if (threadIdx.x == 1023) tile_base[ntt] = run;
 }
 
-template <int UN, bool SCANNED>
-__device__ __forceinline__ void nt_bin_body(int* lds, int m, int n, int ns, int ntt, CblFastDiv dv, const int* __restrict__ idx, const int* __restrict__ order_src,
-                                            const int* __restrict__ rank, const int* __restrict__ tile_cursor, const int* __restrict__ tile_list_off,
-                                            const int* __restrict__ tile_list_n, const int2* __restrict__ lists, int* __restrict__ tile_base,
-                                            int2* __restrict__ bins)
-{
-    int* where = lds;
-    int* hist = lds + ntt;
-    __shared__ int wave_tot[NB / 64], src_ids[TS];
-    const int st = blockIdx.x;
-    const int nsrc = min(TS, m - st * TS);
-    if ((int)threadIdx.x < TS) src_ids[threadIdx.x] = (int)threadIdx.x < nsrc ? (order_src ? order_src[st * TS + threadIdx.x] : st * TS + (int)threadIdx.x) : 0;
-    if (SCANNED) {
-        const int nl0 = tile_list_n[st], lo0 = tile_list_off[st];
-        for (int e = threadIdx.x; e < nl0; e += NB) { const int2 r = lists[lo0 + e]; where[r.x] = tile_base[r.x] + r.y; hist[r.x] = 0; }
-        __syncthreads();
-    } else {
-    for (int e = threadIdx.x; e < ntt; e += NB) { where[e] = tile_cursor[e]; hist[e] = 0; }
-    __syncthreads();
-    const int per = (ntt + NB - 1) / NB;
-    const int c0 = threadIdx.x * per, c1 = min(ntt, c0 + per);
-    int sum = 0;
-    for (int e = c0; e < c1; e++) sum += where[e];
-    int incl = sum;
-    for (int k = 1; k < 64; k <<= 1) { const int v = __shfl_up(incl, k); if ((threadIdx.x & 63) >= k) incl += v; }
-    if ((threadIdx.x & 63) == 63) wave_tot[threadIdx.x >> 6] = incl;
-    __syncthreads();
-    int run = incl - sum;
-    for (int w = 0; w < (int)(threadIdx.x >> 6); w++) run += wave_tot[w];
-    for (int e = c0; e < c1; e++) { const int c = where[e]; where[e] = run; if (st == 0) tile_base[e] = run; run += c; }
-    if (st == 0 && threadIdx.x == NB - 1) tile_base[ntt] = run;
-    __syncthreads();
-    const int nl = tile_list_n[st], lo = tile_list_off[st];
-    for (int e = threadIdx.x; e < nl; e += NB) { const int2 r = lists[lo + e]; where[r.x] += r.y; }
-    __syncthreads();
-    }
-    const unsigned total = (unsigned)nsrc * (unsigned)ns;
-    for (unsigned base = 0; base < total; base += UN * NB) {
-        NtPairs<UN> q;
-        nt_load_pairs<UN>(q, base, total, n, ns, dv, src_ids, idx, rank);
-#pragma unroll
-        for (int u = 0; u < UN; u++)
-            if (q.r[u] >= 0) { const int tt = q.r[u] / TT; bins[where[tt] + atomicAdd(&hist[tt], 1)] = make_int2(q.r[u] & (TT - 1), (int)q.p[u]); }
-    }
-}
-template <int UN, bool SCANNED>
-__global__ __launch_bounds__(NB) void nt_bin_kernel(int m, int n, int ns, int ntt, CblFastDiv dv, const int* __restrict__ idx, const int* __restrict__ order_src,
-                                                    const int* __restrict__ rank, const int* __restrict__ tile_cursor, const int* __restrict__ tile_list_off,
-                                                    const int* __restrict__ tile_list_n, const int2* __restrict__ lists, int* __restrict__ tile_base,
-                                                    int2* __restrict__ bins)
-{
-    extern __shared__ int lds[];
-    nt_bin_body<UN, SCANNED>(lds, m, n, ns, ntt, dv, idx, order_src, rank, tile_cursor, tile_list_off, tile_list_n, lists, tile_base, bins);
-}
-template <int UNA, int UNB>
-__global__ __launch_bounds__(NB) void nt_bin_pair_kernel(int m, int n, int ntt, const int* __restrict__ order_src, const int* __restrict__ rank, NtJob a, NtJob b)
-{
-    extern __shared__ int lds[];
-    if (blockIdx.y == 0) nt_bin_body<UNA, false>(lds, m, n, a.ns, ntt, a.dv, a.idx, order_src, rank, a.tile_cursor, a.tile_list_off, a.tile_list_n, a.lists, a.tile_base, a.bins);
-    else                 nt_bin_body<UNB, false>(lds, m, n, b.ns, ntt, b.dv, b.idx, order_src, rank, b.tile_cursor, b.tile_list_off, b.tile_list_n, b.lists, b.tile_base, b.bins);
-}
 
 constexpr int EPT = 16;
 
@@ -283,26 +232,43 @@
     }
 }
 
-__device__ __forceinline__ void nt_finish_body(int n, int ntt, const int* __restrict__ tile_base, const int2* __restrict__ bins, int* __restrict__ scratch,
-                                               int* __restrict__ inv_start, int* __restrict__ inv_src)
-{
-    __shared__ int cnt[TT], lstart[TT + 1];
+template <bool SCANNED>
+__device__ __forceinline__ void nt_finish_body(int n, int ntt, const NtJob& j)
+{
+    __shared__ int cnt[TT], lstart[TT + 1], wave_tot[NB / 64];
     __shared__ int stage_lds[STAGE_CAP];
     const int tt = blockIdx.x;
-    const int b0 = tile_base[tt], E = tile_base[tt + 1] - b0;
-    const bool in_regs = E <= EPT * NB;
+    const int E = j.tile_cursor[tt];
+    const int Eb = min(E, j.cap);
+    const int novf = E > j.cap ? *j.ovf_cursor : 0;
+    const int2* __restrict__ bin = j.bins + (size_t)tt * (size_t)j.cap;
+    const int2* __restrict__ ovf = j.ovf;
+    const bool in_regs = E <= EPT * NB && E <= j.cap;
     if (threadIdx.x < TT) cnt[threadIdx.x] = 0;
     int2 r[EPT];
     if (in_regs) {
 #pragma unroll
-        for (int u = 0; u < EPT; u++) { const int e = u * NB + (int)threadIdx.x; r[u] = e < E ? bins[b0 + e] : make_int2(-1, 0); }
-    }
+        for (int u = 0; u < EPT; u++) { const int e = u * NB + (int)threadIdx.x; r[u] = e < E ? bin[e] : make_int2(-1, 0); }
+    }
+    int b0 = 0;
+    if (SCANNED) b0 = j.tile_base[tt];
+    else {
+        int sum = 0;
+        for (int e = threadIdx.x; e < tt; e += NB) sum += j.tile_cursor[e];
+        for (int k = 1; k < 64; k <<= 1) { const int v = __shfl_up(sum, k); if ((int)(threadIdx.x & 63) >= k) sum += v; }
+        if ((threadIdx.x & 63) == 63) wave_tot[threadIdx.x >> 6] = sum;
+    }
+    auto entries = [&](auto f) {
+        for (int e = threadIdx.x; e < Eb; e += NB) { const int2 v = bin[e]; f(v.x, v.y); }
+        for (int e = threadIdx.x; e < novf; e += NB) { const int2 v = ovf[e]; if (v.x / TT == tt) f(v.x & (TT - 1), v.y); }
+    };
     __syncthreads();
+    if (!SCANNED) for (int w = 0; w < NB / 64; w++) b0 += wave_tot[w];
     if (in_regs) {
 #pragma unroll
         for (int u = 0; u < EPT; u++) if (r[u].x >= 0) atomicAdd(&cnt[r[u].x], 1);
     } else {
-        for (int e = threadIdx.x; e < E; e += NB) atomicAdd(&cnt[bins[b0 + e].x], 1);
+        entries([&](int slot, int) { atomicAdd(&cnt[slot], 1); });
     }
     __syncthreads();
     if (threadIdx.x < 64) {
@@ -312,8 +278,8 @@
         lstart[threadIdx.x] = incl - c;
         if (threadIdx.x == 63) lstart[TT] = incl;
         const int row = tt * TT + threadIdx.x;
-        if (row < n) inv_start[row] = b0 + incl - c;
-        if (tt == ntt - 1 && threadIdx.x == 63) inv_start[n] = b0 + incl;
+        if (row < n) j.inv_start[row] = b0 + incl - c;
+        if (tt == ntt - 1 && threadIdx.x == 63) j.inv_start[n] = b0 + incl;
         cnt[threadIdx.x] = 0;
     }
     __syncthreads();
@@ -322,28 +288,29 @@
 #pragma unroll
             for (int u = 0; u < EPT; u++) if (r[u].x >= 0) stage_lds[lstart[r[u].x] + atomicAdd(&cnt[r[u].x], 1)] = r[u].y;
         } else {
-            for (int e = threadIdx.x; e < E; e += NB) { const int2 v = bins[b0 + e]; stage_lds[lstart[v.x] + atomicAdd(&cnt[v.x], 1)] = v.y; }
+            entries([&](int slot, int pair) { stage_lds[lstart[slot] + atomicAdd(&cnt[slot], 1)] = pair; });
         }
         __syncthreads();
-        nt_rank_sort(stage_lds, lstart, inv_src + b0);
+        nt_rank_sort(stage_lds, lstart, j.inv_src + b0);
     } else {
-        int* stage = scratch + b0;
-        for (int e = threadIdx.x; e < E; e += NB) { const int2 v = bins[b0 + e]; stage[lstart[v.x] + atomicAdd(&cnt[v.x], 1)] = v.y; }
+        int* stage = j.scratch + b0;
+        entries([&](int slot, int pair) { stage[lstart[slot] + atomicAdd(&cnt[slot], 1)] = pair; });
         __threadfence_block();
         __syncthreads();
-        nt_rank_sort(stage, lstart, inv_src + b0);
-    }
-}
-__global__ __launch_bounds__(NB) void nt_finish_kernel(int n, int ntt, const int* __restrict__ tile_base, const int2* __restrict__ bins, int* __restrict__ scratch,
-                                                       int* __restrict__ inv_start, int* __restrict__ inv_src)
-{
-    nt_finish_body(n, ntt, tile_base, bins, scratch, inv_start, inv_src);
+        nt_rank_sort(stage, lstart, j.inv_src + b0);
+    }
+}
+template <bool SCANNED>
+__global__ __launch_bounds__(NB) void nt_finish_kernel(int n, int ntt, NtJob a)
+{
+    nt_finish_body<SCANNED>(n, ntt, a);
 }
 __global__ __launch_bounds__(NB) void nt_finish_pair_kernel(int n, int ntt, NtJob a, NtJob b)
 {
-    const bool fa = blockIdx.y == 0;
-    nt_finish_body(n, ntt, fa ? a.tile_base : b.tile_base, fa ? a.bins : b.bins, fa ? a.scratch : b.scratch, fa ? a.inv_start : b.inv_start, fa ? a.inv_src : b.inv_src);
-}
+    const NtJob j = blockIdx.y == 0 ? a : b;
+    nt_finish_body<false>(n, ntt, j);
+}
+
 
 template <int LG>
 __global__ __launch_bounds__(NB) void grouping_bwd_csr_kernel(unsigned n, const float4* __restrict__ go, const int* __restrict__ order,
@@ -433,6 +400,24 @@
 
 }
 
+static NtJob nt_job(const NtWs& w, int ns, const int* idx, int* inv_start, int* inv_src)
+{
+    NtJob j;
+    j.ns = ns; j.cap = w.cap; j.dv = cbl_fastdiv_make((unsigned)ns); j.idx = idx;
+    j.tile_cursor = w.tile_cursor; j.ovf_cursor = w.ovf_cursor; j.tile_base = w.tile_base;
+    j.bins = w.bins; j.ovf = w.ovf; j.scratch = w.scratch; j.inv_start = inv_start; j.inv_src = inv_src;
+    return j;
+}
+static int nt_un(int ns) { const int per_thread = (TS * ns + NB - 1) / NB; return per_thread <= 4 ? 4 : per_thread <= 8 ? 8 : 16; }
+
+static const int* nt_begin(hipStream_t st, int n, const int* order_dst, const int* rank_dst, int* rank_ws, int* zero, int nzero)
+{
+    const bool invert = order_dst && !rank_dst;
+    const int work = invert && n > nzero ? n : nzero;
+    hipLaunchKernelGGL(nt_prep_kernel, dim3(cbl_div_up(work, NB)), dim3(NB), 0, st, invert ? n : 0, nzero, order_dst, rank_ws, zero);
+    return invert ? rank_ws : (order_dst ? rank_dst : nullptr);
+}
+
 CBL_EXPORT size_t cbl_neighbor_transpose_workspace_bytes(int m, int n, int nsample)
 {
     if (m < 0 || n < 0 || nsample <= 0) return 0;
@@ -440,8 +425,8 @@
     return nt_carve(w, nullptr, m, n, nsample);
 }
 
-CBL_EXPORT int cbl_neighbor_transpose(int m, int n, int nsample, const int* idx, const int* order_src, const int* order_dst, int* inv_start, int* inv_src,
-                                      void* workspace, size_t workspace_bytes, void* stream)
+CBL_EXPORT int cbl_neighbor_transpose_ranked(int m, int n, int nsample, const int* idx, const int* order_src, const int* order_dst, const int* rank_dst,
+                                             int* inv_start, int* inv_src, void* workspace, size_t workspace_bytes, void* stream)
 {
     if (m < 0 || n < 0 || nsample <= 0 || !inv_start) return CBL_ERR_BAD_ARG;
     if ((long long)m * nsample > 0x7fffffffLL) return CBL_ERR_BAD_ARG;
@@ -455,27 +440,26 @@
     if (ntt > NT_MAX_TILES) return CBL_ERR_UNSUPPORTED;
     NtWs w;
     if (nt_carve(w, (char*)workspace, m, n, nsample) > workspace_bytes) return CBL_ERR_WORKSPACE;
-    const CblFastDiv dv = cbl_fastdiv_make((unsigned)nsample);
-    const int nzero = ntt + 2;
-    hipLaunchKernelGGL(nt_prep_kernel, dim3(cbl_div_up(n > nzero ? n : nzero, NB)), dim3(NB), 0, st, n, nzero, order_dst, w.rank, w.tile_cursor, (int*)nullptr);
-    const int* rank = order_dst ? w.rank : nullptr;
-    const long long cap = (long long)TS * nsample < ntt ? (long long)TS * nsample : ntt;
-    const size_t lds_count = sizeof(int) * (size_t)((ntt + 1) & ~1) + sizeof(int2) * (size_t)cap, lds_bin = sizeof(int) * 2 * (size_t)ntt;
-#define CBL_NT(UN_)                                                                                                                                   \
-    hipLaunchKernelGGL((nt_count_kernel<UN_>), dim3(nst), dim3(NB), lds_count, st, m, n, nsample, ntt, dv, idx, order_src, rank, w.tile_cursor,       \
-                       w.list_cursor, w.tile_list_off, w.tile_list_n, w.lists);                                                                       \
-    if (ntt > NT_SCAN_SPLIT) {                                                                                                                        \
-        hipLaunchKernelGGL(nt_scan_kernel, dim3(1), dim3(1024), 0, st, ntt, w.tile_cursor, w.tile_base);                                              \
-        hipLaunchKernelGGL((nt_bin_kernel<UN_, true>), dim3(nst), dim3(NB), lds_bin, st, m, n, nsample, ntt, dv, idx, order_src, rank, w.tile_cursor, \
-                           w.tile_list_off, w.tile_list_n, w.lists, w.tile_base, w.bins);                                                             \
-    } else                                                                                                                                            \
-        hipLaunchKernelGGL((nt_bin_kernel<UN_, false>), dim3(nst), dim3(NB), lds_bin, st, m, n, nsample, ntt, dv, idx, order_src, rank, w.tile_cursor, \
-                           w.tile_list_off, w.tile_list_n, w.lists, w.tile_base, w.bins)
-    const int per_thread = (TS * nsample + NB - 1) / NB;
-    if (per_thread <= 4) { CBL_NT(4); } else if (per_thread <= 8) { CBL_NT(8); } else { CBL_NT(16); }
-#undef CBL_NT
-    hipLaunchKernelGGL(nt_finish_kernel, dim3(ntt), dim3(NB), 0, st, n, ntt, w.tile_base, w.bins, w.scratch, inv_start, inv_src);
+    const int* rank = nt_begin(st, n, order_dst, rank_dst, w.rank, w.tile_cursor, ntt + 2);
+    const NtJob j = nt_job(w, nsample, idx, inv_start, inv_src);
+    const size_t lds = sizeof(int) * 2 * (size_t)ntt;
+    switch (nt_un(nsample)) {
+        case 4: hipLaunchKernelGGL((nt_scatter_kernel<4>), dim3(nst), dim3(NB), lds, st, m, n, ntt, order_src, rank, j); break;
+        case 8: hipLaunchKernelGGL((nt_scatter_kernel<8>), dim3(nst), dim3(NB), lds, st, m, n, ntt, order_src, rank, j); break;
+        default: hipLaunchKernelGGL((nt_scatter_kernel<16>), dim3(nst), dim3(NB), lds, st, m, n, ntt, order_src, rank, j); break;
+    }
+    if (ntt > NT_SCAN_SPLIT) {
+        hipLaunchKernelGGL(nt_scan_kernel, dim3(1), dim3(1024), 0, st, ntt, w.tile_cursor, w.tile_base);
+        hipLaunchKernelGGL((nt_finish_kernel<true>), dim3(ntt), dim3(NB), 0, st, n, ntt, j);
+    } else
+        hipLaunchKernelGGL((nt_finish_kernel<false>), dim3(ntt), dim3(NB), 0, st, n, ntt, j);
     return cbl_status();
+}
+
+CBL_EXPORT int cbl_neighbor_transpose(int m, int n, int nsample, const int* idx, const int* order_src, const int* order_dst, int* inv_start, int* inv_src,
+                                      void* workspace, size_t workspace_bytes, void* stream)
+{
+    return cbl_neighbor_transpose_ranked(m, n, nsample, idx, order_src, order_dst, nullptr, inv_start, inv_src, workspace, workspace_bytes, stream);
 }
 
 CBL_EXPORT size_t cbl_neighbor_transpose_pair_workspace_bytes(int m, int n, int nsample_a, int nsample_b)
@@ -485,8 +469,9 @@
     return nt_carve(w, nullptr, m, n, nsample_a) + nt_carve(w, nullptr, m, n, nsample_b);
 }
 
-CBL_EXPORT int cbl_neighbor_transpose_pair(int m, int n, int nsample_a, const int* idx_a, int nsample_b, const int* idx_b, const int* order_src, const int* order_dst,
-                                           int* inv_start_a, int* inv_src_a, int* inv_start_b, int* inv_src_b, void* workspace, size_t workspace_bytes, void* stream)
+CBL_EXPORT int cbl_neighbor_transpose_pair_ranked(int m, int n, int nsample_a, const int* idx_a, int nsample_b, const int* idx_b, const int* order_src,
+                                                  const int* order_dst, const int* rank_dst, int* inv_start_a, int* inv_src_a, int* inv_start_b, int* inv_src_b,
+                                                  void* workspace, size_t workspace_bytes, void* stream)
 {
     if (m < 0 || n < 0 || nsample_a <= 0 || nsample_b <= 0 || !inv_start_a || !inv_start_b) return CBL_ERR_BAD_ARG;
     if ((long long)m * nsample_a > 0x7fffffffLL || (long long)m * nsample_b > 0x7fffffffLL) return CBL_ERR_BAD_ARG;
@@ -495,42 +480,37 @@
     const size_t bytes_a = nt_carve(wa, (char*)workspace, m, n, nsample_a);
     if (m == 0 || n == 0 || ntt > NT_SCAN_SPLIT) {
         if (m > 0 && n > 0 && (!workspace || bytes_a + nt_carve(wb, nullptr, m, n, nsample_b) > workspace_bytes)) return workspace ? CBL_ERR_WORKSPACE : CBL_ERR_BAD_ARG;
-        const int rc = cbl_neighbor_transpose(m, n, nsample_a, idx_a, order_src, order_dst, inv_start_a, inv_src_a, workspace, bytes_a, stream);
+        const int rc = cbl_neighbor_transpose_ranked(m, n, nsample_a, idx_a, order_src, order_dst, rank_dst, inv_start_a, inv_src_a, workspace, bytes_a, stream);
         if (rc) return rc;
-        return cbl_neighbor_transpose(m, n, nsample_b, idx_b, order_src, order_dst, inv_start_b, inv_src_b, workspace ? (char*)workspace + bytes_a : nullptr,
-                                      workspace_bytes > bytes_a ? workspace_bytes - bytes_a : 0, stream);
+        return cbl_neighbor_transpose_ranked(m, n, nsample_b, idx_b, order_src, order_dst, rank_dst, inv_start_b, inv_src_b,
+                                             workspace ? (char*)workspace + bytes_a : nullptr, workspace_bytes > bytes_a ? workspace_bytes - bytes_a : 0, stream);
     }
     if (!idx_a || !idx_b || !inv_src_a || !inv_src_b || !workspace) return CBL_ERR_BAD_ARG;
     if (bytes_a + nt_carve(wb, (char*)workspace + bytes_a, m, n, nsample_b) > workspace_bytes) return CBL_ERR_WORKSPACE;
     hipStream_t st = cbl_stream(stream);
-    auto job = [&](const NtWs& w, int ns, const int* idx, int* inv_start, int* inv_src) {
-        NtJob j;
-        j.ns = ns; j.dv = cbl_fastdiv_make((unsigned)ns); j.idx = idx;
-        j.tile_cursor = w.tile_cursor; j.list_cursor = w.list_cursor; j.tile_list_off = w.tile_list_off; j.tile_list_n = w.tile_list_n; j.tile_base = w.tile_base;
-        j.lists = w.lists; j.bins = w.bins; j.scratch = w.scratch; j.inv_start = inv_start; j.inv_src = inv_src;
-        return j;
-    };
+    wb.tile_cursor = wa.tile_cursor + ntt + 2; wb.ovf_cursor = wb.tile_cursor + ntt + 1;
+    const int* rank = nt_begin(st, n, order_dst, rank_dst, wa.rank, wa.tile_cursor, 2 * (ntt + 2));
     const bool swap = nsample_b > nsample_a;
-    const NtJob ja = swap ? job(wb, nsample_b, idx_b, inv_start_b, inv_src_b) : job(wa, nsample_a, idx_a, inv_start_a, inv_src_a);
-    const NtJob jb = swap ? job(wa, nsample_a, idx_a, inv_start_a, inv_src_a) : job(wb, nsample_b, idx_b, inv_start_b, inv_src_b);
-    const int nzero = ntt + 2;
-    hipLaunchKernelGGL(nt_prep_kernel, dim3(cbl_div_up(n > nzero ? n : nzero, NB)), dim3(NB), 0, st, n, nzero, order_dst, wa.rank, wa.tile_cursor, wb.tile_cursor);
-    const int* rank = order_dst ? wa.rank : nullptr;
-    const int ns_max = ja.ns;
-    const long long cap = (long long)TS * ns_max < ntt ? (long long)TS * ns_max : ntt;
-    const size_t lds_count = sizeof(int) * (size_t)((ntt + 1) & ~1) + sizeof(int2) * (size_t)cap, lds_bin = sizeof(int) * 2 * (size_t)ntt;
-    auto un_of = [](int ns) { const int per_thread = (TS * ns + NB - 1) / NB; return per_thread <= 4 ? 4 : per_thread <= 8 ? 8 : 16; };
-    const int una = un_of(ja.ns), unb = un_of(jb.ns);
+    const NtJob ja = swap ? nt_job(wb, nsample_b, idx_b, inv_start_b, inv_src_b) : nt_job(wa, nsample_a, idx_a, inv_start_a, inv_src_a);
+    const NtJob jb = swap ? nt_job(wa, nsample_a, idx_a, inv_start_a, inv_src_a) : nt_job(wb, nsample_b, idx_b, inv_start_b, inv_src_b);
+    const size_t lds = sizeof(int) * 2 * (size_t)ntt;
+    const int una = nt_un(ja.ns), unb = nt_un(jb.ns);
     const dim3 gsrc(nst, 2), gdst(ntt, 2);
-#define CBL_NTP(UA_, UB_)                                                                                                                        \
-    { hipLaunchKernelGGL((nt_count_pair_kernel<UA_, UB_>), gsrc, dim3(NB), lds_count, st, m, n, ntt, order_src, rank, ja, jb);                  \
-      hipLaunchKernelGGL((nt_bin_pair_kernel<UA_, UB_>), gsrc, dim3(NB), lds_bin, st, m, n, ntt, order_src, rank, ja, jb); }
+#define CBL_NTP(UA_, UB_) { hipLaunchKernelGGL((nt_scatter_pair_kernel<UA_, UB_>), gsrc, dim3(NB), lds, st, m, n, ntt, order_src, rank, ja, jb); }
     if (una == 16 && unb == 16) CBL_NTP(16, 16) else if (una == 16 && unb == 8) CBL_NTP(16, 8) else if (una == 16) CBL_NTP(16, 4)
     else if (una == 8 && unb == 8) CBL_NTP(8, 8) else if (una == 8) CBL_NTP(8, 4) else CBL_NTP(4, 4)
 #undef CBL_NTP
     hipLaunchKernelGGL(nt_finish_pair_kernel, gdst, dim3(NB), 0, st, n, ntt, ja, jb);
     return cbl_status();
 }
+
+CBL_EXPORT int cbl_neighbor_transpose_pair(int m, int n, int nsample_a, const int* idx_a, int nsample_b, const int* idx_b, const int* order_src, const int* order_dst,
+                                           int* inv_start_a, int* inv_src_a, int* inv_start_b, int* inv_src_b, void* workspace, size_t workspace_bytes, void* stream)
+{
+    return cbl_neighbor_transpose_pair_ranked(m, n, nsample_a, idx_a, nsample_b, idx_b, order_src, order_dst, nullptr, inv_start_a, inv_src_a, inv_start_b, inv_src_b,
+                                              workspace, workspace_bytes, stream);
+}
+
 
 CBL_EXPORT int cbl_grouping_backward_csr(int n, int c, const float* grad_output, const int* order_dst, const int* inv_start, const int* inv_src,
                                          float* grad_input, void* stream)
diff --git a/contrastboundary_amd/neighbor_state.py b/contrastboundary_amd/neighbor_state.py
--- a/contrastboundary_amd/neighbor_state.py
+++ b/contrastboundary_amd/neighbor_state.py
@@ -45,10 +45,12 @@
     return ent is None or stream_id not in ent
 
 
-def _order_register(points, order, stream):
+def _order_register(points, order, stream, rank=None):
     key = _order_key(points)
     ent = _order_registry.setdefault(key, {})
     ent[stream.cuda_stream] = (order, stream)
+    if rank is not None:
+        order._cbl_rank = rank
     _order_registry.move_to_end(key)
     while len(_order_registry) > _ORDER_REGISTRY_MAX:
         _order_registry.popitem(last=False)
@@ -109,6 +111,15 @@
     order.record_stream(cur)
     ent[cur.cuda_stream] = (order, cur)
     return order
+
+
+def new_order(n, device):
+    both = torch.empty(2 * n, dtype=torch.int32, device=device)
+    return both[:n], both[n:]
+
+
+def order_rank(order):
+    return None if order is None else getattr(order, "_cbl_rank", None)
 
 
 use_spatial_order = True
diff --git a/contrastboundary_amd/pointops.py b/contrastboundary_amd/pointops.py
--- a/contrastboundary_amd/pointops.py
+++ b/contrastboundary_amd/pointops.py
@@ -184,17 +184,17 @@
     ws = _workspace(need, dev)
     cur = torch.cuda.current_stream(dev)
     self_search = new_xyz is xyz or (new_xyz.data_ptr() == xyz.data_ptr() and m == n)
-    order = torch.empty(n, dtype=torch.int32, device=dev) if (self_search and _order_wanted(xyz, cur.cuda_stream)) else None
+    order, rank = neighbor_state.new_order(n, dev) if (self_search and _order_wanted(xyz, cur.cuda_stream)) else (None, None)
     pw = 1 if algo_wide == "set" else 2 if algo_wide == "anytie" else 0
-    rc = L.cbl_knnquery_nested(_c_int(b), _c_int(n), _c_int(m), _c_int(nsample_wide), _c_int(pw), _c_int(nsample), _c_int(1 if algo == "set" else 0),
-                               _lib.ptr(xyz), _lib.ptr(new_xyz), _lib.ptr(offset), _lib.ptr(new_offset), _lib.ptr(wi), _lib.ptr(wd), _lib.ptr(idx),
-                               _lib.ptr(dist2), _lib.ptr(order), ctypes.c_void_p(event.cuda_event if event is not None else 0),
-                               _lib.ptr(ws), ctypes.c_size_t(ws.numel()), _lib.stream_of(xyz))
+    rc = L.cbl_knnquery_nested_ranked(_c_int(b), _c_int(n), _c_int(m), _c_int(nsample_wide), _c_int(pw), _c_int(nsample), _c_int(1 if algo == "set" else 0),
+                                      _lib.ptr(xyz), _lib.ptr(new_xyz), _lib.ptr(offset), _lib.ptr(new_offset), _lib.ptr(wi), _lib.ptr(wd), _lib.ptr(idx),
+                                      _lib.ptr(dist2), _lib.ptr(order), _lib.ptr(rank), ctypes.c_void_p(event.cuda_event if event is not None else 0),
+                                      _lib.ptr(ws), ctypes.c_size_t(ws.numel()), _lib.stream_of(xyz))
     if rc == _lib.ERR_UNSUPPORTED:
         return None
-    _lib.check(rc, "cbl_knnquery_nested")
+    _lib.check(rc, "cbl_knnquery_nested_ranked")
     if order is not None:
-        _order_register(xyz, order, cur)
+        _order_register(xyz, order, cur, rank)
     if self_search and n >= ORDER_MIN_POINTS and neighbor_state.use_spatial_order:
         _order_alias(wi, xyz); _order_alias(idx, xyz)
     return wi, wd, idx, dist2
@@ -218,15 +218,15 @@
         cur = torch.cuda.current_stream(xyz.device)
         self_search = new_xyz is xyz or (new_xyz.data_ptr() == xyz.data_ptr() and m == n)
         if self_search and need and nsample <= 64 and _order_wanted(xyz, cur.cuda_stream):
-            order = torch.empty(n, dtype=torch.int32, device=xyz.device)
+            order, rank = neighbor_state.new_order(n, xyz.device)
             policy = 1 if algo == "set" else 2 if algo == "anytie" else 0
-            rc = L.cbl_knnquery_ordered(*args, _c_int(policy), _lib.ptr(order), _lib.ptr(ws), ctypes.c_size_t(ws.numel()), st)
+            rc = L.cbl_knnquery_ordered_ranked(*args, _c_int(policy), _lib.ptr(order), _lib.ptr(rank), _lib.ptr(ws), ctypes.c_size_t(ws.numel()), st)
             if rc == 0:
-                _order_register(xyz, order, cur)
+                _order_register(xyz, order, cur, rank)
                 _order_alias(idx, xyz)
                 return idx, dist2
             if rc != _lib.ERR_UNSUPPORTED:
-                _lib.check(rc, "cbl_knnquery_ordered")
+                _lib.check(rc, "cbl_knnquery_ordered_ranked")
         fn = L.cbl_knnquery_set if algo == "set" else L.cbl_knnquery_anytie if algo == "anytie" else L.cbl_knnquery
         _lib.check(fn(*args, _lib.ptr(ws), ctypes.c_size_t(ws.numel() if ws is not None else 0), st), "cbl_knnquery")
         if self_search and n >= ORDER_MIN_POINTS and neighbor_state.use_spatial_order:
@@ -262,6 +262,7 @@
         return hit
     m, nsample = idx.shape
     order = spatial_order(idx) if m == n else None
+    rank = neighbor_state.order_rank(order)
     L = _lib.lib()
     inv_start = torch.empty(n + 1, dtype=torch.int32, device=idx.device)
     inv_src = torch.empty(max(m * nsample, 1), dtype=torch.int32, device=idx.device)
@@ -271,9 +272,9 @@
         inv_start2 = torch.empty(n + 1, dtype=torch.int32, device=idx.device)
         inv_src2 = torch.empty(max(m * ns2, 1), dtype=torch.int32, device=idx.device)
         ws = _workspace(max(L.cbl_neighbor_transpose_pair_workspace_bytes(_c_int(m), _c_int(n), _c_int(nsample), _c_int(ns2)), 1), idx.device)
-        rc = L.cbl_neighbor_transpose_pair(_c_int(m), _c_int(n), _c_int(nsample), _lib.ptr(idx), _c_int(ns2), _lib.ptr(companion), _lib.ptr(order), _lib.ptr(order),
-                                           _lib.ptr(inv_start), _lib.ptr(inv_src), _lib.ptr(inv_start2), _lib.ptr(inv_src2), _lib.ptr(ws), ctypes.c_size_t(ws.numel()),
-                                           _lib.stream_of(idx))
+        rc = L.cbl_neighbor_transpose_pair_ranked(_c_int(m), _c_int(n), _c_int(nsample), _lib.ptr(idx), _c_int(ns2), _lib.ptr(companion), _lib.ptr(order),
+                                                  _lib.ptr(order), _lib.ptr(rank), _lib.ptr(inv_start), _lib.ptr(inv_src), _lib.ptr(inv_start2), _lib.ptr(inv_src2),
+                                                  _lib.ptr(ws), ctypes.c_size_t(ws.numel()), _lib.stream_of(idx))
         if rc == _lib.ERR_UNSUPPORTED:
             return None
         _lib.check(rc, "cbl_neighbor_transpose_pair")
@@ -281,8 +282,8 @@
         neighbor_state.transpose_register(companion, order, inv_start2, inv_src2)
         return order, inv_start, inv_src
     ws = _workspace(max(L.cbl_neighbor_transpose_workspace_bytes(_c_int(m), _c_int(n), _c_int(nsample)), 1), idx.device)
-    rc = L.cbl_neighbor_transpose(_c_int(m), _c_int(n), _c_int(nsample), _lib.ptr(idx), _lib.ptr(order), _lib.ptr(order), _lib.ptr(inv_start),
-                                  _lib.ptr(inv_src), _lib.ptr(ws), ctypes.c_size_t(ws.numel()), _lib.stream_of(idx))
+    rc = L.cbl_neighbor_transpose_ranked(_c_int(m), _c_int(n), _c_int(nsample), _lib.ptr(idx), _lib.ptr(order), _lib.ptr(order), _lib.ptr(rank), _lib.ptr(inv_start),
+                                         _lib.ptr(inv_src), _lib.ptr(ws), ctypes.c_size_t(ws.numel()), _lib.stream_of(idx))
     if rc == _lib.ERR_UNSUPPORTED:
         return None
     _lib.check(rc, "cbl_neighbor_transpose")
diff --git a/include/cbl_amd.h b/include/cbl_amd.h
--- a/include/cbl_amd.h
+++ b/include/cbl_amd.h
@@ -43,6 +43,11 @@
                          const int* offset, const int* new_offset,
                          int* idx, float* dist2, int tie_policy, int* cell_order,
                          void* workspace, size_t workspace_bytes, void* stream);
+int cbl_knnquery_ordered_ranked(int b, int n, int m, int nsample,
+                                const float* xyz, const float* new_xyz,
+                                const int* offset, const int* new_offset,
+                                int* idx, float* dist2, int tie_policy, int* cell_order, int* cell_rank,
+                                void* workspace, size_t workspace_bytes, void* stream);
 
 int cbl_knn_grid_block_candidates(int b, int n, int nsample, const int* offset, int* count, void* workspace, size_t workspace_bytes, void* stream);
 
@@ -56,6 +61,10 @@
                         const float* xyz, const float* new_xyz, const int* offset, const int* new_offset,
                         int* idx_wide, float* dist2_wide, int* idx, float* dist2, int* cell_order, void* event_after_wide,
                         void* workspace, size_t workspace_bytes, void* stream);
+int cbl_knnquery_nested_ranked(int b, int n, int m, int nsample_wide, int tie_policy_wide, int nsample, int tie_policy,
+                               const float* xyz, const float* new_xyz, const int* offset, const int* new_offset,
+                               int* idx_wide, float* dist2_wide, int* idx, float* dist2, int* cell_order, int* cell_rank, void* event_after_wide,
+                               void* workspace, size_t workspace_bytes, void* stream);
 
 int cbl_knnquery_exact(int b, int n, int m, int nsample,
                        const float* xyz, const float* new_xyz,
@@ -77,9 +86,14 @@
 size_t cbl_neighbor_transpose_workspace_bytes(int m, int n, int nsample);
 int cbl_neighbor_transpose(int m, int n, int nsample, const int* idx, const int* order_src, const int* order_dst, int* inv_start, int* inv_src,
                            void* workspace, size_t workspace_bytes, void* stream);
+int cbl_neighbor_transpose_ranked(int m, int n, int nsample, const int* idx, const int* order_src, const int* order_dst, const int* rank_dst, int* inv_start,
+                                  int* inv_src, void* workspace, size_t workspace_bytes, void* stream);
 size_t cbl_neighbor_transpose_pair_workspace_bytes(int m, int n, int nsample_a, int nsample_b);
 int cbl_neighbor_transpose_pair(int m, int n, int nsample_a, const int* idx_a, int nsample_b, const int* idx_b, const int* order_src, const int* order_dst,
                                 int* inv_start_a, int* inv_src_a, int* inv_start_b, int* inv_src_b, void* workspace, size_t workspace_bytes, void* stream);
+int cbl_neighbor_transpose_pair_ranked(int m, int n, int nsample_a, const int* idx_a, int nsample_b, const int* idx_b, const int* order_src, const int* order_dst,
+                                       const int* rank_dst, int* inv_start_a, int* inv_src_a, int* inv_start_b, int* inv_src_b, void* workspace,
+                                       size_t workspace_bytes, void* stream);
 int cbl_grouping_backward_csr(int n, int c, const float* grad_output, const int* order_dst, const int* inv_start, const int* inv_src,
                               float* grad_input, void* stream);
 int cbl_grouping_backward_csr_rows(int n, int c, int row_stride, int col_offset, const float* grad_output, const int* order_dst,
```
